# datvo06/MSAU

Measured on AMD Instinct MI355X. Metric: chargrid tiles/sec (train fwd+bwd), 336x256x64 3-stage MSAU, higher is better.
Workload: dtype bf16; 1 GPU; configs[1]: one-hot chargrid 336x256x64, 3-stage MSAU (featRoot 8, 4 scales, res_depth 2), batch 16/GPU, fwd+masked-CE+bwd+clip+Adam; global_batch=16, parallelism=dp1, graph=False

## Files before the change

### include/msau_hip.h

```cpp
#ifndef MSAU_HIP_H
#define MSAU_HIP_H

#include <stdint.h>

#ifdef __cplusplus
extern "C" {
#endif

typedef enum { MSAU_F32 = 0, MSAU_BF16 = 1 } msau_dtype;

typedef enum {
    MSAU_OK = 0,
    MSAU_ERR_ARG = -1,
    MSAU_ERR_LDS = -2,
    MSAU_ERR_HIP = -3
} msau_status;

const char* msau_last_error(void);
int msau_version(void);
const char* msau_source_hash(void);
int msau_sizeof(int which);
int msau_lds_pixel_stride(int raw_bytes, int esz, int c8_per_chunk, int read_stride);
int msau_lds_wrow_stride(int nks, int esz);

enum {
    MSAU_CONV_RELU_IN  = 1,
    MSAU_CONV_RELU_OUT = 2,
    MSAU_CONV_ADD      = 4,
    MSAU_CONV_ACCUM    = 8,
    MSAU_CONV_MASK_A   = 16,
    MSAU_CONV_MASK_B   = 32,
    MSAU_CONV_DOUT     = 128,
    MSAU_CONV_LRN      = 256,
    MSAU_CONV_POOL     = 512,
    MSAU_CONV_IDS      = 1024,
    MSAU_CONV_OWNER    = 2048,
    MSAU_CONV_NCHW     = 4096,
    MSAU_CONV_WGRAD    = 8192,
    MSAU_CONV_ELU      = 32768,
    MSAU_CONV_EXTENT   = 65536,
    MSAU_CONV_HEAD     = 64
};

typedef struct {
    int32_t B, Hin, Win, Hout, Wout;
    int32_t C1, C2;
    int32_t Cout;
    int32_t KH, KW, dil;
    int32_t pad_t, pad_l;
    int32_t stride;
    int32_t ups;
    int32_t flags;
    const void* x1;
    const void* x2;
    const void* wpack;
    const float* bias;
    const void* add;
    const void* mask_a;
    const void* mask_b;
    void* y;
    float* head_probs;
    uint8_t* head_argmax;
    int32_t head_classes;
    int32_t flags2;
    void* y2;
    const void* mask_b2;
    float lrn_alpha_over_n, lrn_beta, lrn_k;
    int32_t reserved0;
    void* pool_y;
    uint8_t* pool_idx;
    const void* wg_x1;
    float* wg_slabs;
    int32_t wg_nslabs;
    int32_t reserved1;
    const int32_t* extent;
} msau_conv_desc;
int msau_conv2d_rider_slabs(int dtype, const msau_conv_desc* d);

typedef struct {
    int32_t cch;
    int32_t nchunks;
    int32_t kchunk;
    int32_t rows;
    int64_t bytes;
} msau_conv_pack_geom;

int msau_conv_pack_geometry(int dtype, int C1_stored, int C2_stored, int Cout_stored, int KH, int KW, int dil,
                            int stride, int ups, msau_conv_pack_geom* out);
int msau_conv2d(void* stream, int dtype, const msau_conv_desc* d);
int msau_conv2d_launch_info(int dtype, const msau_conv_desc* d, int32_t* info8);

enum { MSAU_PAIR_RELU_IN = 1, MSAU_PAIR_RELU_MID = 2, MSAU_PAIR_MASK_MID = 4,
       MSAU_PAIR_LRN_BWD = 16,
       MSAU_PAIR_WGRAD1 = 32,
       MSAU_PAIR_COUPLE = 64,
       MSAU_PAIR_DCOUPLE = 128,
       MSAU_PAIR_TILES = 8 };
typedef struct {
    int32_t B, H, W, C;
    int32_t flags1, flags2;
    const void* x;
    const void* w1;
    const float* b1;
    const void* mask_mid;
    void* mid;
    const void* w2;
    const float* b2;
    const void* add;
    const void* mask_a;
    const void* mask_b;
    void* y;
    void* pool_y;
    uint8_t* pool_idx;
    uint8_t* bits_mid;
    uint8_t* bits_a;
    const void* lrn_a;
    void* lrn_da;
    float lrn_alpha_over_n, lrn_beta, lrn_k;
    int32_t reserved0;
    const void* wg1_x;
    float* wg1_slabs;
    int32_t wg1_nslabs;
    int32_t reserved1;
    const void* cpl_prev;
    const void* cpl_w;
    const float* cpl_b;
    void* cpl_y;
    void* cpl_pool_y;
    uint8_t* cpl_pool_idx;
    const void* dcp_dz;
    const void* dcp_w;
    const void* dcp_mask;
    void* dcp_dprev;
} msau_conv_pair_desc;
int msau_conv_pair_applicable(int dtype, const msau_conv_pair_desc* d);
int msau_conv_pair(void* stream, int dtype, const msau_conv_pair_desc* d);
int64_t msau_conv_pair_bits_bytes(int dtype, const msau_conv_pair_desc* d);
int msau_conv_pair_wgrad_slabs(int dtype, const msau_conv_pair_desc* d);
int msau_conv_pair_instance(int dtype, const msau_conv_pair_desc* d);
void msau_reload_env(void);

typedef struct {
    int32_t B, Hin, Win, Hout, Wout;
    int32_t C1, C2, Cout;
    int32_t KH, KW, dil, pad_t, pad_l, stride;
    int32_t flags;
    const void* x1;
    const void* x2;
    const void* g;
    float* slabs;
    int32_t nslabs;
} msau_wgrad_desc;

typedef struct {
    int32_t cch, nchunks;
    int32_t kext;
    int32_t max_slabs;
    int64_t slab_bytes;
    int32_t lean;
    int32_t reserved;
} msau_wgrad_geom;

int msau_wgrad_geometry(int dtype, const msau_wgrad_desc* d, msau_wgrad_geom* out);
int msau_conv2d_wgrad(void* stream, int dtype, const msau_wgrad_desc* d);
int msau_conv2d_wgrad_groupable(int dtype, const msau_wgrad_desc* a, const msau_wgrad_desc* b);
int msau_conv2d_wgrad_group(void* stream, int dtype, const msau_wgrad_desc* const* ds, int n);

typedef struct {
    int64_t src_off;
    int64_t dst_off;
    int32_t kind;
    int32_t dim0, dim1;
    int32_t KH, KW;
    int32_t row_is_dim0;
    int32_t flip;
    int32_t row_off;
    int32_t rows_real;
    int32_t rows_pad;
    int32_t k1_real, k1_store, k2_real, k2_store;
    int32_t cch, nchunks, kchunk;
    int32_t dtype;
} msau_pack_entry;

int msau_pack_params(void* stream, const float* flat_params, void* pack_arena,
                     const msau_pack_entry* table_dev, int n_entries, int max_elems_per_entry);

typedef struct {
    int64_t slab_off;
    int64_t w_off;
    int64_t b_off;
    int64_t b_src_off;
    int64_t b_slab_stride;
    int32_t b_elem_stride;
    int32_t b_nslabs;
    int32_t b_count;
    int32_t nslabs;
    int32_t slab_elems;
    int32_t kext;
    int32_t dim0, dim1, KH, KW;
    int32_t row_is_dim0;
    int32_t rows_real;
    int32_t k1_real, k1_store, k2_real, k2_store;
    int32_t cch, nchunks;
    int32_t accumulate;
} msau_unpack_entry;

int msau_wgrad_reduce(void* stream, const float* slab_arena, float* flat_grads,
                      const msau_unpack_entry* table_dev, int n_entries, int max_elems_per_entry);

int msau_channel_sum(void* stream, int dtype, const void* g, int64_t npix, int Cs, float* partials, int nblk);

int msau_nchw_to_nhwc(void* stream, int dtype, const float* src, void* dst, int B, int C, int Cs, int H, int W);
int msau_nhwc_to_nchw(void* stream, int dtype, const void* src, float* dst, int B, int C, int Cs, int H, int W);
int msau_nchw_grad_to_nhwc(void* stream, int dtype, const float* src, void* dst, int B, int C, int Cs, int H, int W,
                           int accumulate);

int msau_lrn_fwd(void* stream, int dtype, const void* a, void* y, int64_t npix, int C, int Cs, int n,
                 float alpha, float beta, float k);
int msau_lrn_bwd(void* stream, int dtype, const void* a, const void* dy, void* da, int64_t npix, int C, int Cs,
                 int n, float alpha, float beta, float k);

int msau_maxpool2x2_fwd(void* stream, int dtype, const void* x, void* y, uint8_t* idx, int B, int H, int W, int Cs);
int msau_maxpool2x2_bwd(void* stream, int dtype, const void* dy, const uint8_t* idx, void* dx, const void* mask,
                        int B, int H, int W, int Cs, int accumulate);
int msau_maxpool2x2_bwd_ext(void* stream, int dtype, const void* dy, const uint8_t* idx, void* dx, const void* mask,
                            int B, int H, int W, int Cs, int accumulate, const int32_t* extent);

int msau_selfattn_fwd(void* stream, int dtype, const void* f, const void* g, const void* h, const void* x, void* y,
                      float* stats , int B, int N, int Ds, int Cs);
int msau_selfattn_bwd(void* stream, int dtype, const void* f, const void* g, const void* h, const void* dy,
                      const float* stats, void* df, void* dg, void* dh, float* ws, int B, int N, int Ds, int Cs);
int msau_selfattn_fwd_ext(void* stream, int dtype, const void* f, const void* g, const void* h, const void* x, void* y,
                          float* stats, int B, int N, int Ds, int Cs, const int32_t* extent, int W);
int msau_selfattn_bwd_ext(void* stream, int dtype, const void* f, const void* g, const void* h, const void* dy,
                          const float* stats, void* df, void* dg, void* dh, float* ws, int B, int N, int Ds, int Cs,
                          const int32_t* extent, int W);

int msau_extent_copy(void* stream, const void* src, void* dst, int B, int planes, int H, int W, int pixel_bytes, const int32_t* extent);

typedef struct {
    const void* df; const void* dg; const void* dh;
    const void* wf_pack; const void* wg_pack; const void* wh_pack;
    const void* add;
    const void* mask_b;
    void* dx;
    int64_t npix;
    int32_t C, accumulate;
} msau_attn_proj_bwd_args;
int msau_attn_proj_bwd(void* stream, int dtype, const msau_attn_proj_bwd_args* a);

typedef struct {
    const void* g;
    const void* w1_pack; const void* w2_pack;
    void* dx1; void* dx2;
    const void* mask1; const void* mask2;
    int64_t npix;
    int32_t C, accumulate1, accumulate2, reserved;
} msau_dgrad2_args;
int msau_dgrad2_1x1(void* stream, int dtype, const msau_dgrad2_args* a);

int msau_label_counts(void* stream, const int64_t* labels, int32_t* counts, int B, int64_t hw);
int msau_label_counts_split(void* stream, const int64_t* labels, int32_t* partial, int B, int64_t hw, int K);
int64_t msau_ce_ws_floats(int64_t npix_total);
int msau_masked_ce(void* stream, int dtype, const void* logits, const int64_t* labels, const int32_t* counts,
                   void* dlogits, float* loss_accum, float* ws, int B, int64_t hw, int C, int Cs, float scale);
int64_t msau_ce_multi_ws_floats(int64_t npix_total);
int msau_masked_ce_multi(void* stream, int dtype, const void* logits, const void* aux, const int64_t* labels,
                         const int32_t* counts, void* dlogits, void* daux, float* loss, float* ws,
                         int B, int64_t hw, int C, int Cs, float scale, int counts_k);

int msau_softmax_ce(void* stream, int dtype, const void* logits, const int64_t* labels, void* dlogits,
                    float* loss_accum, float* ws, int B, int64_t hw, int C, int Cs, float scale);
int msau_softmax_ce_weighted(void* stream, int dtype, const void* logits, const int64_t* labels, const float* class_w,
                             void* dlogits, float* sums, float* ws, int B, int64_t hw, int C, int Cs);

int64_t msau_adam_ws_floats(int64_t n);
int msau_clip_adam_step(void* stream, float* params, const float* grads, float* m, float* v, float* state,
                        float* ws, int64_t n, float lr, float beta1, float beta2, float eps, float max_norm,
                        float grad_scale);

#define MSAU_OPTIM_ADAM 0
#define MSAU_OPTIM_RMSPROP 1
#define MSAU_OPTIM_MOMENTUM 2
#define MSAU_OPTIM_MAX_SKIP 8
int64_t msau_optim_ws_floats(int64_t n);
int msau_optim_step(void* stream, int kind, float* params, const float* grads, float* state_a, float* state_b, float* state,
                    float* ws, int64_t n, float lr, double c1, double c2, float eps, float weight_decay, float max_norm,
                    float grad_scale, const int64_t* skip, int n_skip);

int msau_raster_owner(void* stream, const int32_t* boxes, int n, int32_t* owner, int B, int H, int W);
int msau_raster_owner_ext(void* stream, const int32_t* boxes, int n, int32_t* owner, int B, int H, int W, const int32_t* extent);
int msau_raster_onehot(void* stream, int dtype, const int32_t* boxes, const int32_t* owner, void* grid_nhwc,
                       int B, int H, int W, int C, int Cs);
int msau_raster_labels(void* stream, const int32_t* boxes, const int32_t* owner, int64_t* labels, int B, int H, int W);
int msau_raster_dense(void* stream, int dtype, const int32_t* boxes, const int32_t* owner, const float* feats,
                      void* grid_nhwc, int B, int H, int W, int C, int Cs);

int64_t msau_box_integral_ws_floats(int B, int H, int W, int C);
int msau_box_integral(void* stream, int dtype, const void* in_nhwc, float* ii, float* ws, int B, int H, int W, int C, int Cs, int relu_in);
int msau_box_params(void* stream, const float* flat_params, int64_t off_hmin, int64_t off_hmax, int64_t off_wmin, int64_t off_wmax,
                    int C, int F, float max_h, float max_w, float* params_fwd, float* params_refl);
// ... 119 lines not shown
```

### msau_amd/_lib.py

```python
from __future__ import annotations

import ctypes as C
import os

HERE = os.path.dirname(os.path.abspath(__file__))
LIB_PATH = os.environ.get("MSAU_HIP_LIB", os.path.join(HERE, "libmsau_hip.so"))

F32, BF16 = 0, 1
OPTIM_ADAM, OPTIM_RMSPROP, OPTIM_MOMENTUM, OPTIM_MAX_SKIP = 0, 1, 2, 8

CONV_RELU_IN, CONV_RELU_OUT, CONV_ADD, CONV_ACCUM, CONV_MASK_A, CONV_MASK_B, CONV_HEAD, CONV_DOUT = 1, 2, 4, 8, 16, 32, 64, 128
CONV_LRN, CONV_POOL, CONV_IDS, CONV_OWNER, CONV_NCHW, CONV_WGRAD, CONV_ELU = 256, 512, 1024, 2048, 4096, 8192, 32768
CONV_EXTENT = 65536

i32, i64, vp, f32 = C.c_int32, C.c_int64, C.c_void_p, C.c_float


class ConvDesc(C.Structure):
    _fields_ = [(n, i32) for n in ("B", "Hin", "Win", "Hout", "Wout", "C1", "C2", "Cout", "KH", "KW", "dil",
                                   "pad_t", "pad_l", "stride", "ups", "flags")] + \
               [(n, vp) for n in ("x1", "x2", "wpack", "bias", "add", "mask_a", "mask_b", "y", "head_probs", "head_argmax")] + \
               [("head_classes", i32), ("flags2", i32), ("y2", vp), ("mask_b2", vp)] + \
               [("lrn_alpha_over_n", f32), ("lrn_beta", f32), ("lrn_k", f32), ("reserved0", i32), ("pool_y", vp), ("pool_idx", vp)] + \
               [("wg_x1", vp), ("wg_slabs", vp), ("wg_nslabs", i32), ("reserved1", i32), ("extent", vp)]


class ConvPairDesc(C.Structure):
    _fields_ = [(n, i32) for n in ("B", "H", "W", "C", "flags1", "flags2")] + \
               [(n, vp) for n in ("x", "w1", "b1", "mask_mid", "mid", "w2", "b2", "add", "mask_a", "mask_b", "y", "pool_y", "pool_idx", "bits_mid", "bits_a",
                                  "lrn_a", "lrn_da")] + \
               [("lrn_alpha_over_n", f32), ("lrn_beta", f32), ("lrn_k", f32), ("reserved0", i32), ("wg1_x", vp), ("wg1_slabs", vp), ("wg1_nslabs", i32), ("reserved1", i32)] + \
               [(n, vp) for n in ("cpl_prev", "cpl_w", "cpl_b", "cpl_y", "cpl_pool_y", "cpl_pool_idx", "dcp_dz", "dcp_w", "dcp_mask", "dcp_dprev")]


PAIR_RELU_IN, PAIR_RELU_MID, PAIR_MASK_MID, PAIR_TILES, PAIR_LRN_BWD, PAIR_WGRAD1, PAIR_COUPLE, PAIR_DCOUPLE = 1, 2, 4, 8, 16, 32, 64, 128


class BoxArgs(C.Structure):
    _fields_ = [(n, vp) for n in ("in_", "ii", "params_fwd", "params_refl", "out", "gout", "gin", "ii_g", "ws", "flat_grads", "ws_ii",
                                  "mask_a", "add", "mask_b")] + \
               [(n, i64) for n in ("off_hmin", "off_hmax", "off_wmin", "off_wmax")] + \
               [(n, i32) for n in ("B", "H", "W", "C", "F", "Cs_in", "Cs_out", "relu_in", "accumulate")] + \
               [("max_h", f32), ("max_w", f32)]


class ConvPackGeom(C.Structure):
    _fields_ = [("cch", i32), ("nchunks", i32), ("kchunk", i32), ("rows", i32), ("bytes", i64)]


class WgradDesc(C.Structure):
    _fields_ = [(n, i32) for n in ("B", "Hin", "Win", "Hout", "Wout", "C1", "C2", "Cout", "KH", "KW", "dil",
                                   "pad_t", "pad_l", "stride", "flags")] + \
               [(n, vp) for n in ("x1", "x2", "g", "slabs")] + [("nslabs", i32)]


class WgradGeom(C.Structure):
    _fields_ = [("cch", i32), ("nchunks", i32), ("kext", i32), ("max_slabs", i32), ("slab_bytes", i64),
                ("lean", i32), ("reserved", i32)]


class PackEntry(C.Structure):
    _fields_ = [("src_off", i64), ("dst_off", i64)] + \
               [(n, i32) for n in ("kind", "dim0", "dim1", "KH", "KW", "row_is_dim0", "flip", "row_off", "rows_real",
                                   "rows_pad", "k1_real", "k1_store", "k2_real", "k2_store", "cch", "nchunks",
                                   "kchunk", "dtype")]


class UnpackEntry(C.Structure):
    _fields_ = [("slab_off", i64), ("w_off", i64), ("b_off", i64), ("b_src_off", i64), ("b_slab_stride", i64)] + \
               [(n, i32) for n in ("b_elem_stride", "b_nslabs", "b_count", "nslabs", "slab_elems", "kext", "dim0", "dim1", "KH",
                                   "KW", "row_is_dim0", "rows_real", "k1_real", "k1_store", "k2_real", "k2_store",
                                   "cch", "nchunks", "accumulate")]


class Op(C.Structure):
    _fields_ = [("kind", i32), ("dtype", i32), ("args", vp)]


class LrnArgs(C.Structure):
    _fields_ = [("a", vp), ("dy", vp), ("out", vp), ("npix", i64), ("C", i32), ("Cs", i32), ("n", i32),
                ("alpha", f32), ("beta", f32), ("k", f32)]


class PoolArgs(C.Structure):
    _fields_ = [("x_or_dy", vp), ("y_or_dx", vp), ("idx", vp), ("mask", vp)] + \
               [(n, i32) for n in ("B", "H", "W", "Cs", "accumulate")] + [("extent", vp)]


class AttnArgs(C.Structure):
    _fields_ = [(n, vp) for n in ("f", "g", "h", "x_or_dy", "y", "stats", "df", "dg", "dh", "ws")] + \
               [(n, i32) for n in ("B", "N", "Ds", "Cs")] + [("extent", vp), ("W", i32), ("reserved0", i32)]


class CsumArgs(C.Structure):
    _fields_ = [("g", vp), ("npix", i64), ("Cs", i32), ("partials", vp), ("nblk", i32)]


class ReduceArgs(C.Structure):
    _fields_ = [("slab_arena", vp), ("flat_grads", vp), ("table_dev", vp), ("n_entries", i32), ("max_elems", i32)]


class AllreduceArgs(C.Structure):
    _fields_ = [("comm", vp), ("buf", vp), ("count", i64)]


class OwnerCtx(C.Structure):
    _fields_ = [(n, vp) for n in ("owner", "boxes", "feats", "w", "wt", "table", "sums", "csum")] + \
               [(n, i32) for n in ("n_boxes", "n_vec", "C", "csum_blocks", "wt_floats", "reserved0")]


class AttnProjBwdArgs(C.Structure):
    _fields_ = [(n, vp) for n in ("df", "dg", "dh", "wf_pack", "wg_pack", "wh_pack", "add", "mask_b", "dx")] + \
               [("npix", i64), ("C", i32), ("accumulate", i32)]


class Dgrad2Args(C.Structure):
    _fields_ = [(n, vp) for n in ("g", "w1_pack", "w2_pack", "dx1", "dx2", "mask1", "mask2")] + \
               [("npix", i64), ("C", i32), ("accumulate1", i32), ("accumulate2", i32), ("reserved", i32)]


OP_SIDE = 0x100
OP_PROBE = 0x200
OP_COMM = 0x400
OP_JOIN = 0x800
OP_ALLREDUCE = 14
OP_WGRAD_REDUCE = 10
OP_CONV_PAIR = 11
OP_BOX_FWD, OP_BOX_BWD = 12, 13
OP_ATTN_PROJ_BWD = 15
OP_DGRAD2_1X1 = 16
OP_CONV2D, OP_WGRAD, OP_LRN_FWD, OP_LRN_BWD, OP_POOL_FWD, OP_POOL_BWD, OP_ATTN_FWD, OP_ATTN_BWD, OP_CHANNEL_SUM = range(1, 10)

_SIGNATURES = {
    "msau_last_error": (C.c_char_p, []),
    "msau_version": (C.c_int, []),
    "msau_source_hash": (C.c_char_p, []),
    "msau_sizeof": (C.c_int, [C.c_int]),
    "msau_lds_pixel_stride": (C.c_int, [C.c_int, C.c_int, C.c_int, C.c_int]),
    "msau_lds_wrow_stride": (C.c_int, [C.c_int, C.c_int]),
    "msau_conv_pack_geometry": (C.c_int, [C.c_int] * 9 + [C.POINTER(ConvPackGeom)]),
    "msau_conv2d": (C.c_int, [vp, C.c_int, C.POINTER(ConvDesc)]),
    "msau_conv2d_rider_slabs": (C.c_int, [C.c_int, C.POINTER(ConvDesc)]),
    "msau_attn_proj_bwd": (C.c_int, [vp, C.c_int, C.POINTER(AttnProjBwdArgs)]),
    "msau_dgrad2_1x1": (C.c_int, [vp, C.c_int, C.POINTER(Dgrad2Args)]),
    "msau_conv2d_launch_info": (C.c_int, [C.c_int, C.POINTER(ConvDesc), C.POINTER(i32)]),
    "msau_conv_pair_applicable": (C.c_int, [C.c_int, C.POINTER(ConvPairDesc)]),
    "msau_conv_pair": (C.c_int, [vp, C.c_int, C.POINTER(ConvPairDesc)]),
    "msau_conv_pair_bits_bytes": (C.c_int64, [C.c_int, C.POINTER(ConvPairDesc)]),
    "msau_conv_pair_instance": (C.c_int, [C.c_int, C.POINTER(ConvPairDesc)]),
    "msau_conv_pair_wgrad_slabs": (C.c_int, [C.c_int, C.POINTER(ConvPairDesc)]),
    "msau_owner_slabs": (C.c_int, [C.POINTER(WgradDesc)]),
    "msau_comm_available": (C.c_int, []),
    "msau_comm_unique_id": (C.c_int, [vp, C.c_int]),
    "msau_comm_init": (C.c_int, [C.POINTER(vp), C.c_int, C.c_int, vp, C.c_int]),
    "msau_comm_destroy": (C.c_int, [vp]),
    "msau_allreduce_bucket": (C.c_int, [vp, vp, vp, C.c_int64]),
    "msau_run_ops_dp": (C.c_int, [vp, vp, vp, C.POINTER(Op), C.c_int, C.c_int]),
    "msau_reload_env": (None, []),
    "msau_wgrad_geometry": (C.c_int, [C.c_int, C.POINTER(WgradDesc), C.POINTER(WgradGeom)]),
    "msau_conv2d_wgrad": (C.c_int, [vp, C.c_int, C.POINTER(WgradDesc)]),
    "msau_conv2d_wgrad_groupable": (C.c_int, [C.c_int, C.POINTER(WgradDesc), C.POINTER(WgradDesc)]),
    "msau_conv2d_wgrad_group": (C.c_int, [vp, C.c_int, C.POINTER(C.POINTER(WgradDesc)), C.c_int]),
    "msau_pack_params": (C.c_int, [vp, vp, vp, vp, C.c_int, C.c_int]),
    "msau_wgrad_reduce": (C.c_int, [vp, vp, vp, vp, C.c_int, C.c_int]),
    "msau_channel_sum": (C.c_int, [vp, C.c_int, vp, i64, C.c_int, vp, C.c_int]),
    "msau_nchw_to_nhwc": (C.c_int, [vp, C.c_int, vp, vp] + [C.c_int] * 5),
    "msau_nhwc_to_nchw": (C.c_int, [vp, C.c_int, vp, vp] + [C.c_int] * 5),
    "msau_nchw_grad_to_nhwc": (C.c_int, [vp, C.c_int, vp, vp] + [C.c_int] * 6),
    "msau_lrn_fwd": (C.c_int, [vp, C.c_int, vp, vp, i64, C.c_int, C.c_int, C.c_int, f32, f32, f32]),
    "msau_lrn_bwd": (C.c_int, [vp, C.c_int, vp, vp, vp, i64, C.c_int, C.c_int, C.c_int, f32, f32, f32]),
    "msau_maxpool2x2_fwd": (C.c_int, [vp, C.c_int, vp, vp, vp] + [C.c_int] * 4),
    "msau_maxpool2x2_bwd": (C.c_int, [vp, C.c_int, vp, vp, vp, vp] + [C.c_int] * 5),
    "msau_selfattn_fwd": (C.c_int, [vp, C.c_int, vp, vp, vp, vp, vp, vp] + [C.c_int] * 4),
    "msau_selfattn_bwd": (C.c_int, [vp, C.c_int, vp, vp, vp, vp, vp, vp, vp, vp, vp] + [C.c_int] * 4),
    "msau_maxpool2x2_bwd_ext": (C.c_int, [vp, C.c_int, vp, vp, vp, vp] + [C.c_int] * 5 + [vp]),
    "msau_selfattn_fwd_ext": (C.c_int, [vp, C.c_int, vp, vp, vp, vp, vp, vp] + [C.c_int] * 4 + [vp, C.c_int]),
    "msau_selfattn_bwd_ext": (C.c_int, [vp, C.c_int, vp, vp, vp, vp, vp, vp, vp, vp, vp] + [C.c_int] * 4 + [vp, C.c_int]),
    "msau_extent_copy": (C.c_int, [vp, vp, vp] + [C.c_int] * 5 + [vp]),
    "msau_label_counts": (C.c_int, [vp, vp, vp, C.c_int, i64]),
    "msau_label_counts_split": (C.c_int, [vp, vp, vp, C.c_int, i64, C.c_int]),
    "msau_ce_ws_floats": (i64, [i64]),
    "msau_ce_multi_ws_floats": (i64, [i64]),
    "msau_masked_ce_multi": (C.c_int, [vp, C.c_int, vp, vp, vp, vp, vp, vp, vp, vp, C.c_int, i64, C.c_int, C.c_int, f32, C.c_int]),
    "msau_masked_ce": (C.c_int, [vp, C.c_int, vp, vp, vp, vp, vp, vp, C.c_int, i64, C.c_int, C.c_int, f32]),
    "msau_softmax_ce": (C.c_int, [vp, C.c_int, vp, vp, vp, vp, vp, C.c_int, i64, C.c_int, C.c_int, f32]),
    "msau_softmax_ce_weighted": (C.c_int, [vp, C.c_int, vp, vp, vp, vp, vp, vp, C.c_int, i64, C.c_int, C.c_int]),
    "msau_adam_ws_floats": (i64, [i64]),
    "msau_clip_adam_step": (C.c_int, [vp, vp, vp, vp, vp, vp, vp, i64, f32, f32, f32, f32, f32, f32]),
    "msau_optim_ws_floats": (i64, [i64]),
    "msau_optim_step": (C.c_int, [vp, C.c_int, vp, vp, vp, vp, vp, vp, i64, f32, C.c_double, C.c_double, f32, f32, f32, f32, vp, C.c_int]),
    "msau_raster_owner": (C.c_int, [vp, vp, C.c_int, vp, C.c_int, C.c_int, C.c_int]),
    "msau_raster_owner_ext": (C.c_int, [vp, vp, C.c_int, vp, C.c_int, C.c_int, C.c_int, vp]),
    "msau_raster_onehot": (C.c_int, [vp, C.c_int, vp, vp, vp] + [C.c_int] * 5),
    "msau_raster_labels": (C.c_int, [vp, vp, vp, vp, C.c_int, C.c_int, C.c_int]),
    "msau_raster_dense": (C.c_int, [vp, C.c_int, vp, vp, vp, vp] + [C.c_int] * 5),
    "msau_box_integral_ws_floats": (i64, [C.c_int] * 4),
    "msau_box_integral": (C.c_int, [vp, C.c_int, vp, vp, vp] + [C.c_int] * 6),
    "msau_box_params": (C.c_int, [vp, vp, i64, i64, i64, i64, C.c_int, C.c_int, f32, f32, vp, vp]),
    "msau_box_filter": (C.c_int, [vp, C.c_int, vp, vp, vp] + [C.c_int] * 8 + [vp, vp, vp]),
    "msau_box_fwd": (C.c_int, [vp, C.c_int, C.POINTER(BoxArgs)]),
    "msau_box_bwd": (C.c_int, [vp, C.c_int, C.POINTER(BoxArgs)]),
    "msau_box_pgrad_ws_floats": (i64, [C.c_int] * 5),
    "msau_box_param_grad": (C.c_int, [vp, C.c_int, vp, vp, vp, vp, vp, i64, i64, i64, i64] + [C.c_int] * 6 + [f32, f32]),
    "msau_run_ops": (C.c_int, [vp, C.POINTER(Op), C.c_int]),
    "msau_run_ops_overlap": (C.c_int, [vp, vp, C.POINTER(Op), C.c_int, C.c_int]),
    "msau_spin": (C.c_int, [vp, C.c_int]),
    "msau_fill_zero": (C.c_int, [vp, vp, i64]),
    "msau_fork_visibility_check": (C.c_int, [vp, vp, C.c_int, i64, C.c_int, C.POINTER(i64)]),
    "msau_stream_create": (C.c_int, [C.c_int, C.POINTER(vp)]),
    "msau_stream_destroy": (C.c_int, [vp]),
    "msau_softmax_channels_nchw": (C.c_int, [vp, vp, vp, C.c_int, C.c_int, i64]),
    "msau_probe_read": (C.c_int, [vp, C.c_int, vp]),
    "msau_probe_overhead": (C.c_int, [vp, C.c_int, vp]),
    "msau_softmax_argmax_nhwc": (C.c_int, [vp, C.c_int, vp, vp, vp, i64, C.c_int, C.c_int]),
    "msau_onehot_ids": (C.c_int, [vp, C.c_int, vp, vp, i64, C.c_int, C.c_int]),
    "msau_onehot_ids_ext": (C.c_int, [vp, C.c_int, vp, vp] + [C.c_int] * 5 + [vp]),
    "msau_eval_confusion": (C.c_int, [vp, C.c_int, vp, vp, vp] + [C.c_int] * 6 + [vp]),
    "msau_kv_regions_limits": (C.c_int, [C.POINTER(i32)]),
    "msau_kv_regions": (C.c_int, [vp] * 7 + [C.c_int] * 4 + [vp, vp, C.c_int, vp, C.c_int, vp]),
    "msau_kv_paint": (C.c_int, [vp] * 6 + [C.c_int] * 3 + [vp, vp, vp]),
    "msau_kv_paint_train": (C.c_int, [vp] * 7 + [C.c_int] * 3 + [vp, vp, vp]),
    "msau_label_hist": (C.c_int, [vp, vp, vp, vp] + [C.c_int] * 5),
    "msau_unet_ce_ws_floats": (i64, [i64]),
    "msau_unet_ce": (C.c_int, [vp, C.c_int] + [vp] * 7 + [C.c_int, vp, vp, vp, vp] + [C.c_int] * 5),
    "msau_unet_eval_ws_bytes": (i64, [C.c_int, C.c_int]),
    "msau_unet_eval": (C.c_int, [vp, C.c_int] + [vp] * 6 + [C.c_int, vp, vp, vp] + [C.c_int] * 5),
}

EXPORTED_SYMBOLS = tuple(_SIGNATURES)

ABI_STRUCTS = (ConvDesc, WgradDesc, PackEntry, UnpackEntry, Op, LrnArgs, PoolArgs, AttnArgs, CsumArgs, ReduceArgs,
               ConvPackGeom, WgradGeom, ConvPairDesc, BoxArgs, AllreduceArgs, OwnerCtx, AttnProjBwdArgs, Dgrad2Args)


class MsauHipError(RuntimeError):
    pass


_lib = None


def load():
    global _lib
    if _lib is not None:
        return _lib
    if not os.path.exists(LIB_PATH):
        raise MsauHipError(f"{LIB_PATH} not found: the MSAU HIP kernels are not built "
                           f"(run `python -m msau_amd.build`); there is no CPU fallback")
    lib = C.CDLL(LIB_PATH)
    for name, (res, args) in _SIGNATURES.items():
        fn = getattr(lib, name)
        fn.restype = res
        fn.argtypes = args
    for which, st in enumerate(ABI_STRUCTS):
        if lib.msau_sizeof(which) != C.sizeof(st):
            raise MsauHipError(f"{LIB_PATH}: sizeof({st.__name__}) is {lib.msau_sizeof(which)} in the library, "
                               f"{C.sizeof(st)} in msau_amd/_lib.py -- rebuild (python -m msau_amd.build)")
    if "MSAU_HIP_LIB" not in os.environ and os.path.isdir(os.path.join(HERE, "csrc")):
        from .build import source_hash
        have, want = lib.msau_source_hash().decode(), source_hash()
        if have != want:
            raise MsauHipError(f"{LIB_PATH} was built from kernel sources {have}, the tree holds {want}: rebuild "
                               f"(python -m msau_amd.build)")
    _lib = lib
    return lib


def check(rc: int, what: str = ""):
    if rc != 0:
        msg = load().msau_last_error().decode("utf-8", "replace")
        raise MsauHipError(f"{what or 'msau call'} failed (status {rc}): {msg}")


class Profiler:

    def __init__(self):
        self.records = []
        self.key = None

    def summary(self):
        import collections
        out = collections.OrderedDict()
        for key, e0, e1 in self.records:
            c, t = out.get(key, (0, 0.0))
            out[key] = (c + 1, t + e0.elapsed_time(e1))
        return out


_profiler = None


def set_profiler(p):
    global _profiler
    _profiler = p


def call(name: str, *args, key=None):
    if _profiler is None:
# ... 48 lines not shown
```

### msau_amd/csrc/conv.hip

```cpp
#include "msau_common.h"

namespace {

struct ConvGeom {
    int esz, taps, cch, nchunks, kchunk, rows, CT, ngroups;
    int nslices;
};

__host__ __device__ inline int pix_stride_bytes(int cch, int esz) {
    int ps = cch * esz;
    if (((ps >> 4) & 1) == 0) ps += 16;
    return ps;
}

struct TileGeom { int TH, TIH, TIW, PS, WS, in_bytes, w_bytes, tab_bytes, total; };

inline bool conv_compact(int KH, int KW, int dil, int stride, int ups) { return stride == 1 && ups == 1 && dil >= 16 && KH * KW > 1; }

inline TileGeom tile_geom(const ConvGeom& g, int PT, int KH, int KW, int dil, int stride, int ups = 1) {
    TileGeom t;
    t.TH = 4 * PT;
    t.TIH = (t.TH - 1) * stride + (KH - 1) * dil + 1;
    t.TIW = 15 * stride + (KW - 1) * dil + 1;
    if (conv_compact(KH, KW, dil, stride, ups)) { t.TIH = KH * KW * t.TH; t.TIW = 16; }
// ... 161 lines not shown
            }
            *reinterpret_cast<V8*>(lds_in + pix * a.PS + cg * 8 * (int)sizeof(T)) = v;
        }
        const T* wsrc = wp + ((size_t)chunk * a.rows_total + ct0 * 16) * a.kchunk;
        for (int idx = tid; idx < rows * wg_per_row; idx += 256) {
            int r = idx / wg_per_row, g8 = idx - r * wg_per_row;
            *reinterpret_cast<V8*>(lds_w + r * a.WS + g8 * 8 * (int)sizeof(T)) = load8<T>(wsrc + (size_t)r * a.kchunk + g8 * 8);
        }
        __syncthreads();
        for (int ks = 0; ks < nks; ++ks) {
            const int G = ks * 4 + lg;
            const int koff = koff_tab[G];
            V8 bfrag[PT];
#pragma unroll
            for (int pt = 0; pt < PT; ++pt) bfrag[pt] = *reinterpret_cast<const V8*>(lds_in + pixoff[pt] + koff);
#pragma unroll
            for (int ct = 0; ct < CT; ++ct) {
                V8 afrag = *reinterpret_cast<const V8*>(lds_w + (ct * 16 + lr) * a.WS + G * 8 * (int)sizeof(T));
#pragma unroll
                for (int pt = 0; pt < PT; ++pt) acc[ct][pt] = mma8(afrag, bfrag[pt], acc[ct][pt]);
            }
        }
    }

    const int Cout = d.Cout;
    T* y = static_cast<T*>(d.y);
    const T* add = static_cast<const T*>(d.add);
    const T* mask_a = static_cast<const T*>(d.mask_a);
    const T* mask_b = static_cast<const T*>(d.mask_b);
    const int flags = d.flags;
    int ext_h = d.Hout, ext_w = d.Wout;
    if (flags & MSAU_CONV_EXTENT) { ext_h = d.extent[2 * b]; ext_w = d.extent[2 * b + 1]; }
#pragma unroll
    for (int pt = 0; pt < PT; ++pt) {
        const int oy = oy0 + wave * PT + pt, ox = ox0 + lr;
        if (oy >= d.Hout || ox >= d.Wout) continue;
        const bool outside = oy >= ext_h || ox >= ext_w;
        const size_t pbase = (((size_t)b * d.Hout + oy) * d.Wout + ox) * a.ystride;
#pragma unroll
        for (int ct = 0; ct < CT; ++ct) {
            const int co = lg * (CTT * 4) + (ct0 + ct) * 4;
            if (co >= Cout) continue;
            f32x4 v = acc[ct][pt];
            if (d.bias) {
                f32x4 bv = *reinterpret_cast<const f32x4*>(d.bias + co);
                v += bv;
            }
            if (flags & MSAU_CONV_MASK_A) {
                V4 m = load4<T>(mask_a + pbase + co);
#pragma unroll
                for (int j = 0; j < 4; ++j) v[j] = ((float)m[j] > 0.f) ? v[j] : 0.f;
            }
            if (flags & MSAU_CONV_ADD) {
                V4 r = load4<T>(add + pbase + co);
#pragma unroll
                for (int j = 0; j < 4; ++j) v[j] += (float)r[j];
            }
            if (flags & MSAU_CONV_ACCUM) {
                V4 r = load4<T>(y + pbase + co);
#pragma unroll
                for (int j = 0; j < 4; ++j) v[j] += (float)r[j];
            }
            if (flags & MSAU_CONV_RELU_OUT) {
                if (flags & MSAU_CONV_ELU) {
#pragma unroll
                    for (int j = 0; j < 4; ++j) v[j] = v[j] > 0.f ? v[j] : expm1f(v[j]);
                } else {
#pragma unroll
                    for (int j = 0; j < 4; ++j) v[j] = fmaxf(v[j], 0.f);
                }
            }
            if (flags & MSAU_CONV_MASK_B) {
                V4 m = load4<T>(mask_b + pbase + co);
                if (flags & MSAU_CONV_ELU) {
#pragma unroll
                    for (int j = 0; j < 4; ++j) v[j] = ((float)m[j] > 0.f) ? v[j] : v[j] * ((float)m[j] + 1.f);
                } else {
#pragma unroll
                    for (int j = 0; j < 4; ++j) v[j] = ((float)m[j] > 0.f) ? v[j] : 0.f;
                }
            }
            if (outside) v = f32x4{0.f, 0.f, 0.f, 0.f};
            V4 o;
#pragma unroll
            for (int j = 0; j < 4; ++j) o[j] = (T)v[j];
            store4<T>(y + pbase + co, o);
        }
    }
}

template <typename T, int CT, int PT>
int launch_conv(hipStream_t s, const ConvArgs& a, int nblocks, int nsplit, int lds) {
    static bool attr_set = false;
    if (!attr_set) {
        hipError_t e = hipFuncSetAttribute(reinterpret_cast<const void*>(&conv_kernel<T, CT, PT>),
                                           hipFuncAttributeMaxDynamicSharedMemorySize, MSAU_LDS_LIMIT);
        if (e != hipSuccess) return msau_set_error(MSAU_ERR_HIP, "conv: hipFuncSetAttribute: %s", hipGetErrorString(e));
        attr_set = true;
    }
    hipLaunchKernelGGL((conv_kernel<T, CT, PT>), dim3(nblocks, nsplit), dim3(256), lds, s, a);
    MSAU_CHECK_LAUNCH("conv_kernel");
    return 0;
}

template <typename T, int CT>
int launch_conv_pt(hipStream_t s, const ConvArgs& a, int PT, int nblocks, int nsplit, int lds) {
    switch (PT) {
        case 4: return launch_conv<T, CT, 4>(s, a, nblocks, nsplit, lds);
        case 2: return launch_conv<T, CT, 2>(s, a, nblocks, nsplit, lds);
        default: return launch_conv<T, CT, 1>(s, a, nblocks, nsplit, lds);
    }
}

template <typename T>
int launch_conv_ct(hipStream_t s, const ConvArgs& a, int CT, int PT, int nblocks, int nsplit, int lds) {
    switch (CT) {
        case 1: return launch_conv_pt<T, 1>(s, a, PT, nblocks, nsplit, lds);
        case 2: return launch_conv_pt<T, 2>(s, a, PT, nblocks, nsplit, lds);
        case 4: return launch_conv_pt<T, 4>(s, a, PT, nblocks, nsplit, lds);
        default: return launch_conv_pt<T, 8>(s, a, PT, nblocks, nsplit, lds);
    }
}

}

extern "C" int msau_conv_pack_geometry(int dtype, int C1, int C2, int Cout, int KH, int KW, int dil, int stride, int ups,
                                       msau_conv_pack_geom* out) {
    ConvGeom g;
    int rc = conv_geom(dtype, C1, C2, Cout, KH, KW, dil, stride, ups, &g);
    if (rc) return rc;
    out->cch = g.cch; out->nchunks = g.nchunks; out->kchunk = g.kchunk; out->rows = g.rows * g.nslices;
    out->bytes = (int64_t)g.nslices * g.nchunks * g.rows * g.kchunk * g.esz;
    return 0;
}

static int conv_plan(int dtype, const msau_conv_desc* d, ConvGeom* gout, TileGeom* tout, int* PTout, int64_t* nbout) {
    ConvGeom g;
    int rc = conv_geom(dtype, d->C1, d->C2, d->Cout, d->KH, d->KW, d->dil, d->stride, d->ups, &g);
    if (rc) return rc;
    int PT = 4;
    auto ntiles = [&](int pt) { return (int64_t)d->B * cdiv(d->Hout, 4 * pt) * cdiv(d->Wout, 16); };
    if (ntiles(4) < 512) PT = ntiles(2) >= 384 ? 2 : 1;
    TileGeom t = tile_geom(g, PT, d->KH, d->KW, d->dil, d->stride, d->ups);
    while (t.total > 150 * 1024 && PT > 1) { PT >>= 1; t = tile_geom(g, PT, d->KH, d->KW, d->dil, d->stride, d->ups); }
    if (t.total > 150 * 1024) return msau_set_error(MSAU_ERR_LDS, "conv2d: tile needs %d B of LDS", t.total);
    int64_t nb = ntiles(PT);
    MSAU_CHECK_ARG(nb < (1ll << 31), "conv2d: grid too large");
    *gout = g; *tout = t; *PTout = PT; *nbout = nb;
    return 0;
}

enum { CONV_TILE = 0, CONV_LEAN = 1, CONV_CHUNKED = 2, CONV_ROWS = 3,
       CONV_OWNER = 4, CONV_FIRST_NCHW = 5, CONV_REFUSED = 6 };
constexpr int kRefusalOrder[] = {MSAU_CONV_EXTENT, MSAU_CONV_WGRAD, MSAU_CONV_OWNER, MSAU_CONV_NCHW, MSAU_CONV_HEAD, MSAU_CONV_DOUT,
                                 MSAU_CONV_LRN, MSAU_CONV_IDS, MSAU_CONV_POOL};
constexpr int kOnlyOthers = MSAU_CONV_WGRAD | MSAU_CONV_OWNER | MSAU_CONV_NCHW | MSAU_CONV_HEAD | MSAU_CONV_DOUT | MSAU_CONV_LRN |
                            MSAU_CONV_IDS | MSAU_CONV_POOL;
struct ConvRoute {
    int family, inst;
    int refused;
    int geom_rc;
    ConvGeom g; TileGeom t; int PT; int64_t nb;
};

static int conv_route(int dtype, const msau_conv_desc* d, ConvRoute* r, int families = ~0) {
    const int f = d->flags;
    auto asked = [&](int family) { return (families >> family) & 1; };
    *r = ConvRoute{};
    r->family = CONV_REFUSED;
    const int rc = r->geom_rc = conv_plan(dtype, d, &r->g, &r->t, &r->PT, &r->nb);
    if (f & MSAU_CONV_OWNER) {
        if (asked(CONV_OWNER) && msau_ownerconv_takes(dtype, d)) { r->family = CONV_OWNER; r->inst = 1; return 0; }
    } else if (f & MSAU_CONV_NCHW) {
        if (asked(CONV_FIRST_NCHW) && msau_firstconv_takes(dtype, d)) { r->family = CONV_FIRST_NCHW; r->inst = 1; return 0; }
    } else if (!rc) {
        const ConvGeom& g = r->g;
        if (g.nslices > 1) r->inst = 0;
        else if (asked(CONV_ROWS) && (r->inst = msau_rowconv_case(dtype, d))) r->family = CONV_ROWS;
        else if (asked(CONV_CHUNKED) && (r->inst = msau_conv_chunked_case(dtype, d, g.cch, g.nchunks, g.CT))) r->family = CONV_CHUNKED;
        else if (asked(CONV_LEAN) && (r->inst = msau_conv_lean_case(dtype, d, g.nchunks, g.CT))) r->family = CONV_LEAN;
        if (r->family == CONV_REFUSED && asked(CONV_TILE) && !(f & kOnlyOthers)) r->family = CONV_TILE;
    }
    if (rc) return rc;
    if (r->family == CONV_REFUSED)
        for (int flag : kRefusalOrder)
            if (f & flag) { r->refused = flag; break; }
    return 0;
}

static int conv_refusal(const msau_conv_desc* d, int flag) {
    switch (flag) {
        case MSAU_CONV_EXTENT:
            return msau_set_error(MSAU_ERR_ARG, "conv2d: MSAU_CONV_EXTENT is not implemented for this launch (flags 0x%x; see "
                                  "msau_conv2d_launch_info info[7] & 128): only the generic tile kernel and the box-list instance have it", d->flags);
        case MSAU_CONV_WGRAD:
            return msau_set_error(MSAU_ERR_ARG, "conv2d: MSAU_CONV_WGRAD is not implemented for this launch (msau_conv2d_rider_slabs says 0)");
        case MSAU_CONV_OWNER:
            return msau_set_error(MSAU_ERR_ARG, "conv2d: MSAU_CONV_OWNER is the 3x3 stride-1 C -> 8 conv, no other flag but RELU_OUT and EXTENT");
        case MSAU_CONV_NCHW:
            return msau_set_error(MSAU_ERR_ARG, "conv2d: MSAU_CONV_NCHW is the bf16 3x3 64 -> 8 conv (W %% 4 == 0, W <= 288), head_classes = real input channels");
        case MSAU_CONV_HEAD:
            return msau_set_error(MSAU_ERR_ARG, "conv2d: MSAU_CONV_HEAD is not implemented for this launch (see "
                                  "msau_conv2d_launch_info info[7]); run msau_softmax_argmax_nhwc on y instead");
        case MSAU_CONV_DOUT:
            return msau_set_error(MSAU_ERR_ARG, "conv2d: MSAU_CONV_DOUT is not implemented for this launch (see "
                                  "msau_conv2d_launch_info info[7]); issue one launch per output instead");
        case MSAU_CONV_LRN:
            return msau_set_error(MSAU_ERR_ARG, "conv2d: MSAU_CONV_LRN is not implemented for this launch (see "
                                  "msau_conv2d_launch_info info[7]); run msau_lrn_fwd on y instead");
        case MSAU_CONV_IDS:
            return msau_set_error(MSAU_ERR_ARG, "conv2d: MSAU_CONV_IDS is not implemented for this launch (see msau_conv2d_launch_info "
                                  "info[7] & 16); paint the one-hot input with msau_onehot_ids instead");
        default:
            return msau_set_error(MSAU_ERR_ARG, "conv2d: MSAU_CONV_POOL is not implemented for this launch (see "
                                  "msau_conv2d_launch_info info[7]); run msau_maxpool2x2_fwd on y instead");
    }
}

static int conv_offers(int dtype, const msau_conv_desc* d, int flag, int ignore = 0, int families = ~0) {
    msau_conv_desc p = *d;
    p.flags = (p.flags & ~ignore) | flag;
    if (flag == MSAU_CONV_LRN) {
        if (!p.y2) p.y2 = p.y;
        if (!(p.lrn_k > 0.f)) p.lrn_k = 1.f;
    }
    ConvRoute r;
    return conv_route(dtype, &p, &r, families) || r.family == CONV_REFUSED ? -1 : r.family;
}

extern "C" int msau_conv2d_launch_info(int dtype, const msau_conv_desc* d, int32_t* info) {
    MSAU_CHECK_ARG(d && info, "conv2d_launch_info: null pointer");
    ConvRoute r;
    int rc = conv_route(dtype, d, &r);
    if (rc || r.geom_rc) return rc ? rc : r.geom_rc;
    info[0] = r.g.CT; info[1] = r.PT; info[2] = r.t.total; info[3] = (int32_t)r.nb; info[4] = r.g.cch; info[5] = r.g.nchunks;
    info[6] = r.family <= CONV_ROWS ? r.family : 0;
    const int lean = 1 << CONV_LEAN, rows = 1 << CONV_ROWS;
    const int feeds = MSAU_CONV_IDS | MSAU_CONV_OWNER | MSAU_CONV_NCHW | MSAU_CONV_WGRAD;
    const int fused = MSAU_CONV_HEAD | MSAU_CONV_DOUT | MSAU_CONV_LRN | MSAU_CONV_POOL;
    info[7] = (conv_offers(dtype, d, MSAU_CONV_HEAD, feeds | fused, lean) == CONV_LEAN) |
              ((conv_offers(dtype, d, MSAU_CONV_DOUT, feeds | fused, lean) == CONV_LEAN ||
                ((d->flags & MSAU_CONV_DOUT) && r.family == CONV_ROWS)) << 1) |
              ((conv_offers(dtype, d, MSAU_CONV_LRN, feeds, lean) == CONV_LEAN || conv_offers(dtype, d, MSAU_CONV_LRN, 0, rows) == CONV_ROWS) << 2) |
              ((conv_offers(dtype, d, MSAU_CONV_POOL, feeds, lean) == CONV_LEAN) << 3) |
              ((conv_offers(dtype, d, MSAU_CONV_IDS) == CONV_LEAN) << 4) |
              ((conv_offers(dtype, d, MSAU_CONV_OWNER) == CONV_OWNER) << 5) |
              ((conv_offers(dtype, d, MSAU_CONV_NCHW) == CONV_FIRST_NCHW) << 6) |
              ((conv_offers(dtype, d, MSAU_CONV_EXTENT) >= 0) << 7);
    return 0;
}

extern "C" int msau_conv2d_rider_slabs(int dtype, const msau_conv_desc* d) {
    ConvRoute r;
    if (!d || !(d->flags & MSAU_CONV_WGRAD) || conv_route(dtype, d, &r) || r.family != CONV_ROWS) return 0;
    return msau_rowconv_workgroups(d);
}

static int tile_launch(hipStream_t s, int dtype, const msau_conv_desc* d, const ConvRoute& r) {
    const ConvGeom& g = r.g;
    const TileGeom& t = r.t;
    const int PT = r.PT;
    static const int split_wgs = getenv("MSAU_CONV_ROWSPLIT") ? atoi(getenv("MSAU_CONV_ROWSPLIT")) : 768;
    int cts = g.CT;
    while (cts > 1 && r.nb * g.nslices * (g.CT / cts) < split_wgs) cts >>= 1;
    const int w_bytes = roundup(cts * 16 * t.WS, 16), lds_total = t.in_bytes + w_bytes + t.tab_bytes;
    for (int sl = 0; sl < g.nslices; ++sl) {
        ConvArgs a;
        a.d = *d;
        a.ystride = d->Cout;
        a.compact = conv_compact(d->KH, d->KW, d->dil, d->stride, d->ups);
        if (g.nslices > 1) {
            const size_t co0 = (size_t)sl * 128, esz = g.esz;
            a.d.Cout = d->Cout - (int)co0 < 128 ? d->Cout - (int)co0 : 128;
            a.d.wpack = static_cast<const char*>(d->wpack) + (size_t)sl * g.nchunks * g.rows * g.kchunk * esz;
            if (d->bias) a.d.bias = d->bias + co0;
            a.d.y = static_cast<char*>(d->y) + co0 * esz;
            if (d->add) a.d.add = static_cast<const char*>(d->add) + co0 * esz;
            if (d->mask_a) a.d.mask_a = static_cast<const char*>(d->mask_a) + co0 * esz;
            if (d->mask_b) a.d.mask_b = static_cast<const char*>(d->mask_b) + co0 * esz;
        }
        a.cch = g.cch; a.nchunks = g.nchunks; a.kchunk = g.kchunk; a.ngroups = g.ngroups;
        a.TIH = t.TIH; a.TIW = t.TIW; a.PS = t.PS; a.WS = t.WS; a.in_bytes = t.in_bytes; a.w_bytes = w_bytes;
        a.tiles_x = cdiv(d->Wout, 16); a.tiles_y = cdiv(d->Hout, 4 * PT);
        a.ct_total = g.CT; a.rows_total = g.rows;
        int rc = dtype == MSAU_F32 ? launch_conv_ct<float>(s, a, cts, PT, (int)r.nb, g.CT / cts, lds_total)
                                   : launch_conv_ct<bf16_t>(s, a, cts, PT, (int)r.nb, g.CT / cts, lds_total);
        if (rc) return rc;
    }
    return 0;
}

extern "C" int msau_conv2d(void* stream, int dtype, const msau_conv_desc* d) {
    MSAU_CHECK_ARG(d && d->x1 && d->wpack && d->y, "conv2d: null pointer");
    MSAU_CHECK_ARG(d->B > 0 && d->Hin > 0 && d->Win > 0 && d->Hout > 0 && d->Wout > 0, "conv2d: bad dims");
    MSAU_CHECK_ARG(d->C1 % 8 == 0 && d->C2 % 8 == 0 && (d->C2 == 0 || d->x2), "conv2d: bad sources");
    MSAU_CHECK_ARG(!(d->flags & MSAU_CONV_ADD) || d->add, "conv2d: ADD without pointer");
    MSAU_CHECK_ARG(!(d->flags & MSAU_CONV_MASK_A) || d->mask_a, "conv2d: MASK_A without pointer");
    MSAU_CHECK_ARG(!(d->flags & MSAU_CONV_MASK_B) || d->mask_b, "conv2d: MASK_B without pointer");
    MSAU_CHECK_ARG(!(d->flags & MSAU_CONV_EXTENT) || d->extent, "conv2d: MSAU_CONV_EXTENT without extent pointer");
    ConvRoute r;
    int rc = conv_route(dtype, d, &r);
    if (rc) return rc;
    const bool refused = r.family == CONV_REFUSED;
    if (refused && (r.refused & (MSAU_CONV_EXTENT | MSAU_CONV_WGRAD | MSAU_CONV_OWNER | MSAU_CONV_NCHW))) return conv_refusal(d, r.refused);
    if (d->flags & MSAU_CONV_HEAD)
        MSAU_CHECK_ARG(d->head_probs && d->head_argmax && d->head_classes > 0 && d->head_classes <= 16 &&
                       d->head_classes <= d->Cout && d->flags == MSAU_CONV_HEAD, "conv2d: bad HEAD arguments");
    if (d->flags & MSAU_CONV_DOUT) {
        const int okf = MSAU_CONV_DOUT | MSAU_CONV_ADD | MSAU_CONV_ACCUM | MSAU_CONV_MASK_B | MSAU_CONV_WGRAD;
        MSAU_CHECK_ARG(d->y2 && !(d->flags & ~okf) && !(d->flags2 & ~(MSAU_CONV_ACCUM | MSAU_CONV_MASK_B)) &&
                       (!(d->flags2 & MSAU_CONV_MASK_B) || d->mask_b2), "conv2d: bad DOUT arguments");
    }
    if (d->flags & MSAU_CONV_LRN)
        MSAU_CHECK_ARG(d->y2 && !(d->flags & ~(MSAU_CONV_LRN | MSAU_CONV_RELU_IN)) && d->lrn_k > 0.f, "conv2d: bad LRN arguments");
    if (refused && r.refused != MSAU_CONV_POOL) return conv_refusal(d, r.refused);
    if (d->flags & MSAU_CONV_POOL)
        MSAU_CHECK_ARG(d->pool_y && !(d->flags & (MSAU_CONV_DOUT | MSAU_CONV_HEAD | MSAU_CONV_LRN)), "conv2d: bad POOL arguments");
    if (refused) return conv_refusal(d, r.refused);
    hipStream_t s = static_cast<hipStream_t>(stream);
    switch (r.family) {
        case CONV_OWNER: return msau_ownerconv_fwd(s, dtype, d);
        case CONV_FIRST_NCHW:
            if (!(d->head_classes > 0 && d->head_classes <= d->C1)) return conv_refusal(d, MSAU_CONV_NCHW);
            return msau_firstconv_launch(s, dtype, d, d->head_classes);
        case CONV_ROWS: return msau_rowconv_launch(s, d, r.g.kchunk, r.g.rows, r.inst);
        case CONV_CHUNKED: return msau_conv_chunked_launch(s, dtype, d, r.g.kchunk, r.g.nchunks, r.g.CT, r.inst);
        case CONV_LEAN: return msau_conv_lean_launch(s, dtype, d, r.g.kchunk, r.g.CT, r.inst);
        default: return tile_launch(s, dtype, d, r);
    }
}
```

### msau_amd/csrc/conv_first.hip

```cpp
#include "msau_common.h"
#include <cstdlib>

#ifndef MSAU_FIRST_DEPTH
#define MSAU_FIRST_DEPTH 2
#endif

namespace {

typedef unsigned int u32x4 __attribute__((ext_vector_type(4)));
constexpr unsigned kOOB = 0x80000000u;
constexpr int PS = 160;
constexpr int WS = 18 * 64 + 32;
constexpr int W_BYTES = 16 * WS;

struct FirstArgs {
    const float* x;
    unsigned char* xn;
    const bf16_t* wpack;
    const float* bias;
    unsigned char* y;
    int B, C, H, W;
    int nseg, SH;
    int slot_px;
    int relu_out;
};

__device__ __forceinline__ __amdgpu_buffer_rsrc_t rsrc_of(const void* p, unsigned bytes) {
    return __builtin_amdgcn_make_buffer_rsrc(const_cast<void*>(p), 0, bytes, 0x00020000);
}

template <int NI, int NTW>
__global__ __launch_bounds__(256) void first_conv_nchw_kernel(const FirstArgs a) {
    extern __shared__ __align__(16) unsigned char smem[];
    const int tid = threadIdx.x, lane = tid & 63;
    const int wave = __builtin_amdgcn_readfirstlane(tid >> 6);
    const int lr = lane & 15, lg = lane >> 4;
    const int b = blockIdx.x / a.nseg, seg = blockIdx.x - b * a.nseg;
    const int H = a.H, W = a.W;
    const int y0 = seg * a.SH, y1 = min(H, y0 + a.SH);
    if (y0 >= y1) return;
    const int slot_bytes = a.slot_px * PS;
    unsigned char* wl = smem + 3 * slot_bytes;

    {
        constexpr int NWI = 16 * 72, NITW = (NWI + 255) / 256;
        bf16x8 wr[NITW];
#pragma unroll
        for (int it = 0; it < NITW; ++it) {
            const int idx = min(tid + it * 256, NWI - 1);
            const int r = idx / 72, g8 = idx - r * 72;
            wr[it] = load8<bf16_t>(a.wpack + r * 576 + g8 * 8);
        }
        for (int i = tid; i < 3 * slot_bytes / 16; i += 256) *reinterpret_cast<u32x4*>(smem + i * 16) = u32x4{0u, 0u, 0u, 0u};
#pragma unroll
        for (int it = 0; it < NITW; ++it) {
            const int idx = tid + it * 256;
            const int r = idx / 72, g8 = idx - r * 72;
            if (idx < NWI) *reinterpret_cast<bf16x8*>(wl + r * WS + g8 * 16) = wr[it];
        }
    }

    const unsigned plane = (unsigned)H * (unsigned)W * 4u;
    const float* xb = a.x + (size_t)b * a.C * H * W;
    const unsigned img_n = (unsigned)H * (unsigned)W * 128u;
    unsigned char* nb = a.xn ? a.xn + (size_t)b * img_n : nullptr;
    const unsigned img_y = (unsigned)H * (unsigned)W * 16u;
    const __amdgpu_buffer_rsrc_t ry = rsrc_of(a.y + (size_t)b * img_y, img_y);

    const int cg = lane & 7, qs = lane >> 3;
    unsigned ld_off[NI];
    unsigned st_off[NI];
    int lds_px[NI];
#pragma unroll
    for (int it = 0; it < NI; ++it) {
        const int px0 = ((wave + 4 * it) * 8 + qs) * 4;
        ld_off[it] = px0 < W ? (unsigned)(cg * 8) * plane + (unsigned)px0 * 4u : kOOB;
        st_off[it] = px0 < W ? (unsigned)px0 * 128u + (unsigned)cg * 16u : kOOB;
        lds_px[it] = px0 < W ? (px0 + 1) * PS : 0;
    }
    constexpr int DEPTH = MSAU_FIRST_DEPTH;
    f32x4 rr[DEPTH][NI][8];
    auto load_row = [&](int r, f32x4 (&v)[NI][8]) {
        const bool ok = r >= 0 && r < H;
        const __amdgpu_buffer_rsrc_t rx = rsrc_of(xb, ok ? (unsigned)a.C * plane : 0u);
        const unsigned ro = ok ? (unsigned)r * (unsigned)W * 4u : 0u;
#pragma unroll
        for (int it = 0; it < NI; ++it)
#pragma unroll
            for (int k = 0; k < 8; ++k)
                v[it][k] = __builtin_bit_cast(f32x4, __builtin_amdgcn_raw_buffer_load_b128(rx, ld_off[it] + (unsigned)k * plane + ro, 0, 0));
    };
    auto put_row = [&](int r, const f32x4 (&v)[NI][8]) {
        unsigned char* slot = smem + ((r + 3) % 3) * slot_bytes;
        const bool own = r >= y0 && r < y1;
        const __amdgpu_buffer_rsrc_t rn = rsrc_of(nb, own && nb ? img_n : 0u);
        const unsigned no = own ? (unsigned)r * (unsigned)W * 128u : 0u;
#pragma unroll
        for (int it = 0; it < NI; ++it) {
#pragma unroll
            for (int p = 0; p < 4; ++p) {
                bf16x8 o;
#pragma unroll
                for (int k = 0; k < 8; ++k) o[k] = (bf16_t)v[it][k][p];
                *reinterpret_cast<bf16x8*>(slot + lds_px[it] + (lds_px[it] ? p * PS : 0) + cg * 16) = o;
                __builtin_amdgcn_raw_buffer_store_b128(__builtin_bit_cast(u32x4, o), rn, st_off[it] + (unsigned)p * 128u + no, 0, 0);
            }
        }
    };

    const int col0 = wave * 16 + lr;
    float bv[4] = {0.f, 0.f, 0.f, 0.f};
    if (a.bias && lg < 2) {
#pragma unroll
        for (int j = 0; j < 4; ++j) bv[j] = a.bias[lg * 4 + j];
    }
    auto compute_row = [&](int o) {
        f32x4 acc[NTW];
#pragma unroll
        for (int t = 0; t < NTW; ++t) acc[t] = f32x4{0.f, 0.f, 0.f, 0.f};
#pragma unroll
        for (int ks = 0; ks < 18; ++ks) {
            const int tap = ks >> 1, ky = tap / 3, kx = tap - ky * 3;
            const bf16x8 af = *reinterpret_cast<const bf16x8*>(wl + lr * WS + ks * 64 + lg * 16);
            const unsigned char* rowp = smem + ((o + ky + 2) % 3) * slot_bytes + (col0 + kx) * PS + ((ks & 1) * 4 + lg) * 16;
#pragma unroll
            for (int t = 0; t < NTW; ++t) {
                const bf16x8 bf = *reinterpret_cast<const bf16x8*>(rowp + t * 64 * PS);
                acc[t] = __builtin_amdgcn_mfma_f32_16x16x32_bf16(af, bf, acc[t], 0, 0, 0);
            }
        }
        const unsigned yo = (unsigned)o * (unsigned)W * 16u;
#pragma unroll
        for (int t = 0; t < NTW; ++t) {
            const int col = col0 + 64 * t;
            bf16x4 ov;
#pragma unroll
            for (int j = 0; j < 4; ++j) {
                float v = acc[t][j] + bv[j];
                if (a.relu_out) v = fmaxf(v, 0.f);
                ov[j] = (bf16_t)v;
            }
            __builtin_amdgcn_raw_buffer_store_b64(__builtin_bit_cast(unsigned __attribute__((ext_vector_type(2))), ov), ry,
                                                  lg < 2 && col < W ? yo + (unsigned)col * 16u + (unsigned)lg * 8u : kOOB, 0, 0);
        }
    };

#pragma unroll
    for (int dd = 0; dd < DEPTH; ++dd) load_row(y0 - 1 + dd, rr[dd]);
    __syncthreads();
    for (int r = y0 - 1; r <= y1; r += DEPTH) {
#pragma unroll
        for (int dd = 0; dd < DEPTH; ++dd) {
            const int row = r + dd;
            if (row <= y1) {
                put_row(row, rr[dd]);
                load_row(row + DEPTH <= y1 ? row + DEPTH : -1, rr[dd]);
                __syncthreads();
                if (row - 1 >= y0) compute_row(row - 1);
                __syncthreads();
            }
        }
    }
}

int slot_pixels(int W) { return roundup(W, 16) + 2; }

}

int msau_firstconv_takes(int dtype, const msau_conv_desc* d) {
    static const bool off = std::getenv("MSAU_FIRST_NCHW") && std::getenv("MSAU_FIRST_NCHW")[0] == '0';
    if (off || dtype != MSAU_BF16 || !d) return 0;
    if (d->flags & ~(MSAU_CONV_NCHW | MSAU_CONV_RELU_OUT)) return 0;
    if (d->C1 != 64 || d->C2 || d->Cout != 8 || d->KH != 3 || d->KW != 3 || d->dil != 1 || d->stride != 1 || d->ups != 1) return 0;
    if (d->pad_t != 1 || d->pad_l != 1 || d->Hin != d->Hout || d->Win != d->Wout) return 0;
    if (d->Win % 4 || d->Win > 320 || d->Win < 16 || d->Hin < 2) return 0;
    if ((int64_t)d->Hin * d->Win * 64 * 4 >= (1ll << 31)) return 0;
    if (3 * slot_pixels(d->Win) * PS + W_BYTES + 256 > MSAU_LDS_LIMIT) return 0;
    return 1;
}

int msau_firstconv_launch(hipStream_t s, int dtype, const msau_conv_desc* d, int real_channels) {
    (void)dtype;
    FirstArgs a;
    a.x = static_cast<const float*>(d->x1);
    a.xn = static_cast<unsigned char*>(d->y2);
    a.wpack = static_cast<const bf16_t*>(d->wpack);
    a.bias = d->bias;
    a.y = static_cast<unsigned char*>(d->y);
    a.B = d->B; a.C = real_channels; a.H = d->Hin; a.W = d->Win;
    int nseg = cdiv(256, d->B);
    if (nseg > d->Hin / 8) nseg = d->Hin / 8;
    if (nseg < 1) nseg = 1;
    a.SH = cdiv(d->Hin, nseg);
    a.nseg = cdiv(d->Hin, a.SH);
    a.slot_px = slot_pixels(d->Win);
    a.relu_out = (d->flags & MSAU_CONV_RELU_OUT) ? 1 : 0;
    const int lds = 3 * a.slot_px * PS + W_BYTES;
    const int ni = cdiv(d->Win, 128), ntw = cdiv(d->Win, 64);
#define FIRST_CASE(NIV, NTWV)                                                                                                  \
    if (ni <= NIV && ntw <= NTWV) {                                                                                            \
        static bool attr_set = false;                                                                                          \
        if (!attr_set) {                                                                                                       \
            hipError_t e = hipFuncSetAttribute(reinterpret_cast<const void*>(&first_conv_nchw_kernel<NIV, NTWV>),              \
                                               hipFuncAttributeMaxDynamicSharedMemorySize, MSAU_LDS_LIMIT);                    \
            if (e != hipSuccess) return msau_set_error(MSAU_ERR_HIP, "first_conv: hipFuncSetAttribute: %s", hipGetErrorString(e)); \
            attr_set = true;                                                                                                   \
        }                                                                                                                      \
        hipLaunchKernelGGL((first_conv_nchw_kernel<NIV, NTWV>), dim3(a.B * a.nseg), dim3(256), lds, s, a);                    \
        MSAU_CHECK_LAUNCH("first_conv_nchw_kernel");                                                                           \
        return 0;                                                                                                              \
    }
    FIRST_CASE(1, 2) FIRST_CASE(2, 4) FIRST_CASE(3, 5)
#undef FIRST_CASE
    return msau_set_error(MSAU_ERR_ARG, "first_conv: no instance for width %d", d->Win);
}
```

### msau_amd/csrc/conv_wgrad.hip

```cpp
#include "msau_common.h"

namespace {

struct WGeom {
    int esz, taps, cch, nchunks, kreal, kextc, NKT, NKW, CTN, compact, slice;
    int TIH, TIW, PSx, PSg, x_bytes, g_bytes, tab_bytes, total;
};

inline int pix_stride(int c, int esz) {
    int ps = c * esz;
    if (((ps >> 4) & 1) == 0) ps += 16;
    return ps;
}

int wgrad_geom(int dtype, const msau_wgrad_desc* d, WGeom* out) {
    MSAU_CHECK_ARG(dtype == MSAU_F32 || dtype == MSAU_BF16, "wgrad: bad dtype");
    const int Cin = d->C1 + d->C2;
    MSAU_CHECK_ARG(Cin > 0 && Cin % 8 == 0 && d->Cout > 0 && d->Cout % 8 == 0 && d->Cout <= 1024, "wgrad: bad channels");
    MSAU_CHECK_ARG(d->KH >= 1 && d->KW >= 1 && d->KH <= 7 && d->KW <= 7 && d->dil >= 1 && (d->stride == 1 || d->stride == 2), "wgrad: bad kernel");
    WGeom g;
    g.esz = dtype == MSAU_F32 ? 4 : 2;
    g.taps = d->KH * d->KW;
    g.compact = d->stride == 1 && d->dil >= 16 && g.taps > 1;
    g.slice = g.esz == 4 ? (g.compact ? 32 : 64) : 128;
// ... 116 lines not shown
            *reinterpret_cast<V8*>(lds_x + pix * a.PSx + cg * 8 * (int)sizeof(T)) = v;
        }
        for (int idx = tid; idx < 256 * cog; idx += 256) {
            int m = idx / cog, cg = idx - m * cog;
            int oy = oy0 + (m >> 4), ox = ox0 + (m & 15);
            V8 v = zero8<T>();
            if (oy < d.Hout && ox < d.Wout)
                v = load8<T>(gp + (((size_t)b * d.Hout + oy) * d.Wout + ox) * a.g_stride + a.co0 + cg * 8);
            *reinterpret_cast<V8*>(lds_g + m * a.PSg + cg * 8 * (int)sizeof(T)) = v;
        }
        __syncthreads();

        if constexpr (sizeof(T) == 2) {
            typedef __attribute__((address_space(3))) bf16x4* lds_v4;
            const int q = li >> 2, p = li & 3;
            for (int blk = 0; blk < 8; ++blk) {
                const int m0 = blk * 32 + lg * 8 + q;
                const int m1 = m0 + 4;
                bf16x8 afrag[CTN];
#pragma unroll
                for (int ct = 0; ct < CTN; ++ct) {
                    bf16x4 lo = __builtin_amdgcn_ds_read_tr16_b64_v4bf16((lds_v4)(lds_g + m0 * a.PSg + (ct * 16 + 4 * p) * 2));
                    bf16x4 hi = __builtin_amdgcn_ds_read_tr16_b64_v4bf16((lds_v4)(lds_g + m1 * a.PSg + (ct * 16 + 4 * p) * 2));
                    afrag[ct] = __builtin_shufflevector(lo, hi, 0, 1, 2, 3, 4, 5, 6, 7);
                }
                const int pb0 = (((m0 >> 4) * d.stride) * a.TIW + (m0 & 15) * d.stride) * a.PSx;
                const int pb1 = (((m1 >> 4) * d.stride) * a.TIW + (m1 & 15) * d.stride) * a.PSx;
#pragma unroll
                for (int i = 0; i < NKW; ++i) {
                    const int e = tab[(wave + 4 * i) * 4 + p];
                    const int o0 = (e & TAB_ABS) ? (e & ~TAB_ABS) : pb0 + e;
                    const int o1 = (e & TAB_ABS) ? (e & ~TAB_ABS) : pb1 + e;
                    bf16x4 lo = __builtin_amdgcn_ds_read_tr16_b64_v4bf16((lds_v4)(smem + o0));
                    bf16x4 hi = __builtin_amdgcn_ds_read_tr16_b64_v4bf16((lds_v4)(smem + o1));
                    bf16x8 bfrag = __builtin_shufflevector(lo, hi, 0, 1, 2, 3, 4, 5, 6, 7);
#pragma unroll
                    for (int ct = 0; ct < CTN; ++ct)
                        acc[i][ct] = __builtin_amdgcn_mfma_f32_16x16x32_bf16(afrag[ct], bfrag, acc[i][ct], 0, 0, 0);
                }
            }
        } else {
            int colofs[NKW];
#pragma unroll
            for (int i = 0; i < NKW; ++i) colofs[i] = tab[(wave + 4 * i) * 4 + (li >> 2)] + (li & 3) * 4;
            for (int step = 0; step < 64; ++step) {
                const int m = step * 4 + lg;
                float afrag[CTN];
#pragma unroll
                for (int ct = 0; ct < CTN; ++ct)
                    afrag[ct] = *reinterpret_cast<const float*>(lds_g + m * a.PSg + (ct * 16 + li) * 4);
                const int pb = (((m >> 4) * d.stride) * a.TIW + (m & 15) * d.stride) * a.PSx;
#pragma unroll
                for (int i = 0; i < NKW; ++i) {
                    const int e = colofs[i];
                    const int o = (e & TAB_ABS) ? (e & ~TAB_ABS) : pb + e;
                    const float bv = *reinterpret_cast<const float*>(smem + o);
#pragma unroll
                    for (int ct = 0; ct < CTN; ++ct)
                        acc[i][ct] = __builtin_amdgcn_mfma_f32_16x16x4f32(afrag[ct], bv, acc[i][ct], 0, 0, 0);
                }
            }
        }
    }

    float* slab = d.slabs + (((size_t)blockIdx.x * a.nchunks + chunk) * a.cout_total + a.co0) * a.kextc;
#pragma unroll
    for (int i = 0; i < NKW; ++i) {
        const int nkt = wave + 4 * i;
        if (nkt >= a.NKT) continue;
#pragma unroll
        for (int ct = 0; ct < CTN; ++ct)
#pragma unroll
            for (int j = 0; j < 4; ++j) {
                const int co = ct * 16 + lg * 4 + j;
                if (co < d.Cout) slab[(size_t)co * a.kextc + nkt * 16 + li] = acc[i][ct][j];
            }
    }
}

template <typename T, int CTN, int NKW>
int launch_wgrad(hipStream_t s, const WArgs& a, dim3 grid, int lds) {
    static bool attr_set = false;
    if (!attr_set) {
        hipError_t e = hipFuncSetAttribute(reinterpret_cast<const void*>(&wgrad_kernel<T, CTN, NKW>),
                                           hipFuncAttributeMaxDynamicSharedMemorySize, MSAU_LDS_LIMIT);
        if (e != hipSuccess) return msau_set_error(MSAU_ERR_HIP, "wgrad: hipFuncSetAttribute: %s", hipGetErrorString(e));
        attr_set = true;
    }
    hipLaunchKernelGGL((wgrad_kernel<T, CTN, NKW>), grid, dim3(256), lds, s, a);
    MSAU_CHECK_LAUNCH("wgrad_kernel");
    return 0;
}

template <typename T, int CTN>
int launch_wgrad_nkw(hipStream_t s, const WArgs& a, int NKW, dim3 grid, int lds) {
    if constexpr (CTN == 8) {
        switch (NKW) {
            case 1: return launch_wgrad<T, CTN, 1>(s, a, grid, lds);
            case 2: return launch_wgrad<T, CTN, 2>(s, a, grid, lds);
            case 3: return launch_wgrad<T, CTN, 3>(s, a, grid, lds);
            default: return launch_wgrad<T, CTN, 5>(s, a, grid, lds);
        }
    } else {
        switch (NKW) {
            case 1: return launch_wgrad<T, CTN, 1>(s, a, grid, lds);
            case 2: return launch_wgrad<T, CTN, 2>(s, a, grid, lds);
            case 3: return launch_wgrad<T, CTN, 3>(s, a, grid, lds);
            case 5: return launch_wgrad<T, CTN, 5>(s, a, grid, lds);
            default: return launch_wgrad<T, CTN, 10>(s, a, grid, lds);
        }
    }
}

template <typename T>
int launch_wgrad_ct(hipStream_t s, const WArgs& a, int CTN, int NKW, dim3 grid, int lds) {
    switch (CTN) {
        case 1: return launch_wgrad_nkw<T, 1>(s, a, NKW, grid, lds);
        case 2: return launch_wgrad_nkw<T, 2>(s, a, NKW, grid, lds);
        case 3: case 4: return launch_wgrad_nkw<T, 4>(s, a, NKW, grid, lds);
        default: return launch_wgrad_nkw<T, 8>(s, a, NKW, grid, lds);
    }
}

}

int msau_wgrad_lean_applicable(int dtype, const msau_wgrad_desc* d, int cch);
int msau_wgrad_lean_try(hipStream_t s, int dtype, const msau_wgrad_desc* d, int cch, int nchunks, int kextc);
int msau_wgrad_lean_group(hipStream_t s, int dtype, const msau_wgrad_desc* const* ds, int n, int cch, int nchunks, int kextc);
int msau_wgrad_lean_groupable(int dtype, const msau_wgrad_desc* d, int cch);

extern "C" int msau_wgrad_geometry(int dtype, const msau_wgrad_desc* d, msau_wgrad_geom* out) {
    WGeom g;
    int rc = wgrad_geom(dtype, d, &g);
    if (rc) return rc;
    out->cch = g.cch; out->nchunks = g.nchunks; out->kext = g.kextc;
    out->max_slabs = d->B * cdiv(d->Hout, 16) * cdiv(d->Wout, 16);
    out->slab_bytes = (int64_t)g.nchunks * d->Cout * g.kextc * 4;
    out->lean = msau_wgrad_lean_applicable(dtype, d, g.cch);
    if (d->nslabs >= 1 && msau_rowwgrad_takes(dtype, d, g.cch, g.nchunks, g.kextc)) out->lean = 2;
    out->reserved = 0;
    return 0;
}

extern "C" int msau_conv2d_wgrad(void* stream, int dtype, const msau_wgrad_desc* d) {
    MSAU_CHECK_ARG(d && d->x1 && d->g && d->slabs, "wgrad: null pointer");
    MSAU_CHECK_ARG(d->C2 == 0 || d->x2, "wgrad: x2 missing");
    WGeom g;
    int rc = wgrad_geom(dtype, d, &g);
    if (rc) return rc;
    if (d->flags & MSAU_CONV_OWNER)
        return msau_ownerconv_wgrad(static_cast<hipStream_t>(stream), dtype, d, g.cch, g.nchunks, g.kextc);
    const int tiles_x = cdiv(d->Wout, 16), tiles_y = cdiv(d->Hout, 16), ntiles = d->B * tiles_x * tiles_y;
    MSAU_CHECK_ARG(d->nslabs >= 1 && d->nslabs <= ntiles, "wgrad: nslabs %d not in [1,%d]", d->nslabs, ntiles);
    if (msau_rowwgrad_takes(dtype, d, g.cch, g.nchunks, g.kextc))
        return msau_rowwgrad_launch(static_cast<hipStream_t>(stream), d);
    if (d->Cout <= g.slice) {
        rc = msau_wgrad_lean_try(static_cast<hipStream_t>(stream), dtype, d, g.cch, g.nchunks, g.kextc);
        if (rc != 0) return rc < 0 ? rc : 0;
    }
    MSAU_CHECK_ARG(!(d->flags & MSAU_CONV_IDS), "wgrad: MSAU_CONV_IDS is implemented by the bf16 64 -> 8 3x3 instance only");
    int CTN = g.CTN == 3 ? 4 : (g.CTN > 4 ? 8 : g.CTN);
    MSAU_CHECK_ARG(!(CTN == 8 && g.NKW > 5), "wgrad: Cout %d with K %d unsupported", d->Cout, g.kextc);
    dim3 grid(d->nslabs, g.nchunks);
    hipStream_t s = static_cast<hipStream_t>(stream);
    for (int co0 = 0; co0 < d->Cout; co0 += g.slice) {
        WArgs a;
        a.d = *d;
        a.d.Cout = d->Cout - co0 < g.slice ? d->Cout - co0 : g.slice;
        a.g_stride = d->Cout; a.co0 = co0; a.cout_total = d->Cout; a.compact = g.compact;
        a.cch = g.cch; a.nchunks = g.nchunks; a.kreal = g.kreal; a.kextc = g.kextc; a.NKT = g.NKT;
        a.TIH = g.TIH; a.TIW = g.TIW; a.PSx = g.PSx; a.PSg = g.PSg;
        a.x_bytes = g.x_bytes; a.g_bytes = g.g_bytes; a.tab_bytes = g.tab_bytes;
        a.tiles_x = tiles_x; a.tiles_y = tiles_y; a.ntiles = ntiles;
        rc = dtype == MSAU_F32 ? launch_wgrad_ct<float>(s, a, CTN, g.NKW, grid, g.total) : launch_wgrad_ct<bf16_t>(s, a, CTN, g.NKW, grid, g.total);
        if (rc) return rc;
    }
    return 0;
}

extern "C" int msau_owner_slabs(const msau_wgrad_desc* d) { return d ? msau_ownerconv_slabs(d) : 0; }

extern "C" int msau_conv2d_wgrad_groupable(int dtype, const msau_wgrad_desc* a, const msau_wgrad_desc* b) {
    if (!a || !b) return 0;
    WGeom g;
    if (wgrad_geom(dtype, a, &g)) return 0;
    if (msau_rowwgrad_takes(dtype, a, g.cch, g.nchunks, g.kextc)) return 0;
    if (a->Cout > g.slice || !msau_wgrad_lean_groupable(dtype, a, g.cch)) return 0;
    return a->B == b->B && a->Hin == b->Hin && a->Win == b->Win && a->Hout == b->Hout && a->Wout == b->Wout && a->C1 == b->C1 &&
           a->C2 == b->C2 && a->Cout == b->Cout && a->KH == b->KH && a->KW == b->KW && a->dil == b->dil && a->pad_t == b->pad_t &&
           a->pad_l == b->pad_l && a->stride == b->stride && a->nslabs == b->nslabs;
}

extern "C" int msau_conv2d_wgrad_group(void* stream, int dtype, const msau_wgrad_desc* const* ds, int n) {
    MSAU_CHECK_ARG(ds && n >= 1 && n <= 4, "wgrad_group: 1..4 launches");
    for (int i = 0; i < n; ++i) {
        MSAU_CHECK_ARG(ds[i] && ds[i]->x1 && ds[i]->g && ds[i]->slabs && (ds[i]->C2 == 0 || ds[i]->x2), "wgrad_group: null pointer");
        MSAU_CHECK_ARG(i == 0 || msau_conv2d_wgrad_groupable(dtype, ds[0], ds[i]), "wgrad_group: launch %d differs in shape from launch 0", i);
    }
    if (n == 1) return msau_conv2d_wgrad(stream, dtype, ds[0]);
    WGeom g;
    int rc = wgrad_geom(dtype, ds[0], &g);
    if (rc) return rc;
    const int ntiles = ds[0]->B * cdiv(ds[0]->Wout, 16) * cdiv(ds[0]->Hout, 16);
    MSAU_CHECK_ARG(ds[0]->nslabs >= 1 && ds[0]->nslabs <= ntiles, "wgrad: nslabs %d not in [1,%d]", ds[0]->nslabs, ntiles);
    rc = msau_wgrad_lean_group(static_cast<hipStream_t>(stream), dtype, ds, n, g.cch, g.nchunks, g.kextc);
    if (rc == 1) return 0;
    if (rc < 0) return rc;
    return msau_set_error(MSAU_ERR_ARG, "wgrad_group: no shared-grid instance for this shape");
}
```

### msau_amd/csrc/wgrad_lean.hip

```cpp
#include "msau_common.h"
#include <cstdlib>

namespace {

struct WLeanArgs {
    msau_wgrad_desc d;
    int kextc, nchunks;
    int tiles_x, tiles_y, ntiles;
    unsigned mag_tx, mag_ty;
};

constexpr int kWGroup = 4;
struct WLeanMulti { WLeanArgs a[kWGroup]; };

#define WL_ABS 0x40000000
#ifndef MSAU_WPS_MAX
#define MSAU_WPS_MAX 10
#endif

typedef __attribute__((address_space(3))) bf16x4* lds_v4;

template <typename T, int C8, int CO8, int KS, int DIL = 1, int STRIDE = 1>
struct WLeanCfg {
    static constexpr int ESZ = (int)sizeof(T);
// ... 143 lines not shown

        if constexpr (PS) {
            const int q = li >> 2, p = li & 3;
#pragma unroll
            for (int bb = 0; bb < 2; ++bb) {
                const int blk = wave * 2 + bb;
                const int row = blk * 2 + (lg >> 1), col = (lg & 1) * Cfg::QS + q;
                const unsigned char* ga = lds_g + (row * 16 + col) * PSG + 4 * p * 2;
                bf16x8 afrag[CTN];
#pragma unroll
                for (int ct = 0; ct < CTN; ++ct) {
                    bf16x4 lo = __builtin_amdgcn_ds_read_tr16_b64_v4bf16((lds_v4)(ga + ct * 32));
                    bf16x4 hi = __builtin_amdgcn_ds_read_tr16_b64_v4bf16((lds_v4)(ga + Cfg::HI * PSG + ct * 32));
                    afrag[ct] = __builtin_shufflevector(lo, hi, 0, 1, 2, 3, 4, 5, 6, 7);
                }
                const int pb0 = (row * STRIDE * TI + col * STRIDE) * PSX;
#pragma unroll
                for (int i = 0; i < NKT; ++i) {
                    const int e = coloff[i];
                    const bool abs_ok = (i + 1) * 16 > Cfg::KREAL;
                    const int o0 = (abs_ok && (e & WL_ABS)) ? (e & ~WL_ABS) : pb0 + e;
                    const int o1 = (abs_ok && (e & WL_ABS)) ? (e & ~WL_ABS) : pb0 + Cfg::HI * STRIDE * PSX + e;
                    bf16x4 lo = __builtin_amdgcn_ds_read_tr16_b64_v4bf16((lds_v4)(smem + o0));
                    bf16x4 hi = __builtin_amdgcn_ds_read_tr16_b64_v4bf16((lds_v4)(smem + o1));
                    bf16x8 bfrag = __builtin_shufflevector(lo, hi, 0, 1, 2, 3, 4, 5, 6, 7);
#pragma unroll
                    for (int ct = 0; ct < CTN; ++ct)
                        acc[i][ct] = __builtin_amdgcn_mfma_f32_16x16x32_bf16(afrag[ct], bfrag, acc[i][ct], 0, 0, 0);
                }
            }
        } else if constexpr (sizeof(T) == 2) {
            const int q = li >> 2, p = li & 3;
            constexpr int NBLK = Cfg::W2 ? 4 : 8;
            constexpr int UNR = NKW * CTN >= 40 ? 1 : NBLK;
#pragma unroll UNR
            for (int bq = 0; bq < NBLK; ++bq) {
                const int blk = Cfg::W2 ? wset * 4 + bq : bq;
                const int row = blk * 2 + (lg >> 1), col = (lg & 1) * Cfg::QS + q;
                const unsigned char* ga = lds_g + (row * 16 + col) * PSG + 4 * p * 2;
                bf16x8 afrag[CTN];
#pragma unroll
                for (int ct = 0; ct < CTN; ++ct) {
                    bf16x4 lo = __builtin_amdgcn_ds_read_tr16_b64_v4bf16((lds_v4)(ga + ct * 32));
                    bf16x4 hi = __builtin_amdgcn_ds_read_tr16_b64_v4bf16((lds_v4)(ga + Cfg::HI * PSG + ct * 32));
                    afrag[ct] = __builtin_shufflevector(lo, hi, 0, 1, 2, 3, 4, 5, 6, 7);
                }
                const int pb0 = (row * STRIDE * TI + col * STRIDE) * PSX;
#pragma unroll
                for (int i = 0; i < NKW; ++i) {
                    const int e = coloff[i];
                    const int o0 = (e & WL_ABS) ? (e & ~WL_ABS) : pb0 + e;
                    const int o1 = (e & WL_ABS) ? (e & ~WL_ABS) : pb0 + Cfg::HI * STRIDE * PSX + e;
                    bf16x4 lo = __builtin_amdgcn_ds_read_tr16_b64_v4bf16((lds_v4)(smem + o0));
                    bf16x4 hi = __builtin_amdgcn_ds_read_tr16_b64_v4bf16((lds_v4)(smem + o1));
                    bf16x8 bfrag = __builtin_shufflevector(lo, hi, 0, 1, 2, 3, 4, 5, 6, 7);
#pragma unroll
                    for (int ct = 0; ct < CTN; ++ct)
                        acc[i][ct] = __builtin_amdgcn_mfma_f32_16x16x32_bf16(afrag[ct], bfrag, acc[i][ct], 0, 0, 0);
                }
            }
        } else {
            for (int step = 0; step < 64; ++step) {
                const int m = step * 4 + lg;
                float afrag[CTN];
#pragma unroll
                for (int ct = 0; ct < CTN; ++ct) afrag[ct] = *reinterpret_cast<const float*>(lds_g + m * PSG + (ct * 16 + li) * 4);
                const int pb = ((m >> 4) * STRIDE * TI + (m & 15) * STRIDE) * PSX;
#pragma unroll
                for (int i = 0; i < NKW; ++i) {
                    const int e = coloff[i];
                    const float bv = *reinterpret_cast<const float*>(smem + ((e & WL_ABS) ? (e & ~WL_ABS) : pb + e));
#pragma unroll
                    for (int ct = 0; ct < CTN; ++ct)
                        acc[i][ct] = __builtin_amdgcn_mfma_f32_16x16x4f32(afrag[ct], bv, acc[i][ct], 0, 0, 0);
                }
            }
        }
    }

    float* slab = d.slabs + ((size_t)blockIdx.x * a.nchunks + chunk) * d.Cout * a.kextc;
    if constexpr (PS) {
        __syncthreads();
        f32x4* red = reinterpret_cast<f32x4*>(smem);
#pragma unroll
        for (int i = 0; i < NKT; ++i)
#pragma unroll
            for (int ct = 0; ct < CTN; ++ct) red[((wave * NKT + i) * CTN + ct) * 64 + lane] = acc[i][ct];
        __syncthreads();
#pragma unroll
        for (int ii = 0; ii < NKW; ++ii) {
            const int nkt = wave + 4 * ii;
            if (nkt >= NKT) continue;
#pragma unroll
            for (int ct = 0; ct < CTN; ++ct) {
                f32x4 v = red[((0 * NKT + nkt) * CTN + ct) * 64 + lane];
#pragma unroll
                for (int w = 1; w < 4; ++w) v += red[((w * NKT + nkt) * CTN + ct) * 64 + lane];
#pragma unroll
                for (int j = 0; j < 4; ++j) {
                    const int co = ct * 16 + lg * 4 + j;
                    if (co < d.Cout) slab[(size_t)co * a.kextc + nkt * 16 + li] = v[j];
                }
            }
        }
        return;
    }
    if constexpr (Cfg::W2) {
        constexpr int PER = Cfg::TILE_BYTES / (4 * CTN * 1024) < 1 ? 1 : Cfg::TILE_BYTES / (4 * CTN * 1024);
        f32x4* red = reinterpret_cast<f32x4*>(smem);
        for (int i0 = 0; i0 < NKW; i0 += PER) {
            __syncthreads();
            if (wset == 1) {
#pragma unroll
                for (int i = 0; i < NKW; ++i)
                    if (i >= i0 && i < i0 + PER)
#pragma unroll
                        for (int ct = 0; ct < CTN; ++ct) red[((wave * PER + (i - i0)) * CTN + ct) * 64 + lane] = acc[i][ct];
            }
            __syncthreads();
            if (wset == 0) {
#pragma unroll
                for (int i = 0; i < NKW; ++i)
                    if (i >= i0 && i < i0 + PER)
#pragma unroll
                        for (int ct = 0; ct < CTN; ++ct) acc[i][ct] += red[((wave * PER + (i - i0)) * CTN + ct) * 64 + lane];
            }
        }
        if (wset == 1) return;
    }
#pragma unroll
    for (int i = 0; i < NKW; ++i) {
        const int nkt = wave + 4 * i;
        if (nkt >= NKT) continue;
#pragma unroll
        for (int ct = 0; ct < CTN; ++ct)
#pragma unroll
            for (int j = 0; j < 4; ++j) {
                const int co = ct * 16 + lg * 4 + j;
                if (co < d.Cout) slab[(size_t)co * a.kextc + nkt * 16 + li] = acc[i][ct][j];
            }
    }
}


struct WIn64 {
    static constexpr int PSX = 64 * 2 + 32, PSG = 8 * 2 + 32, TG = 18;
    static constexpr int X_BYTES = 256 * PSX, G_BYTES = TG * TG * PSG;
    static constexpr int ZERO = X_BYTES + G_BYTES;
    static constexpr int TILE_BYTES = ZERO + 64;
    static constexpr int RED_BYTES = 4 * 10 * 1024;
    static constexpr int LDS = TILE_BYTES > RED_BYTES ? TILE_BYTES : RED_BYTES;
};

template <bool IDS>
__global__ __launch_bounds__(256) void wgrad_in64_kernel(const WLeanArgs a) {
    typedef bf16_t T;
    typedef Vec8<T>::type V8;
    constexpr int PSX = WIn64::PSX, PSG = WIn64::PSG, TG = WIn64::TG;
    extern __shared__ __align__(16) unsigned char smem[];
    unsigned char* lds_x = smem;
    unsigned char* lds_g = smem + WIn64::X_BYTES;
    const msau_wgrad_desc& d = a.d;
    const int tid = threadIdx.x, lane = tid & 63;
    const int wave = __builtin_amdgcn_readfirstlane(tid >> 6);
    const int li = lane & 15, lg = lane >> 4;
    const int chunk = blockIdx.y;
    const bool relu_in = d.flags & MSAU_CONV_RELU_IN;
    const int c0 = chunk * 64;
    const bool second = d.C2 != 0 && c0 >= d.C1;
    const char* xsrc = static_cast<const char*>(second ? d.x2 : d.x1);
    const int Cx = second ? d.C2 : d.C1;
    const int cb = (second ? c0 - d.C1 : c0) * 2;
    const int in_px = Cx * 2, in_row = d.Win * in_px;
    const int g_px = d.Cout * 2, g_row = d.Wout * g_px;
    if (tid < 4) reinterpret_cast<unsigned*>(smem + WIn64::ZERO)[tid] = 0u;

    int goff[5];
#pragma unroll
    for (int nt = 0; nt < 5; ++nt) {
        const int grp = li & 3, tap = 2 * nt + (grp >> 1);
        const int ky = tap / 3, kx = tap - ky * 3;
        goff[nt] = tap < 9 ? ((2 - ky) * TG + (2 - kx)) * PSG + (grp & 1) * 8 : WL_ABS | WIn64::ZERO;
    }
    f32x4 acc[4][5];
#pragma unroll
    for (int mt = 0; mt < 4; ++mt)
#pragma unroll
        for (int nt = 0; nt < 5; ++nt) acc[mt][nt] = f32x4{0.f, 0.f, 0.f, 0.f};
    float bsum[2][8];
#pragma unroll
    for (int it = 0; it < 2; ++it)
#pragma unroll
        for (int j = 0; j < 8; ++j) bsum[it][j] = 0.f;

    V8 xr[IDS ? 1 : 8], gr[2];
    int idr = -1;
    auto issue_loads = [&](int tile) {
        const int t1 = a.tiles_x > 1 ? __umulhi((unsigned)tile, a.mag_tx) : tile;
        const int txi = tile - t1 * a.tiles_x;
        const int b = a.tiles_y > 1 ? __umulhi((unsigned)t1, a.mag_ty) : t1;
        const int tyi = t1 - b * a.tiles_y;
        const int iy0 = tyi * 16, ix0 = txi * 16;
        const char* xb = xsrc + (long long)b * d.Hin * in_row + cb;
        if constexpr (IDS) {
            const int iy = iy0 + (tid >> 4), ix = ix0 + (tid & 15);
            idr = -1;
            if (iy < d.Hin && ix < d.Win) idr = static_cast<const int*>(d.x1)[((long long)b * d.Hin + iy) * d.Win + ix];
        } else
#pragma unroll
        for (int it = 0; it < 8; ++it) {
            const int idx = tid + it * 256;
            const int pix = idx >> 3, cg = idx & 7;
            const int iy = iy0 + (pix >> 4), ix = ix0 + (pix & 15);
            xr[it] = zero8<T>();
            if (iy < d.Hin && ix < d.Win) xr[it] = *reinterpret_cast<const V8*>(xb + (unsigned)(iy * in_row + ix * in_px + cg * 16));
        }
        const char* gb = static_cast<const char*>(d.g) + (long long)b * d.Hout * g_row;
        const int gy0 = iy0 + d.pad_t - 2, gx0 = ix0 + d.pad_l - 2;
#pragma unroll
        for (int it = 0; it < 2; ++it) {
            const int m = tid + it * 256;
            const int i = m / TG, j = m - i * TG;
            const int oy = gy0 + i, ox = gx0 + j;
            gr[it] = zero8<T>();
            if (m < TG * TG && (unsigned)oy < (unsigned)d.Hout && (unsigned)ox < (unsigned)d.Wout)
                gr[it] = *reinterpret_cast<const V8*>(gb + (unsigned)(oy * g_row + ox * g_px));
        }
    };
    if ((int)blockIdx.x < a.ntiles) issue_loads(blockIdx.x);

    for (int tile = blockIdx.x; tile < a.ntiles; tile += gridDim.x) {
        __syncthreads();
        if constexpr (IDS) {
#pragma unroll
            for (int cg = 0; cg < 8; ++cg) {
                V8 v;
#pragma unroll
                for (int j = 0; j < 8; ++j) v[j] = (T)(cg * 8 + j == idr ? 1.0f : 0.0f);
                *reinterpret_cast<V8*>(lds_x + tid * PSX + cg * 16) = v;
            }
        } else
#pragma unroll
        for (int it = 0; it < 8; ++it) {
            const int idx = tid + it * 256;
            V8 v = xr[it];
            if (relu_in) v = relu8<T>(v);
            *reinterpret_cast<V8*>(lds_x + (idx >> 3) * PSX + (idx & 7) * 16) = v;
        }
#pragma unroll
        for (int it = 0; it < 2; ++it) {
            const int m = tid + it * 256;
            if (m < TG * TG) {
                *reinterpret_cast<V8*>(lds_g + m * PSG) = gr[it];
                const int i = m / TG, j = m - i * TG;
                if (chunk == 0 && i >= 2 - d.pad_t && i <= 17 - d.pad_t && j >= 2 - d.pad_l && j <= 17 - d.pad_l) {
#pragma unroll
                    for (int e = 0; e < 8; ++e) bsum[it][e] += (float)gr[it][e];
                }
            }
        }
        __syncthreads();
        if (tile + (int)gridDim.x < a.ntiles) issue_loads(tile + gridDim.x);

        const int q = li >> 2, p = li & 3;
#pragma unroll
        for (int bb = 0; bb < 2; ++bb) {
            const int blk = wave * 2 + bb;
            const int row = blk * 2 + (lg >> 1), col = (lg & 1) * 4 + q;
            const unsigned char* xa = lds_x + (row * 16 + col) * PSX + 8 * p;
            bf16x8 afrag[4];
#pragma unroll
            for (int mt = 0; mt < 4; ++mt) {
                bf16x4 lo = __builtin_amdgcn_ds_read_tr16_b64_v4bf16((lds_v4)(xa + mt * 32));
                bf16x4 hi = __builtin_amdgcn_ds_read_tr16_b64_v4bf16((lds_v4)(xa + 8 * PSX + mt * 32));
                afrag[mt] = __builtin_shufflevector(lo, hi, 0, 1, 2, 3, 4, 5, 6, 7);
            }
            const int pb0 = WIn64::X_BYTES + (row * TG + col) * PSG;
#pragma unroll
            for (int nt = 0; nt < 5; ++nt) {
                const int e = goff[nt];
                const bool abs_ok = nt == 4;
                const int o0 = (abs_ok && (e & WL_ABS)) ? (e & ~WL_ABS) : pb0 + e;
                const int o1 = (abs_ok && (e & WL_ABS)) ? (e & ~WL_ABS) : pb0 + 8 * PSG + e;
                bf16x4 lo = __builtin_amdgcn_ds_read_tr16_b64_v4bf16((lds_v4)(smem + o0));
                bf16x4 hi = __builtin_amdgcn_ds_read_tr16_b64_v4bf16((lds_v4)(smem + o1));
                bf16x8 bfrag = __builtin_shufflevector(lo, hi, 0, 1, 2, 3, 4, 5, 6, 7);
#pragma unroll
                for (int mt = 0; mt < 4; ++mt)
                    acc[mt][nt] = __builtin_amdgcn_mfma_f32_16x16x32_bf16(afrag[mt], bfrag, acc[mt][nt], 0, 0, 0);
            }
        }
    }

    float* slab = d.slabs + ((size_t)blockIdx.x * a.nchunks + chunk) * d.Cout * a.kextc;
    f32x4* red = reinterpret_cast<f32x4*>(smem);
#pragma unroll
    for (int half = 0; half < 2; ++half) {
        __syncthreads();
#pragma unroll
        for (int t = 0; t < 10; ++t) {
            const int tt = half * 10 + t;
            red[(wave * 10 + t) * 64 + lane] = acc[tt / 5][tt % 5];
        }
        __syncthreads();
#pragma unroll
        for (int ii = 0; ii < 3; ++ii) {
            const int t = wave + 4 * ii;
            if (t >= 10) continue;
            const int tt = half * 10 + t, mt = tt / 5, nt = tt % 5;
            f32x4 v = red[(0 * 10 + t) * 64 + lane];
#pragma unroll
            for (int w = 1; w < 4; ++w) v += red[(w * 10 + t) * 64 + lane];
            const int tap = 2 * nt + (li >> 3), co = li & 7;
            if (tap < 9 && co < d.Cout) {
#pragma unroll
                for (int j = 0; j < 4; ++j) slab[(size_t)co * a.kextc + tap * 64 + mt * 16 + lg * 4 + j] = v[j];
            }
        }
    }
    __syncthreads();
    float* bred = reinterpret_cast<float*>(smem);
#pragma unroll
    for (int it = 0; it < 2; ++it)
#pragma unroll
        for (int e = 0; e < 8; ++e) bred[(it * 256 + tid) * 8 + e] = bsum[it][e];
    __syncthreads();
    if (tid < 8 && tid < d.Cout) {
        float s = 0.f;
        for (int t = 0; t < 512; ++t) s += bred[t * 8 + tid];
        for (int k = 576; k < a.kextc; ++k) slab[(size_t)tid * a.kextc + k] = k == 576 && chunk == 0 ? s : 0.f;
    }
}

int launch_wgrad_in64(hipStream_t s, const WLeanArgs& a) {
    if (a.kextc != 592) return 0;
    if (a.d.flags & MSAU_CONV_IDS) {
        if (a.nchunks != 1 || a.d.C2) return msau_set_error(MSAU_ERR_ARG, "wgrad: MSAU_CONV_IDS needs one 64-channel one-hot source");
        hipLaunchKernelGGL(wgrad_in64_kernel<true>, dim3(a.d.nslabs, 1), dim3(256), WIn64::LDS, s, a);
    } else
    hipLaunchKernelGGL(wgrad_in64_kernel<false>, dim3(a.d.nslabs, a.nchunks), dim3(256), WIn64::LDS, s, a);
    MSAU_CHECK_LAUNCH("wgrad_in64_kernel");
    return 1;
}

template <typename T, int C8, int CO8, int KS, int DIL = 1, int STRIDE = 1>
int launch_wlean(hipStream_t s, const WLeanMulti& m, int n) {
    using Cfg = WLeanCfg<T, C8, CO8, KS, DIL, STRIDE>;
    const WLeanArgs& a = m.a[0];
    if (Cfg::KEXT != a.kextc) return 0;
    static bool attr_set = false;
    if (!attr_set && Cfg::LDS > 60 * 1024) {
        hipError_t e = hipFuncSetAttribute(reinterpret_cast<const void*>(&wgrad_lean_kernel<T, C8, CO8, KS, DIL, STRIDE>),
                                           hipFuncAttributeMaxDynamicSharedMemorySize, MSAU_LDS_LIMIT);
        if (e != hipSuccess) return msau_set_error(MSAU_ERR_HIP, "wgrad_lean: hipFuncSetAttribute: %s", hipGetErrorString(e));
        attr_set = true;
    }
    hipLaunchKernelGGL((wgrad_lean_kernel<T, C8, CO8, KS, DIL, STRIDE>), dim3(a.d.nslabs, a.nchunks, n), dim3(Cfg::NTH), Cfg::LDS, s, m);
    MSAU_CHECK_LAUNCH("wgrad_lean_kernel");
    return 1;
}

template <typename T, int KS>
int wlean_dispatch(hipStream_t s, const WLeanMulti& m, int n, int c8, int co8) {
#define WL_CASE(C, O) if (c8 == C && co8 == O) return launch_wlean<T, C, O, KS>(s, m, n);
    WL_CASE(1, 1) WL_CASE(1, 2) WL_CASE(2, 1) WL_CASE(2, 2) WL_CASE(2, 4) WL_CASE(4, 2) WL_CASE(4, 4) WL_CASE(8, 1)
    WL_CASE(4, 8) WL_CASE(8, 4) WL_CASE(8, 8)
#undef WL_CASE
    return 0;
}

template <typename T>
int wlean_special(hipStream_t s, const WLeanMulti& m, int n, int c8, int co8, int dil, int stride) {
    if (stride == 2 && dil == 1) {
        if (c8 == 1 && co8 == 2) return launch_wlean<T, 1, 2, 3, 1, 2>(s, m, n);
        if (c8 == 2 && co8 == 4) return launch_wlean<T, 2, 4, 3, 1, 2>(s, m, n);
        if (c8 == 4 && co8 == 8) return launch_wlean<T, 4, 8, 3, 1, 2>(s, m, n);
        return 0;
    }
    if (stride == 1) {
        if (dil == 2 && c8 == 1 && co8 == 2) return launch_wlean<T, 1, 2, 3, 2, 1>(s, m, n);
        if (dil == 4 && c8 == 2 && co8 == 4) return launch_wlean<T, 2, 4, 3, 4, 1>(s, m, n);
        if (dil == 8 && c8 == 4 && co8 == 8) return launch_wlean<T, 4, 8, 3, 8, 1>(s, m, n);
    }
    return 0;
}

static bool wlean_special_shape(int c8, int co8, int dil, int stride) {
    if (stride == 2 && dil == 1) return (c8 == 1 && co8 == 2) || (c8 == 2 && co8 == 4) || (c8 == 4 && co8 == 8);
    if (stride == 1) return (dil == 2 && c8 == 1 && co8 == 2) || (dil == 4 && c8 == 2 && co8 == 4) || (dil == 8 && c8 == 4 && co8 == 8);
    return false;
}

}

static const int kLeanShapes[][2] = {{1, 1}, {1, 2}, {2, 1}, {2, 2}, {2, 4}, {4, 2}, {4, 4}, {8, 1}, {4, 8}, {8, 4}, {8, 8}};

int msau_wgrad_lean_applicable(int dtype, const msau_wgrad_desc* d, int cch) {
    if (d->KH != d->KW || (d->KH != 1 && d->KH != 3 && d->KH != 4)) return 0;
    const bool special = d->stride != 1 || d->dil != 1;
    if (special) {
        if (d->KH != 3 || d->C2 || cch != d->C1 || !wlean_special_shape(cch / 8, d->Cout / 8, d->dil, d->stride)) return 0;
        if (d->pad_t != d->dil || d->pad_l != d->dil) return 0;
    } else {
        if (d->Hin != d->Hout || d->Win != d->Wout || d->pad_t < 0 || d->pad_l < 0 || d->pad_t >= d->KH || d->pad_l >= d->KW) return 0;
    }
    if (d->KH == 4 && !(cch == 8 && d->Cout == 8)) return 0;
    const int esz = dtype == MSAU_F32 ? 4 : 2;
    if ((int64_t)d->Hin * d->Win * (d->C1 > d->C2 ? d->C1 : d->C2) * esz >= (1ll << 31)) return 0;
    if ((int64_t)d->Hout * d->Wout * d->Cout * esz >= (1ll << 31)) return 0;
    const int tx = cdiv(d->Wout, 16), ty = cdiv(d->Hout, 16);
    if ((int64_t)d->B * tx * ty >= (1 << 20) || tx >= 4096 || ty >= 4096) return 0;
    if (special) return 1;
    for (auto& sh : kLeanShapes)
        if (sh[0] == cch / 8 && sh[1] == d->Cout / 8 && cch % 8 == 0) return 1;
    return 0;
}

static void wlean_fill(WLeanArgs& a, const msau_wgrad_desc* d, int nchunks, int kextc) {
    a.d = *d;
    a.kextc = kextc; a.nchunks = nchunks;
    a.tiles_x = cdiv(d->Wout, 16); a.tiles_y = cdiv(d->Hout, 16);
    a.ntiles = d->B * a.tiles_x * a.tiles_y;
    a.mag_tx = (unsigned)((0x100000000ull + a.tiles_x - 1) / a.tiles_x);
    a.mag_ty = (unsigned)((0x100000000ull + a.tiles_y - 1) / a.tiles_y);
}

static bool wlean_in64(int dtype, const msau_wgrad_desc* d, int cch) {
    static const bool in64_off = std::getenv("MSAU_WGRAD_IN64") && std::getenv("MSAU_WGRAD_IN64")[0] == '0';
    return !in64_off && dtype == MSAU_BF16 && d->stride == 1 && d->dil == 1 && d->KH == 3 && cch == 64 && d->Cout == 8 &&
           d->pad_t <= 2 && d->pad_l <= 2;
}

int msau_wgrad_lean_group(hipStream_t s, int dtype, const msau_wgrad_desc* const* ds, int n, int cch, int nchunks, int kextc) {
    const msau_wgrad_desc* d = ds[0];
    if (n < 1 || n > kWGroup || !msau_wgrad_lean_applicable(dtype, d, cch)) return 0;
    WLeanMulti m;
    for (int i = 0; i < n; ++i) wlean_fill(m.a[i], ds[i], nchunks, kextc);
    for (int i = n; i < kWGroup; ++i) m.a[i] = m.a[0];
    if (d->stride != 1 || d->dil != 1)
        return dtype == MSAU_F32 ? wlean_special<float>(s, m, n, cch / 8, d->Cout / 8, d->dil, d->stride)
                                 : wlean_special<bf16_t>(s, m, n, cch / 8, d->Cout / 8, d->dil, d->stride);
    if (wlean_in64(dtype, d, cch)) {
        if (n != 1) return 0;
        return launch_wgrad_in64(s, m.a[0]);
    }
    if (d->KH == 4) return dtype == MSAU_F32 ? launch_wlean<float, 1, 1, 4>(s, m, n) : launch_wlean<bf16_t, 1, 1, 4>(s, m, n);
    if (dtype == MSAU_F32) return d->KH == 3 ? wlean_dispatch<float, 3>(s, m, n, cch / 8, d->Cout / 8) : wlean_dispatch<float, 1>(s, m, n, cch / 8, d->Cout / 8);
    return d->KH == 3 ? wlean_dispatch<bf16_t, 3>(s, m, n, cch / 8, d->Cout / 8) : wlean_dispatch<bf16_t, 1>(s, m, n, cch / 8, d->Cout / 8);
}

int msau_wgrad_lean_try(hipStream_t s, int dtype, const msau_wgrad_desc* d, int cch, int nchunks, int kextc) {
    return msau_wgrad_lean_group(s, dtype, &d, 1, cch, nchunks, kextc);
}

int msau_wgrad_lean_groupable(int dtype, const msau_wgrad_desc* d, int cch) {
    return msau_wgrad_lean_applicable(dtype, d, cch) && !wlean_in64(dtype, d, cch);
}
```

### msau_amd/model.py

```python
from __future__ import annotations

import os
import weakref

import math

import numpy as np
from collections import OrderedDict
from typing import Dict, Optional, Tuple

import torch
import torch.nn as nn

from . import _lib as L
from .plan import Plan

DTYPES = {"fp32": L.F32, "float32": L.F32, "bf16": L.BF16, "bfloat16": L.BF16}


def param_shapes(cfg: dict) -> "OrderedDict[str, Tuple[int, ...]]":
    S, R, Fr = cfg["scale_space_num"], cfg["res_depth"], cfg["featRoot"]
    k, nb = cfg["filter_size"], cfg.get("num_blocks", 3)
    out: "OrderedDict[str, Tuple[int, ...]]" = OrderedDict()

# ... 654 lines not shown
        if eps is not None: self.eps = float(eps)
        if max_norm is not None: self.max_norm = float(max_norm)
        if weight_decay is not None: self.weight_decay = float(weight_decay)
        if alpha is not None: self.alpha = float(alpha)
        if momentum is not None: self.momentum = float(momentum)
        self._invalidate_graphs()

    @classmethod
    def from_opt_kwargs(cls, model: MSAUWrapper, opt_kwargs={}, **engine_kwargs) -> "TrainEngine":
        from .training.optimizer import engine_options
        opt = engine_options(opt_kwargs)
        shown = opt.pop("shown")
        print(f"Optimizer: {shown[0]}")
        print(f"Learning Rate: {shown[1]}")
        return cls(model, **{**opt, **engine_kwargs})

    def _clip(self) -> float:
        return float(self.max_norm) if self.max_norm is not None and self.max_norm > 0 else 0.0

    def _default_step(self) -> bool:
        return self.optimizer == "adam" and self.weight_decay == 0.0 and self._clip() > 0.0

    def _has_norm(self) -> bool:
        return self.optimizer == "adam" or self._clip() > 0.0

    def optim_launches(self):
        nparam = sum(p.numel() for _, p in self.model._named)
        if self._default_step():
            return [("msau_clip_adam_step", nparam * 4 * 8)]
        nbuf = len(OPTIM_BUFFERS[self.optimizer])
        out = [("msau_optim_step<sqsum>", nparam * 4)] if self._has_norm() else []
        return out + [(f"msau_optim_step<{self.optimizer}>", nparam * 4 * (2 + 2 * nbuf + 1))]

    def _init_native_comm(self, group):
        import torch.distributed as dist
        if not self.sync.active or self.use_graph or os.environ.get("MSAU_DP_NATIVE", "0") != "1":
            return
        if not (dist.is_available() and dist.is_initialized()) or dist.get_backend(group) != "nccl":
            return
        if not L.load().msau_comm_available():
            return
        import ctypes as C
        rank, world = dist.get_rank(group), dist.get_world_size(group)
        ident = torch.zeros(128, dtype=torch.uint8, device=self.model._flat.device)
        if rank == 0:
            buf = (C.c_ubyte * 128)()
            L.call("msau_comm_unique_id", buf, 128)
            ident.copy_(torch.tensor(list(buf), dtype=torch.uint8))
        dist.broadcast(ident, src=dist.get_global_rank(group, 0) if group is not None else 0, group=group)
        raw = bytes(ident.cpu().tolist())
        comm = C.c_void_p()
        L.call("msau_comm_init", C.byref(comm), world, rank, raw, 128)
        self._comm = comm.value
        self._comm_stream = L.concurrent_stream(self.model._flat.device, index=1)
        weakref.finalize(self, L.load().msau_comm_destroy, self._comm)

    def _fwd_bwd(self, plan: Plan, x, labels, ids=None, nhwc_ready=False, owner=None, nhwc_clean=False, loss_grads=None):
        plan.forward(self.model._flat, x, export=False, ids=ids, nhwc_ready=nhwc_ready, owner=owner, single_stream=self.use_graph,
                     nhwc_clean=nhwc_clean)
        loss = plan.loss_grads(labels) if loss_grads is None else loss_grads(plan)
        self._ar_native = False
        native = self._comm is not None and self.sync.active and plan.overlap_wgrad and L._profiler is None \
            and len(self.sync.buckets) == len(plan._bwd_segs) + 1
        if native:
            if getattr(plan, "_dp_flat", None) != self.flat_grad.data_ptr() or getattr(plan, "_dp_comm", None) != self._comm:
                plan.set_native_dp(self._comm, self._comm_stream, self.sync.buckets, self.flat_grad)
                plan._dp_comm = self._comm
            plan.backward(self.flat_grad, native_dp=True)
            self._ar_started = False
            self._ar_native = True
        elif self.sync.active and not self.use_graph and os.environ.get("MSAU_DP_BUCKETS", "stage") != "1":
            nb = self.model.num_blocks
            plan.backward(self.flat_grad, on_stage_done=lambda b, side: self.sync.start(nb - b, after=side))
            self._ar_started = True
        else:
            plan.backward(self.flat_grad, single_stream=self.use_graph)
            self._ar_started = False
        return loss

    def _optim(self):
        n = self.model._flat.numel()
        if self._default_step():
            b1, b2 = self.betas
            L.call("msau_clip_adam_step", torch.cuda.current_stream().cuda_stream, self.model._flat.data_ptr(),
                   self.flat_grad.data_ptr(), self.m.data_ptr(), self.v.data_ptr(), self.state.data_ptr(),
                   self.adam_ws.data_ptr(), n, self.lr, b1, b2, self.eps, self.max_norm, 1.0 / self.world)
            return
        if self.optimizer == "adam":
            a, b, (c1, c2) = self.m, self.v.data_ptr(), self.betas
        elif self.optimizer == "rmsprop":
            a, b, c1, c2 = self.square_avg, None, self.alpha, 0.0
        else:
            a, b, c1, c2 = self.momentum_buffer, None, self.momentum, 0.0
        L.call("msau_optim_step", torch.cuda.current_stream().cuda_stream, OPTIMIZERS[self.optimizer], self.model._flat.data_ptr(),
               self.flat_grad.data_ptr(), a.data_ptr(), b, self.state.data_ptr(), self.adam_ws.data_ptr(), n, self.lr, c1, c2,
               self.eps, self.weight_decay, self._clip(), 1.0 / self.world, self._skip_arr, len(self._skip))

    def _allreduce(self):
        if self._ar_native:
            return
        if self.sync.active:
            if self._ar_started:
                self.sync.start(0)
            elif os.environ.get("MSAU_DP_BUCKETS", "stage") == "1":
                self.sync.start_whole()
            else:
                self.sync.start_all()
            self.sync.finish()

    def _step(self, plan: Plan, labels, x=None, **feed) -> torch.Tensor:
        loss = self._fwd_bwd(plan, x, labels, **feed)
        self._allreduce()
        self._optim()
        return loss

    def _eager(self, name: str):
        if self.use_graph:
            raise RuntimeError(f"{name} is an eager path (use_graph=False)")

    def step(self, x: torch.Tensor, labels: torch.Tensor, sizes=None) -> torch.Tensor:
        x = x.contiguous().float()
        labels = labels.reshape(x.shape[0], x.shape[2], x.shape[3]).contiguous().long()
        if sizes is not None:
            sizes = self.model._check_sizes(x, sizes)
        plan = self.model._plan_for(x, training=True, ragged=sizes is not None)
        if not self.use_graph:
            plan.set_extents(sizes)
            return self._step(plan, labels, x)
        _bury_graphs()
        graphs = plan.__dict__.setdefault("_tgraphs", {})
        key = self._token
        cur = torch.cuda.current_stream()
        gs = self._gstream
        gs.wait_stream(cur)
        with torch.cuda.stream(gs):
            plan.set_extents(sizes)
            if key not in graphs:
                sx, sl = x.clone(), labels.clone()
                self._fwd_bwd(plan, sx, sl)
                torch.cuda.synchronize()
                g1 = _keep_graph(torch.cuda.CUDAGraph())
                with _capture_section():
                    with torch.cuda.graph(g1, stream=gs):
                        loss = self._fwd_bwd(plan, sx, sl)
                g2 = _keep_graph(torch.cuda.CUDAGraph())
                with _capture_section():
                    with torch.cuda.graph(g2, stream=gs):
                        self._optim()
                graphs[key] = (g1, g2, loss, sx, sl)
            g1, g2, loss, sx, sl = graphs[key]
            sx.copy_(x, non_blocking=True)
            sl.copy_(labels, non_blocking=True)
            g1.replay()
            self._allreduce()
            g2.replay()
        cur.wait_stream(gs)
        return loss

    def step_ids(self, ids: torch.Tensor, labels: torch.Tensor, sizes=None) -> torch.Tensor:
        self._eager("step_ids")
        ids = self.model._check_ids(ids)
        B, H, W = ids.shape
        sizes = self.model._check_sizes_for(sizes, B, H, W)
        labels = labels.reshape(B, H, W).contiguous().long()
        plan = self.model._plan(B, H, W, ids.device, True, sizes)
        return self._step(plan, labels, ids=ids)

    def _class_weights(self, class_weights, n_class: int) -> Optional[torch.Tensor]:
        return _device_class_weights(self, class_weights, n_class, self.model._flat.device)

    def step_unet(self, ids: torch.Tensor, labels: torch.Tensor, aux_labels: torch.Tensor, sizes=None, class_weights=None,
                  stats=None) -> torch.Tensor:
        self._eager("step_unet")
        cw = self._class_weights(class_weights, self.model.n_class)
        ids = self.model._check_ids(ids)
        B, H, W = ids.shape
        sizes = self.model._check_sizes_for(sizes, B, H, W)
        labels = labels.reshape(B, H, W).contiguous().long()
        plan = self.model._plan(B, H, W, ids.device, True, sizes)
        aux_labels = aux_labels.reshape(B, H, W).contiguous().long() if plan.aux is not None else None
        if stats is None:
            loss_grads = lambda p: p.loss_grads_unet(labels, aux_labels, cw)
        else:
            def loss_grads(p):
                p.eval_unet(labels, aux_labels, cw, out=stats)
                return p.loss_grads_unet(labels, aux_labels, cw)
        return self._step(plan, None, ids=ids, loss_grads=loss_grads)

    def step_kv(self, tables, class_weights=None, round_to: int = 16, stats=None) -> torch.Tensor:
        self._eager("step_kv")
        from .training import kv_data
        ids, labels, aux_labels, sizes = kv_data.paint_train_device(tables, round_to=round_to, device=self.model._flat.device)
        return self.step_unet(ids, labels, aux_labels, sizes=sizes, class_weights=class_weights, stats=stats)

    def input_nhwc(self, B: int, H: int, W: int) -> torch.Tensor:
        return self.model._plan_for_shape(B, H, W, self.model._flat.device, True).input_nhwc

    def step_nhwc(self, grid: torch.Tensor, labels: torch.Tensor) -> torch.Tensor:
        self._eager("step_nhwc")
        B, H, W, Cs = grid.shape
        plan = self.model._plan_for_shape(B, H, W, grid.device, True)
        buf = plan.input_nhwc
        if tuple(grid.shape) != tuple(buf.shape) or grid.dtype != buf.dtype:
            raise ValueError(f"step_nhwc wants {tuple(buf.shape)} {buf.dtype} (channels padded to a multiple of 8), got {tuple(grid.shape)} {grid.dtype}")
        if grid.data_ptr() != buf.data_ptr():
            buf.copy_(grid)
        labels = labels.reshape(B, H, W).contiguous().long()
        return self._step(plan, labels, nhwc_ready=True)

    def step_boxes(self, grid_boxes, label_boxes, B: int, H: int, W: int, feats=None, sizes=None) -> torch.Tensor:
        self._eager("step_boxes")
        m = self.model
        sizes = m._check_sizes_for(sizes, B, H, W)
        plan = m._plan(B, H, W, m._flat.device, True, sizes)
        feed, labels = m._paint_boxes(plan, grid_boxes, label_boxes, feats)
        return self._step(plan, labels, **feed)

    def prefetch_boxes(self, grid_boxes, label_boxes, B: int, H: int, W: int, feats=None, sizes=None):
        self._eager("prefetch_boxes")
        if sizes is not None:
            raise NotImplementedError("prefetch_boxes paints dense batches only: a ragged batch (sizes=...) goes through "
                                      "step_boxes(..., sizes=sizes)")
        plan = self.model._plan_for_shape(B, H, W, self.model._flat.device, True)
        q = self._prefetched
        if len(q) >= 2:
            raise RuntimeError("prefetch_boxes: two batches are already queued (the plan has two input buffers); call "
                               "step_prefetched() before painting another one")
        k = (q[-1][1] + 1) % 2 if q else (self._pf_last + 1) % 2
        buf = plan.input_buffer(k)
        cur = torch.cuda.current_stream()
        if plan._side is None:
            plan._side = L.concurrent_stream(plan.device)
        side = plan._side
        side.wait_stream(cur)
        with torch.cuda.stream(side):
            _, labels = self.model._paint_boxes(plan, grid_boxes, label_boxes, feats, out=buf)
            ev = torch.cuda.Event()
            ev.record(side)
        labels.record_stream(cur)
        q.append((plan, k, labels, ev))

    def step_prefetched(self) -> torch.Tensor:
        plan, k, labels, ev = self._prefetched.pop(0)
        self._pf_last = k
        torch.cuda.current_stream().wait_event(ev)
        plan.use_input(k)
        return self._step(plan, labels, nhwc_ready=True)

    @property
    def grad_norm(self) -> torch.Tensor:
        if not self._has_norm():
            raise RuntimeError(f"grad_norm: {self.optimizer} without clipping (max_norm {self.max_norm}) is one launch that never "
                               f"computes the gradient's norm; build the engine with max_norm > 0 to have it")
        return self.state[1]

    def _buffers(self):
        return {"adam": (self.m, self.v), "rmsprop": (self.square_avg,), "momentum": (self.momentum_buffer,)}[self.optimizer]

    def state_dict(self) -> dict:
        sd = {"engine": 1, "step": int(round(float(self.state[0])))}
        for name, buf in zip(OPTIM_BUFFERS[self.optimizer], self._buffers()):
            sd[name] = buf.detach().clone()
        sd["lr"] = self.lr
        if self.optimizer == "adam":
            sd.update(betas=tuple(self.betas), eps=self.eps, max_norm=self.max_norm if self.max_norm is not None else 0.0,
                      numel=int(self.m.numel()))
            if self.weight_decay != 0.0:
                sd["weight_decay"] = self.weight_decay
            return sd
        sd.update(optimizer=self.optimizer, eps=self.eps, weight_decay=self.weight_decay, max_norm=self._clip(),
                  numel=int(self.flat_grad.numel()))
        sd["alpha" if self.optimizer == "rmsprop" else "momentum"] = self.alpha if self.optimizer == "rmsprop" else self.momentum
        return sd

    def load_state_dict(self, sd: dict):
        bufs = self._buffers()
        if sd.get("engine") == 1:
            have = sd.get("optimizer", "adam")
            if have != self.optimizer:
                raise ValueError(f"optimizer state is {have}'s, the engine runs {self.optimizer}")
            if int(sd["numel"]) != self.flat_grad.numel():
                raise ValueError(f"optimizer state is for {sd['numel']} parameters, the model has {self.flat_grad.numel()}")
            for name, buf in zip(OPTIM_BUFFERS[self.optimizer], bufs):
                buf.copy_(sd[name])
            self.state.zero_()
            self.state[0] = float(sd["step"])
            self.lr, self.eps = float(sd["lr"]), float(sd["eps"])
            if self.optimizer == "adam":
                self.betas = tuple(sd["betas"])
            self.max_norm = float(sd.get("max_norm", self.max_norm))
            self.weight_decay = float(sd.get("weight_decay", 0.0))
            self.alpha, self.momentum = float(sd.get("alpha", self.alpha)), float(sd.get("momentum", self.momentum))
            self._invalidate_graphs()
            return
        named = [(k, p.numel()) for k, p in self.model._named if p.requires_grad]
        step, flats, g0 = torch_optim_state_to_flat(sd, named, self.model._poff, self.flat_grad.numel(), self.optimizer)
        for buf, flat in zip(bufs, flats):
            buf.copy_(flat)
        self.state.zero_()
        self.state[0] = float(step)
        self.lr, self.weight_decay = float(g0["lr"]), float(g0.get("weight_decay", 0.0))
        if self.optimizer == "adam":
            self.betas, self.eps = tuple(g0["betas"]), float(g0["eps"])
        elif self.optimizer == "rmsprop":
            self.alpha, self.eps = float(g0["alpha"]), float(g0["eps"])
        else:
# ... 3 lines not shown
```

### msau_amd/plan.py

```python
from __future__ import annotations

import ctypes as C
import math
import os
from typing import Dict, List, NamedTuple, Optional, Tuple

import torch

from . import _lib as L


def same_pads(in_size: int, k: int, stride: int = 1, dilation: int = 1) -> Tuple[int, int]:
    k_eff = k + (k - 1) * (dilation - 1)
    out = -(-in_size // stride)
    pad = max((out - 1) * stride + k_eff - in_size, 0)
    return pad // 2, pad - pad // 2


def _ru(a: int, b: int) -> int:
    return -(-a // b) * b


def _launch_info(dtype: int, d) -> "C.Array":
    info = (L.i32 * 8)()
    L.call("msau_conv2d_launch_info", dtype, C.byref(d), info)
    return info


def _ptr(t: Optional[torch.Tensor]) -> Optional[int]:
    return None if t is None else t.data_ptr()


class Launch(NamedTuple):
    kind: int
    args: Optional[C.Structure]
    key: str
    nbytes: float
    flops: float = 0.0


class Act:

    def __init__(self, plan: "Plan", name: str, H: int, W: int, C: int, relu_out: bool = False,
                 needs_grad: bool = True):
        self.plan, self.name, self.H, self.W, self.C = plan, name, H, W, C
        self.Cs = _ru(C, 8)
        self.relu_out = relu_out
        self.needs_grad = needs_grad and plan.training
        self.data = None if plan.reuse else torch.zeros((plan.B, H, W, self.Cs), dtype=plan.tdtype, device=plan.device)
        self.grad: Optional[torch.Tensor] = None
        self.n_contrib = 0
        plan.acts.append(self)

    @property
    def npix(self) -> int:
        return self.plan.B * self.H * self.W

    def register(self) -> int:
        k = self.n_contrib
        self.n_contrib += 1
        return k

    def slot_flags(self, k: int) -> Tuple[bool, bool]:
        return k != self.n_contrib - 1, (k == 0 and self.relu_out)

    def alloc_grad(self):
        if self.needs_grad and self.n_contrib > 0 and self.grad is None:
            self.grad = torch.zeros_like(self.data)


class Op:
    name = "op"

    def reads(self) -> List["Act"]:
        return []

    def writes(self) -> List["Act"]:
        return []

    def finalize(self):
        pass

    def fwd_recs(self) -> List[Launch]:
        raise NotImplementedError

    def bwd_recs(self) -> List[Launch]:
        return []


class ConvOp(Op):

    def __init__(self, plan: "Plan", name: str, x1: Act, x2: Optional[Act], wname: str, bname: str, out: Act,
                 k: int, dil: int = 1, relu_in: bool = False, relu_out: bool = False,
                 fwd_add: Optional[Act] = None, kind: str = "conv", head: bool = False):
        self.plan, self.name, self.x1, self.x2, self.out = plan, name, x1, x2, out
        self.head = head
        self.wname, self.bname, self.k, self.dil, self.kind = wname, bname, k, dil, kind
        self.relu_in, self.relu_out, self.fwd_add = relu_in, relu_out, fwd_add
        self.bwd_add: Optional[Act] = None
        self.pair: Optional["PairOp"] = None
        self.cpl: Optional["ConvOp"] = None
        self.cpl_fused_into: Optional["PairOp"] = None
        self.proj: Optional["ProjBwd"] = None
        self.dgrad2 = None
        self.dgrad_in_pair: Optional["PairOp"] = None
        if kind == "conv" and k == 1 and x2 is not None and relu_out and not relu_in and fwd_add is None and plan.ops:
            prod = plan.ops[-1]
            if isinstance(prod, ConvOp) and prod.out is x2 and prod.pair is not None and prod is prod.pair.c2 \
                    and x1.Cs == x2.Cs == out.Cs == x2.C == out.C:
                prod.cpl = self
        assert out.relu_out == relu_out
        if kind == "conv":
            assert out.H == x1.H and out.W == x1.W
            self.pad_t = same_pads(x1.H, k, 1, dil)[0]
            self.pad_l = same_pads(x1.W, k, 1, dil)[0]
        else:
            assert x2 is None and dil == 1 and not relu_in
            p = k // 2
            for o, i in ((out.H, x1.H), (out.W, x1.W)):
                op = o - ((i - 1) * 2 - 2 * p + k)
                assert 0 <= op < 2, f"{name}: output size {o} unreachable from {i}"
            self.pad_t = self.pad_l = k - 1 - p
        self.slots = []
        for x in (x1, x2):
            self.slots.append(x.register() if (x is not None and x.needs_grad) else None)
        self.stage = plan._cur_stage
        plan.ops.append(self)

    def reduce_group(self):
        return -1 if (self.stage == 0 and self.name.startswith("s0.d0.")) else self.stage

    def reads(self):
        return [t for t in (self.x1, self.x2, self.fwd_add) if t is not None]

    def writes(self):
        lrn, pool = getattr(self, "lrn", None), getattr(self, "pool", None)
        w = [self.out] + ([lrn.y] if lrn is not None else []) + ([pool.y] if pool is not None else [])
        if self.cpl is not None:
            w += [t for t in self.cpl.writes() if t not in w]
        return w

    def _geom(self, C1, C2, Cout, dil, stride, ups):
        g = L.ConvPackGeom()
        L.call("msau_conv_pack_geometry", self.plan.dtype, C1, C2, Cout, self.k, self.k, dil, stride, ups, C.byref(g))
        return g

    def _pack_entry(self, g, off, row_is_dim0, flip, row_off, rows_real, k1, k2):
        shp = self.plan.pshape[self.wname]
        e = L.PackEntry()
        e.src_off = self.plan.poff[self.wname]
        e.dst_off = off
        e.kind, e.dim0, e.dim1, e.KH, e.KW = 0, shp[0], shp[1], self.k, self.k
        e.row_is_dim0, e.flip, e.row_off, e.rows_real, e.rows_pad = int(row_is_dim0), int(flip), row_off, rows_real, g.rows
        e.k1_real, e.k1_store = k1
        e.k2_real, e.k2_store = k2
        e.cch, e.nchunks, e.kchunk, e.dtype = g.cch, g.nchunks, g.kchunk, self.plan.dtype
        return e, g.nchunks * g.rows * g.kchunk

    def finalize(self):
        P = self.plan
        x1, x2, out = self.x1, self.x2, self.out
        C2s = x2.Cs if x2 is not None else 0
        C2r = x2.C if x2 is not None else 0
        conv = self.kind == "conv"
        g = self._geom(x1.Cs, C2s, out.Cs, self.dil, 1, 1 if conv else 2)
        self.w_off = P.alloc_pack(g.bytes)
        e, n = self._pack_entry(g, self.w_off, row_is_dim0=conv, flip=not conv, row_off=0, rows_real=out.C,
                                k1=(x1.C, x1.Cs), k2=(C2r, C2s))
        P.add_pack_entry(e, n)
        self.b_off = P.alloc_pack(out.Cs * 4)
        be = L.PackEntry()
        be.src_off, be.dst_off, be.kind = P.poff[self.bname], self.b_off, 1
        be.row_off, be.rows_real, be.rows_pad = 0, out.C, out.Cs
        P.add_pack_entry(be, out.Cs)
        self.d_off = [None, None]
        self.wg_fused = False
        self.uentry = None
        self.dd_off = None
        if P.training and conv and x2 is not None and None not in self.slots and x1.C == x1.Cs == x2.C == x2.Cs \
                and x1.Cs + x2.Cs <= 128 and os.environ.get("MSAU_FUSE_DGRAD", "1") != "0" and not P.generic_only:
            proto = L.ConvDesc()
            proto.B, proto.Hin, proto.Win, proto.Hout, proto.Wout = P.B, out.H, out.W, x1.H, x1.W
            proto.C1, proto.C2, proto.Cout = out.Cs, 0, x1.Cs + x2.Cs
            proto.KH = proto.KW = self.k
            proto.dil, proto.stride, proto.ups = self.dil, 1, 1
            proto.pad_t = (self.k - 1) * self.dil - self.pad_t
            proto.pad_l = (self.k - 1) * self.dil - self.pad_l
            info = _launch_info(P.dtype, proto)
            if info[7] & 2:
                gd = self._geom(out.Cs, 0, x1.Cs + x2.Cs, self.dil, 1, 1)
                self.dd_off = P.alloc_pack(gd.bytes)
                e, n = self._pack_entry(gd, self.dd_off, row_is_dim0=False, flip=True, row_off=0,
                                        rows_real=x1.C + x2.C, k1=(out.C, out.Cs), k2=(0, 0))
                P.add_pack_entry(e, n)
        self.dcp_off = self.dd_off
        if P.training and conv and self.k == 1 and x2 is not None and self.dd_off is None and None not in self.slots \
                and x1.C == x1.Cs == x2.C == x2.Cs == out.Cs == 32 and P.dtype == L.BF16 and not P.generic_only \
                and any(pr.c2.cpl is self for pr in P.pairs):
            gd = self._geom(out.Cs, 0, x1.Cs + x2.Cs, self.dil, 1, 1)
            self.dcp_off = P.alloc_pack(gd.bytes)
            e, n = self._pack_entry(gd, self.dcp_off, row_is_dim0=False, flip=True, row_off=0,
                                    rows_real=x1.C + x2.C, k1=(out.C, out.Cs), k2=(0, 0))
            P.add_pack_entry(e, n)
        if P.training and self.dd_off is None:
            for si, x in enumerate((x1, x2)):
                if x is None or self.slots[si] is None:
                    continue
                if conv:
                    gd = self._geom(out.Cs, 0, x.Cs, self.dil, 1, 1)
                    self.d_off[si] = P.alloc_pack(gd.bytes)
                    e, n = self._pack_entry(gd, self.d_off[si], row_is_dim0=False, flip=True,
                                            row_off=(0 if si == 0 else x1.C), rows_real=x.C,
                                            k1=(out.C, out.Cs), k2=(0, 0))
                else:
                    gd = self._geom(out.Cs, 0, x.Cs, 1, 2, 1)
                    self.d_off[si] = P.alloc_pack(gd.bytes)
                    e, n = self._pack_entry(gd, self.d_off[si], row_is_dim0=True, flip=False, row_off=0,
                                            rows_real=x.C, k1=(out.C, out.Cs), k2=(0, 0))
                P.add_pack_entry(e, n)

    def bind(self):
# ... 576 lines not shown
        if not bwd:
            return f"pool_fwd<{T},C{x.Cs}>", (nx + ny) * esz + (ny if P.training else 0)
        accum, maskb = x.slot_flags(self.slot)
        return f"pool_bwd<{T},C{x.Cs}>", (ny + nx * (1 + int(accum) + int(maskb))) * esz + ny

    def fwd_recs(self):
        x, y = self.x, self.y
        if self.fused_into is not None:
            return []
        self._fa = L.PoolArgs(_ptr(x.data), _ptr(y.data), _ptr(self.idx), None, self.plan.B, x.H, x.W, x.Cs, 0, None)
        return [Launch(L.OP_POOL_FWD, self._fa, *self._meta(False))]

    def bwd_recs(self):
        x, y = self.x, self.y
        if y.grad is None or x.grad is None:
            return []
        accum, maskb = x.slot_flags(self.slot)
        self._ba = L.PoolArgs(_ptr(y.grad), _ptr(x.grad), _ptr(self.idx), _ptr(x.data) if maskb else None,
                              self.plan.B, x.H, x.W, x.Cs, int(accum) | (2 if maskb and self.plan.act_flag else 0),
                              self.plan.extent_ptr(x))
        return [Launch(L.OP_POOL_BWD, self._ba, *self._meta(True))]


class AttnCoreOp(Op):

    def __init__(self, plan, name, f: Act, g: Act, h: Act, x: Act, y: Act):
        self.plan, self.name, self.f, self.g, self.h, self.x, self.y = plan, name, f, g, h, x, y
        self.N = x.H * x.W
        self.stats = torch.zeros((plan.B, self.N, 2), dtype=torch.float32, device=plan.device)
        self.ws = torch.zeros((plan.B, self.N), dtype=torch.float32, device=plan.device)
        for t in (f, g, h):
            t.register()
        self.stage = plan._cur_stage
        plan.ops.append(self)

    def reads(self):
        return [self.f, self.g, self.h, self.x]

    def writes(self):
        return [self.y]

    def _args(self, bwd):
        return L.AttnArgs(_ptr(self.f.data), _ptr(self.g.data), _ptr(self.h.data),
                          _ptr(self.y.grad) if bwd else _ptr(self.x.data), _ptr(self.y.data), _ptr(self.stats),
                          _ptr(self.f.grad), _ptr(self.g.grad), _ptr(self.h.grad), _ptr(self.ws),
                          self.plan.B, self.N, self.f.Cs, self.h.Cs, self.plan.extent_ptr(self.x), self.x.W)

    def _meta(self, bwd: bool) -> Tuple[str, float, float]:
        P = self.plan
        esz = 4 if P.dtype == L.F32 else 2
        T = "f32" if P.dtype == L.F32 else "bf16"
        npx = P.B * self.N
        small, big = npx * self.f.Cs * esz, npx * self.h.Cs * esz
        ffl = 2.0 * P.B * self.N * self.N * (self.f.C + self.h.C)
        if not bwd:
            return f"selfattn_fwd<{T}>", 2 * small + 3 * big, ffl
        return f"selfattn_bwd<{T}>", 4 * small + 4 * big, 2.0 * ffl

    def fwd_recs(self):
        self._fa = self._args(False)
        return [Launch(L.OP_ATTN_FWD, self._fa, *self._meta(False))]

    def bwd_recs(self):
        if self.y.grad is None:
            return []
        self._ba = self._args(True)
        return [Launch(L.OP_ATTN_BWD, self._ba, *self._meta(True))]


class ProjBwd:

    def __init__(self, plan: "Plan", f: ConvOp, g: ConvOp, h: ConvOp):
        self.plan, self.f, self.g, self.h = plan, f, g, h
        self.active = False
        self.args = None
        for c in (f, g, h):
            c.proj = self
        plan.projs.append(self)

    def bind(self):
        P, f, g, h = self.plan, self.f, self.g, self.h
        x = f.x1
        df, dg, dh = f.ddesc[0], g.ddesc[0], h.ddesc[0]
        if P.dtype != L.BF16 or P.generic_only or os.environ.get("MSAU_ATTN_PROJ_FUSE", "1") == "0" or None in (df, dg, dh):
            return
        if not (x.C == x.Cs == 64 and f.out.Cs == g.out.Cs == 8 and h.out.Cs == 64 and f.k == g.k == h.k == 1
                and g.x1 is x and h.x1 is x and f.x2 is None and g.x2 is None and h.x2 is None
                and f.dd_off is None and not (f.relu_in or g.relu_in or h.relu_in)):
            return
        A, M, D = L.CONV_ACCUM, L.CONV_MASK_B, L.CONV_ADD
        if (dh.flags & ~(A | D)) or dg.flags != A or (df.flags & ~M) != A:
            return
        for c, kch in ((f, 32), (g, 32), (h, 64)):
            gd = c._geom(c.out.Cs, 0, x.Cs, 1, 1, 1)
            if (gd.nchunks, gd.rows, gd.kchunk) != (1, 64, kch):
                return
        a = L.AttnProjBwdArgs()
        a.df, a.dg, a.dh = _ptr(f.out.grad), _ptr(g.out.grad), _ptr(h.out.grad)
        a.wf_pack, a.wg_pack, a.wh_pack = (P.pack_ptr(c.d_off[0]) for c in (f, g, h))
        a.add = dh.add if dh.flags & D else None
        a.mask_b = df.mask_b if df.flags & M else None
        a.dx, a.npix, a.C, a.accumulate = _ptr(x.grad), x.npix, x.Cs, int(bool(dh.flags & A))
        self.args, self.active = a, True

    def recs(self):
        x, outs = self.f.x1, (self.f.out, self.g.out, self.h.out)
        nops = 1 + (1 if self.args.add else 0) + self.args.accumulate + (1 if self.args.mask_b else 0)
        nbytes = x.npix * (sum(o.Cs for o in outs) + nops * x.Cs) * 2
        return [Launch(L.OP_ATTN_PROJ_BWD, self.args, "attn_proj_bwd<bf16,C64>", nbytes, 2.0 * x.npix * x.C * sum(o.C for o in outs))]


class Plan:
    def __init__(self, cfg: dict, B: int, H: int, W: int, dtype: int, device, poff: Dict[str, int],
                 pshape: Dict[str, Tuple[int, ...]], training: bool = True, builder=None, ragged: bool = False):
        self.cfg, self.B, self.H, self.W, self.dtype, self.device = cfg, B, H, W, dtype, device
        self.tdtype = torch.float32 if dtype == L.F32 else torch.bfloat16
        self.poff, self.pshape, self.training = poff, pshape, training
        self.reuse = (not training) and bool(cfg.get("reuse_activations", True))
        assert cfg.get("activation", "relu") in ("relu", "elu"), cfg.get("activation")
        self.act_flag = L.CONV_ELU if cfg.get("activation", "relu") == "elu" else 0
        self.ragged = bool(ragged)
        self.extent_flag = L.CONV_EXTENT if self.ragged else 0
        self.levels = [(-(-H // 2 ** l), -(-W // 2 ** l)) for l in range(max(1, int(cfg.get("scale_space_num", 1))))]
        self.extents = torch.ones((len(self.levels), B, 2), dtype=torch.int32, device=device) if self.ragged else None
        self._ext_host = None
        self.generic_only = bool(self.act_flag) or self.ragged
        self.head_probs = self.head_argmax = None
        self.head_fused = False
        self.acts: List[Act] = []
        self.ops: List[Op] = []
        self.pairs: List[PairOp] = []
        self.projs: List[ProjBwd] = []
        self.box_ops: List["BoxOp"] = []
        self.box_scratch = 0
        self.box_ws_ii = 0
        self.box_ws = None
        self.box_ii_g = None
        self._box_bwd_args: list = []
        self._pack_bytes = 0
        self._slab_elems = 0
        self._pack_entries: List[L.PackEntry] = []
        self._unpack_entries: List[L.UnpackEntry] = []
        self._unpack_stage: List[int] = []
        self._pack_max = 1
        self._unpack_max = 1
        self.launch_meta: Dict[str, Tuple[int, float, float]] = {}
        self.rec_meta: Dict[int, Tuple[str, float]] = {}
        self._cur_stage = 0
        self.overlap_wgrad = bool(cfg.get("overlap_wgrad", os.environ.get("MSAU_OVERLAP_WGRAD", "1") != "0")) and \
            str(device).startswith("cuda")
        self._side = None
        self.deterministic = bool(cfg.get("deterministic", os.environ.get("MSAU_DETERMINISTIC", "0") == "1"))
        self.overlap_max_pix = int(cfg.get("overlap_max_pix", 1 << 62))
        self.x_in = Act(self, "input", H, W, cfg["channels"], needs_grad=bool(cfg.get("input_grad", False)))
        self.logits: Optional[Act] = None
        self.aux: Optional[Act] = None
        if builder is None:
            self._build_net()
        else:
            builder(self)
        self._finish()

    def extent_ptr(self, a: Act) -> Optional[int]:
        if not self.ragged:
            return None
        lv = self.levels.index((a.H, a.W))
        return self.extents.data_ptr() + lv * self.B * 2 * 4

    @staticmethod
    def level_extents(sizes: torch.Tensor, levels: int) -> torch.Tensor:
        s = sizes.to(torch.int64)
        return torch.stack([-((-s) // (2 ** l)) for l in range(levels)]).to(torch.int32).contiguous()

    @staticmethod
    def check_sizes(sizes, B: int, H: int, W: int) -> torch.Tensor:
        if not isinstance(sizes, torch.Tensor):
            sizes = torch.as_tensor(sizes)
        if sizes.device.type != "cpu" or sizes.dtype.is_floating_point or sizes.dtype == torch.bool:
            raise ValueError(f"sizes must be a CPU integer tensor [B, 2] of (h, w), got {sizes.dtype} on {sizes.device}")
        if tuple(sizes.shape) != (B, 2):
            raise ValueError(f"sizes must have shape ({B}, 2) for this batch, got {tuple(sizes.shape)}")
        h, w = sizes[:, 0], sizes[:, 1]
        if bool((h < 1).any() or (w < 1).any() or (h > H).any() or (w > W).any()):
            raise ValueError(f"sizes must satisfy 1 <= h <= {H} and 1 <= w <= {W} (the canvas), got {sizes.tolist()}")
        return sizes

    def set_extents(self, sizes) -> None:
        if not self.ragged:
            assert sizes is None, "sizes on a dense plan"
            return
        host = self.level_extents(self.check_sizes(sizes, self.B, self.H, self.W), len(self.levels))
        if str(self.device).startswith("cuda"):
            host = host.pin_memory()
        self._ext_host = host
        self.extents.copy_(host, non_blocking=True)

    def _zero_outside(self, src: torch.Tensor, dst: torch.Tensor, planes: int, H: int, W: int, pixel_bytes: int, level: int = 0):
        L.call("msau_extent_copy", self._stream(), src.data_ptr(), dst.data_ptr(), self.B, planes, H, W, pixel_bytes,
               self.extents.data_ptr() + level * self.B * 2 * 4)

    def alloc_pack(self, nbytes: int) -> int:
        off = self._pack_bytes
        self._pack_bytes += _ru(int(nbytes), 256)
        return off

    def alloc_slab(self, nelems: int) -> int:
        off = self._slab_elems
        self._slab_elems += _ru(int(nelems), 64)
        return off

    def add_pack_entry(self, e, nelems):
        self._pack_entries.append(e)
        self._pack_max = max(self._pack_max, int(nelems))

    def add_unpack_entry(self, e, nelems, stage=0):
        self._unpack_entries.append(e)
        self._unpack_stage.append(stage)
        self._unpack_max = max(self._unpack_max, int(nelems))

    def pack_ptr(self, off: int) -> int:
        return self.pack_arena.data_ptr() + off

    def slab_ptr(self, off: int) -> int:
        return self.slab_arena.data_ptr() + 4 * off

    def _res_block(self, x0: Act, prefix: str, tag: str) -> Act:
        R, k = self.cfg["res_depth"], self.cfg["filter_size"]
        r_in, first = x0, None
        for i in range(R):
            o = Act(self, f"{tag}.res{i}", x0.H, x0.W, x0.C, relu_out=True)
            op = ConvOp(self, f"{tag}.res{i}", r_in, None, f"{prefix}.conv_res_list.{i}.custom_conv.weight",
                        f"{prefix}.conv_res_list.{i}.custom_conv.bias", o, k, relu_in=(i == 0), relu_out=True,
                        fwd_add=(x0 if i == R - 1 else None))
            first = first or op
            r_in = o
        first.bwd_add = r_in
        if R == 2:
            PairOp(self, first, op)
        return r_in

    def _box_block(self, x0: Act, prefix: str, tag: str) -> Act:
        n, Fn = self.cfg["num_box_convs"], self.cfg["num_box_per_channels"]
        r_in, first = x0, None
        for i in range(n):
            bx = Act(self, f"{tag}.box{i}", x0.H, x0.W, x0.C * Fn)
            bop = BoxOp(self, f"{tag}.box{i}", r_in, bx, f"{prefix}.conv_list.{2 * i}", relu_in=(i == 0))
            first = first or bop
            o = Act(self, f"{tag}.bres{i}", x0.H, x0.W, x0.C, relu_out=True)
            ConvOp(self, f"{tag}.bres{i}", bx, None, f"{prefix}.conv_list.{2 * i + 1}.custom_conv.weight",
                   f"{prefix}.conv_list.{2 * i + 1}.custom_conv.bias", o, 1, relu_out=True, fwd_add=(x0 if i == n - 1 else None))
            r_in = o
        first.bwd_add = r_in
        return r_in

    def _build_net(self):
        cfg = self.cfg
        box = cfg.get("variant") == "box"
        block = (lambda x0, pre, tag: self._box_block(x0, pre.replace(".conv_res_list.", ".conv_box_list."), tag)) if box else self._res_block
        S, Fr, k, nb = cfg["scale_space_num"], cfg["featRoot"], cfg["filter_size"], cfg.get("num_blocks", 3)
        ncls = cfg["n_class"]
        assert cfg["pool_size"] == 2
        inp = self.x_in
        prev_dw = prev_up = None
        self.stage_logits: List[Act] = []
        for b in range(nb):
            self._cur_stage = b
            coupled, last = b > 0, b == nb - 1
            pd = f"msau_net.blocks.{b}.downsamplingblock"
            pu = f"msau_net.blocks.{b}.upsamplingblock"
            dw: Dict[int, Act] = {}
            x_in = inp
            x2 = None
            for l in range(S):
                c = Fr * 2 ** l
                t = f"s{b}.d{l}"
                a = Act(self, t + ".a", x_in.H, x_in.W, c)
                ConvOp(self, t + ".dil", x_in, None, f"{pd}.conv1s.{l}.conv.weight", f"{pd}.conv1s.{l}.conv.bias", a, k,
                       dil=2 ** l)
                x0 = Act(self, t + ".lrn", a.H, a.W, c)
                LrnOp(self, t + ".lrn", a, x0)
                x1 = block(x0, f"{pd}.conv_res_list.{l}", t)
                if coupled:
                    x2 = Act(self, t + ".cpl", a.H, a.W, c, relu_out=True)
                    ConvOp(self, t + ".cpl", prev_dw[l], x1, f"{pd}.conv1_1s.{l}.custom_conv.weight",
                           f"{pd}.conv1_1s.{l}.custom_conv.bias", x2, 1, relu_out=True)
                else:
                    x2 = x1
                if l == S - 1 and not last:
                    pa = f"{pd}.layer_attentions.attention_block"
                    fa = Act(self, t + ".f", a.H, a.W, c // 8)
                    ga = Act(self, t + ".g", a.H, a.W, c // 8)
                    ha = Act(self, t + ".h", a.H, a.W, c)
                    fop = ConvOp(self, t + ".f", x2, None, f"{pa}.f.conv.weight", f"{pa}.f.conv.bias", fa, 1)
                    gop = ConvOp(self, t + ".g", x2, None, f"{pa}.g.conv.weight", f"{pa}.g.conv.bias", ga, 1)
                    hop = ConvOp(self, t + ".h", x2, None, f"{pa}.h.conv.weight", f"{pa}.h.conv.bias", ha, 1)
                    if self.training:
                        ProjBwd(self, fop, gop, hop)
                    y = Act(self, t + ".attn", a.H, a.W, c)
                    AttnCoreOp(self, t + ".attn", fa, ga, ha, x2, y)
                    hop.bwd_add = y
                    dw[l] = y
                else:
                    dw[l] = x2
                if l < S - 1:
                    pooled = Act(self, t + ".pool", (x2.H + 1) // 2, (x2.W + 1) // 2, c, relu_out=False)
                    PoolOp(self, t + ".pool", x2, pooled)
                    x_in = pooled
# ... 35 lines not shown
                    self.ext_slot[t.name] = t.register()
        if self.reuse:
            self._assign_buffers()
        if not self.training and self.logits.C <= 255:
            lg = self.logits
            self.head_probs = torch.zeros((self.B, lg.H, lg.W, lg.C), dtype=torch.float32, device=self.device)
            self.head_argmax = torch.zeros((self.B, lg.H, lg.W), dtype=torch.uint8, device=self.device)
        for a in self.acts:
            a.alloc_grad()
        for op in self.ops:
            op.finalize()
        if self.box_ops:
            self.box_ii_g = torch.zeros((max(self.box_scratch, 1),), dtype=torch.float32, device=self.device)
            self.box_ws = torch.zeros((max(self.box_ws_ii, 1),), dtype=torch.float32, device=self.device)
        self.pack_arena = torch.zeros(max(self._pack_bytes, 256), dtype=torch.uint8, device=self.device)
        for op in self.ops:
            if isinstance(op, ConvOp):
                op.bind()
        for pr in self.pairs:
            pr.bind()
        for pj in self.projs:
            pj.bind()
        self.slab_arena = torch.zeros(max(self._slab_elems, 64), dtype=torch.float32, device=self.device)
        for op in self.ops:
            if isinstance(op, ConvOp):
                op.late_bind()
        for pr in self.pairs:
            pr.late_bind()
        boundary = self._boundary_launches()
        side_ops, join_ops = set(), set()
        if self.training and self.overlap_wgrad and os.environ.get("MSAU_ATTN_SIDE", "1") != "0":
            for op in self.ops:
                if isinstance(op, AttnCoreOp):
                    branch = [c for c in self.ops if isinstance(c, ConvOp) and c.out in (op.f, op.g, op.h)]
                    users = [c for c in self.ops if c is not op and any(t is op.y for t in c.reads())]
                    later = self.ops[self.ops.index(op) + 1:]
                    first = min(users, key=self.ops.index) if users else None
                    if len(branch) == 3 and users and all(u in later for u in users) and \
                            isinstance(first, ConvOp) and first.fwd_recs() and \
                            not any(t in (op.f, op.g, op.h) for o2 in later for t in o2.reads()):
                        side_ops.update(id(c) for c in branch)
                        side_ops.add(id(op))
                        join_ops.add(id(first))
        frecs = []
        for op in self.ops:
            for r in op.fwd_recs():
                if id(op) in side_ops:
                    r = r._replace(kind=r.kind | L.OP_SIDE)
                elif id(op) in join_ops:
                    r = r._replace(kind=r.kind | L.OP_JOIN)
                    join_ops.discard(id(op))
                frecs.append(r)
        assert not join_ops, "a side-stream attention branch lost its join: its first reader emitted no launch record"
        self._fwd_side = bool(side_ops)

        self._fwd_seq = self._make_seq(frecs)
        self.pack_table = self._upload(self._pack_entries, L.PackEntry) if self._pack_entries else None
        self.unpack_table = self._upload(self._unpack_entries, L.UnpackEntry) if self._unpack_entries else None
        self._bwd_seq, self._bwd_segs, self._reduce_args = None, [], []
        if self.training:
            recs = []
            stages = sorted({op.stage for op in self.ops}, reverse=True)
            esz = C.sizeof(L.UnpackEntry)
            slabs = [e.nslabs * e.slab_elems for e in self._unpack_entries]

            def reduce_rec(group):
                idx = [i for i, st in enumerate(self._unpack_stage) if st == group]
                if not idx:
                    return
                assert idx == list(range(idx[0], idx[-1] + 1)), "unpack entries of a group must be contiguous"
                ra = L.ReduceArgs(self.slab_arena.data_ptr(), None, self.unpack_table.data_ptr() + idx[0] * esz,
                                  len(idx), self._unpack_max)
                self._reduce_args.append(ra)
                recs.append(Launch(L.OP_WGRAD_REDUCE | (L.OP_SIDE if self.overlap_wgrad else 0), ra, "msau_wgrad_reduce",
                                   self.reduce_bytes * sum(slabs[i] for i in idx) / sum(slabs)))

            for b in stages:
                start = len(recs)
                ops_b = [op for op in reversed(self.ops) if op.stage == b]
                cut = next((i for i, op in enumerate(ops_b) if isinstance(op, ConvOp) and op.reduce_group() != b), len(ops_b))
                assert all(not isinstance(op, ConvOp) or op.reduce_group() != b for op in ops_b[cut:]), \
                    "separately reduced convs must close their stage's backward"
                recs += [r for op in ops_b[:cut] for r in op.bwd_recs()]
                reduce_rec(b)
                if cut < len(ops_b):
                    recs += [r for op in ops_b[cut:] for r in op.bwd_recs()]
                    reduce_rec(-1)
                self._bwd_segs.append((b, start, len(recs) - start))
            self._bwd_seq = self._make_seq(recs)
        for r in frecs + (recs if self.training else []) + boundary:
            n, nbytes, flops = self.launch_meta.get(r.key, (0, 0.0, 0.0))
            self.launch_meta[r.key] = (n + 1, nbytes + r.nbytes, flops + r.flops)
        HW = self.H * self.W
        lg = self.logits
        self.out_logits = torch.zeros((self.B, lg.C, lg.H, lg.W), dtype=torch.float32, device=self.device)
        self.out_aux = torch.zeros((self.B, self.aux.C, self.aux.H, self.aux.W), dtype=torch.float32,
                                   device=self.device) if self.aux is not None else None
        if self.training:
            self.counts_k = max(1, min(16, 256 // self.B)) if self.B <= 1024 and os.environ.get("MSAU_LABEL_SPLIT", "1") != "0" else 1
            self.counts = torch.zeros((self.B * self.counts_k,), dtype=torch.int32, device=self.device)
            self.ce_ws = torch.zeros((int(L.load().msau_ce_ws_floats(self.B * HW)),), dtype=torch.float32, device=self.device)
            self.ce_multi_ws = torch.zeros((int(L.load().msau_ce_multi_ws_floats(self.B * HW)),), dtype=torch.float32, device=self.device)
            self.loss_buf = torch.zeros((1,), dtype=torch.float32, device=self.device)

    def _assign_buffers(self):
        last_read: Dict[int, int] = {}
        for i, op in enumerate(self.ops):
            for t in op.reads():
                last_read[id(t)] = i
        keep = {id(t) for t in getattr(self, "stage_logits", [])} | {id(t) for t in (self.logits, self.aux) if t is not None}
        free: Dict[int, List[torch.Tensor]] = {}
        self.buffers: List[torch.Tensor] = []

        def take(a: Act):
            n = self.B * a.H * a.W * a.Cs
            pool = free.setdefault(n, [])
            if pool:
                buf = pool.pop()
            else:
                buf = torch.zeros((n,), dtype=self.tdtype, device=self.device)
                self.buffers.append(buf)
            a.data = buf.view(self.B, a.H, a.W, a.Cs)
            a._buf = buf

        def release(a: Act):
            if id(a) not in keep and a.data is not None:
                keep.add(id(a))
                free[a._buf.numel()].append(a._buf)

        take(self.x_in)
        for i, op in enumerate(self.ops):
            for t in op.writes():
                if t.data is None:
                    take(t)
            for t in set(op.reads()) | set(op.writes()):
                if last_read.get(id(t), -1) <= i and (t in op.reads() or id(t) not in last_read):
                    release(t)
        for a in self.acts:
            if a.data is None:
                take(a)

    def _boundary_launches(self) -> List[Launch]:
        esz = 4 if self.dtype == L.F32 else 2
        a = self.x_in
        api_bytes = self.B * a.C * a.H * a.W * 4
        out = []
        c = self._nchw_first_conv()
        if c is None:
            out.append(Launch(0, None, "msau_nchw_to_nhwc", api_bytes + a.npix * a.Cs * esz))
        else:
            T = "f32" if self.dtype == L.F32 else "bf16"
            c.fkey = f"first_conv_nchw<{T},CIN{a.Cs},CO{c.out.Cs}>"
            c.fbytes = api_bytes + (a.npix * a.Cs * esz if self.training else 0) + c.out.npix * c.out.Cs * esz
        nparam = sum(int(math.prod(shp)) for shp in self.pshape.values())
        out.append(Launch(0, None, "msau_pack_params", nparam * 4 + self._pack_bytes))
        if self.training:
            HW = self.H * self.W
            lg = self.logits
            nl = 2 if self.aux is not None else 1
            out.append(Launch(0, None, "msau_label_counts", self.B * HW * 8))
            out.append(Launch(0, None, "msau_masked_ce_multi" if lg.Cs <= 16 else "msau_masked_ce", self.B * HW * (8 + nl * 2 * lg.Cs * esz)))
            self.reduce_bytes = self._slab_elems * 4 + nparam * 4
            out.append(Launch(0, None, "msau_clip_adam_step", nparam * 4 * 8))
        return out

    def set_probe_keys(self, keys, side: bool = False) -> List[Tuple[str, float]]:
        order = []
        for seq in (self._fwd_seq, self._bwd_seq):
            if seq is None:
                continue
            arr, cnt, _ = seq
            for i in range(cnt):
                meta = self.rec_meta.get(arr[i].args)
                if keys is not None and meta is not None and meta[0] in keys and bool(arr[i].kind & L.OP_SIDE) == side:
                    arr[i].kind |= L.OP_PROBE
                    order.append(meta)
                else:
                    arr[i].kind &= ~L.OP_PROBE
        return order

    @staticmethod
    def read_probe(cap: int = 1 << 16):
        buf = (C.c_float * cap)()
        n = C.c_int(0)
        L.call("msau_probe_read", buf, cap, C.byref(n))
        return list(buf[:n.value])

    def _make_seq(self, recs: List[Launch]):
        arr = (L.Op * max(len(recs), 1))()
        for i, r in enumerate(recs):
            arr[i].kind, arr[i].dtype, arr[i].args = r.kind, self.dtype, C.addressof(r.args)
            self.rec_meta[arr[i].args] = (r.key, r.nbytes)
        return arr, len(recs), recs

    def _run_seq(self, seq, s):
        arr, n, recs = seq
        if L._profiler is None:
            L.call("msau_run_ops", s, arr, n)
            return
        for i in range(n):
            L.call("msau_run_ops", s, C.cast(C.byref(arr, i * C.sizeof(L.Op)), C.POINTER(L.Op)), 1, key=recs[i].key)

    def _one_stream(self, single_stream: bool) -> bool:
        return single_stream or L._profiler is not None or \
            (str(self.device).startswith("cuda") and torch.cuda.is_current_stream_capturing())

    def _upload(self, entries, ctype):
        n = len(entries)
        arr = (ctype * n)(*entries)
        raw = bytes(memoryview(arr))
        host = torch.frombuffer(bytearray(raw), dtype=torch.uint8)
        return host.to(self.device)

    @staticmethod
    def _stream() -> int:
        return torch.cuda.current_stream().cuda_stream

    def pack(self, flat_params: torch.Tensor):
        if self.pack_table is None:
            return
        L.call("msau_pack_params", self._stream(), flat_params.data_ptr(), self.pack_arena.data_ptr(),
               self.pack_table.data_ptr(), len(self._pack_entries), self._pack_max)
        for bop in self.box_ops:
            bop.load_params(self._stream(), flat_params)

    def load_input(self, x_nchw: torch.Tensor):
        assert x_nchw.dtype == torch.float32 and x_nchw.is_contiguous() and tuple(x_nchw.shape) == \
            (self.B, self.cfg["channels"], self.H, self.W), (x_nchw.shape, x_nchw.dtype)
        a = self.x_in
        L.call("msau_nchw_to_nhwc", self._stream(), self.dtype, x_nchw.data_ptr(), a.data.data_ptr(), self.B, a.C, a.Cs, self.H, self.W)
        if self.ragged:
            self._zero_outside(a.data, a.data, 1, self.H, self.W, a.data.element_size() * a.Cs)

    def _nchw_first_conv(self):
        if not hasattr(self, "_nchw_conv"):
            c = next((op for op in self.ops if isinstance(op, ConvOp) and op.x1 is self.x_in and op.x2 is None), None)
            ok = c is not None and os.environ.get("MSAU_FIRST_NCHW", "1") != "0" and not (c.pair is not None and c.pair.active) \
                and not (c.fdesc.flags & ~L.CONV_RELU_OUT)
            if ok:
                info = _launch_info(self.dtype, c.fdesc)
                ok = bool(info[7] & 64)
            self._nchw_conv = c if ok else None
            self._nchw_on = False
        return self._nchw_conv

    def _feed_nchw(self, x_nchw: Optional[torch.Tensor]) -> bool:
        c = self._nchw_first_conv()
        if c is None:
            return False
        if x_nchw is not None:
            assert x_nchw.dtype == torch.float32 and x_nchw.is_contiguous() and tuple(x_nchw.shape) == \
                (self.B, self.cfg["channels"], self.H, self.W), (x_nchw.shape, x_nchw.dtype)
            if x_nchw.data_ptr() % 16:
                x_nchw = None
        if x_nchw is not None:
            c.fdesc.flags |= L.CONV_NCHW
            c.fdesc.x1 = x_nchw.data_ptr()
            c.fdesc.y2 = _ptr(self.x_in.data) if self.training else None
            c.fdesc.head_classes = self.x_in.C
            self._nchw_on = True
            return True
        if self._nchw_on:
            c.fdesc.flags &= ~L.CONV_NCHW
            c.fdesc.x1 = _ptr(self.x_in.data)
            c.fdesc.y2 = None
            c.fdesc.head_classes = 0
            self._nchw_on = False
        return False

    def _feed_ids(self, ids: Optional[torch.Tensor]) -> bool:
        self._feed_nchw(None)
        if not hasattr(self, "_ids_conv"):
            c = next((op for op in self.ops if isinstance(op, ConvOp) and op.x1 is self.x_in and op.x2 is None), None)
            ok = c is not None and os.environ.get("MSAU_IDS_DIRECT", "1") != "0" and not (c.pair is not None and c.pair.active)
            if ok:
                probe = L.ConvDesc.from_buffer_copy(c.fdesc)
                probe.flags |= L.CONV_IDS
                info = _launch_info(self.dtype, probe)
                ok = bool(info[7] & 16)
            if ok and self.training and c.wdesc is not None:
                ok = self.dtype == L.BF16 and c.wgeom.lean and c.wdesc.C1 == 64 and c.wdesc.Cout == 8 and c.wgeom.nchunks == 1
            self._ids_conv = c if ok else None
            self._ids_keep = None
        c = self._ids_conv
        if c is None:
            return False
        if ids is not None:
            c.fdesc.flags |= L.CONV_IDS
            c.fdesc.x1 = ids.data_ptr()
            if c.wdesc is not None:
                c.wdesc.flags |= L.CONV_IDS
                c.wdesc.x1 = ids.data_ptr()
            self._ids_keep = ids
        else:
            c.fdesc.flags &= ~L.CONV_IDS
            c.fdesc.x1 = _ptr(self.x_in.data)
            if c.wdesc is not None:
                c.wdesc.flags &= ~L.CONV_IDS
                c.wdesc.x1 = _ptr(self.x_in.data)
            self._ids_keep = None
        return True

    def _feed_owner(self, src, flat_params: Optional[torch.Tensor] = None) -> bool:
        self._feed_nchw(None)
        if not hasattr(self, "_owner_conv"):
            c = next((op for op in self.ops if isinstance(op, ConvOp) and op.x1 is self.x_in and op.x2 is None), None)
            ok = c is not None and os.environ.get("MSAU_OWNER_CONV", "1") != "0" and not (c.pair is not None and c.pair.active) \
                and not (c.fdesc.flags & ~(L.CONV_RELU_OUT | L.CONV_EXTENT))
            if ok:
                info = _launch_info(self.dtype, c.fdesc)
                ok = bool(info[7] & 32)
                if ok and self.ragged:
                    probe = L.ConvDesc.from_buffer_copy(c.fdesc)
                    probe.flags |= L.CONV_OWNER
                    info = _launch_info(self.dtype, probe)
                    ok = bool(info[7] & 128)
            if ok and self.training and c.wdesc is not None:
                ok = c.wdesc.flags == 0 and c.uentry is not None and c.kind == "conv"
            self._owner_conv = c if ok else None
            self._owner_keep = None
            self._owner_slabs = None
        c = self._owner_conv
        if c is None:
            return False
        if src is None:
            if self._owner_keep is not None:
                c.fdesc.flags &= ~L.CONV_OWNER
                c.fdesc.x1 = _ptr(self.x_in.data)
                if c.wdesc is not None:
                    c.wdesc.flags &= ~(L.CONV_OWNER | L.CONV_EXTENT)
                    c.wdesc.x1 = _ptr(self.x_in.data)
                    self._set_unpack_slabs(c, c.wdesc.nslabs)
                self._owner_keep = None
            return True
        owner, boxes, n_boxes, feats = src
        assert owner.dtype == torch.int32 and owner.is_contiguous() and tuple(owner.shape) == (self.B, self.H, self.W)
        assert feats.dtype == torch.float32 and feats.is_contiguous() and feats.dim() == 2 and int(feats.shape[1]) == self.x_in.C, feats.shape
        self._feed_ids(None)
        n_vec = int(feats.shape[0])
        ctx = L.OwnerCtx()
        blocks = max(1, min(256, c.out.npix // 1024))
        wt = torch.empty((_ru(self.x_in.C, 32) * 72,), dtype=torch.float32, device=self.device)
        table = torch.empty((max(n_vec, 1) * 72,), dtype=torch.float32, device=self.device)
        sums = torch.empty((max(n_boxes, 1) * 72,), dtype=torch.float32, device=self.device)
        csum = torch.empty((blocks * 8,), dtype=torch.float32, device=self.device)
        ctx.owner, ctx.boxes, ctx.feats = owner.data_ptr(), (boxes.data_ptr() if n_boxes else None), feats.data_ptr()
        ctx.w = flat_params.data_ptr() + 4 * self.poff[c.wname]
        ctx.wt, ctx.table, ctx.sums, ctx.csum = wt.data_ptr(), table.data_ptr(), sums.data_ptr(), csum.data_ptr()
        ctx.n_boxes, ctx.n_vec, ctx.C, ctx.csum_blocks, ctx.wt_floats = n_boxes, n_vec, self.x_in.C, blocks, wt.numel()
        c.fdesc.flags |= L.CONV_OWNER
        c.fdesc.x1 = C.addressof(ctx)
        if c.wdesc is not None:
            c.wdesc.flags |= L.CONV_OWNER | self.extent_flag
            c.wdesc.x1 = C.addressof(ctx)
            self._set_unpack_slabs(c, int(L.load().msau_owner_slabs(C.byref(c.wdesc))))
        self._owner_keep = (ctx, owner, boxes, feats, wt, table, sums, csum, flat_params)
        return True

    def _set_unpack_slabs(self, c: "ConvOp", n: int):
        if self._owner_slabs == n or self.unpack_table is None:
            return
        idx = next(i for i, e in enumerate(self._unpack_entries) if e is c.uentry)
        off = idx * C.sizeof(L.UnpackEntry) + L.UnpackEntry.nslabs.offset
        self.unpack_table[off:off + 4].copy_(torch.tensor([n], dtype=torch.int32).view(torch.uint8))
        self._owner_slabs = n

    def load_ids(self, ids: torch.Tensor):
        assert ids.dtype == torch.int32 and ids.is_contiguous() and tuple(ids.shape) == (self.B, self.H, self.W), (ids.shape, ids.dtype)
        a = self.x_in
        if self.ragged:
            L.call("msau_onehot_ids_ext", self._stream(), self.dtype, ids.data_ptr(), a.data.data_ptr(), self.B, self.H, self.W,
                   a.C, a.Cs, self.extents.data_ptr())
            return
        L.call("msau_onehot_ids", self._stream(), self.dtype, ids.data_ptr(), a.data.data_ptr(), a.npix, a.C, a.Cs)

    def _feed(self, flat_params: torch.Tensor, x_nchw: Optional[torch.Tensor], ids: Optional[torch.Tensor] = None, owner=None,
              nhwc_ready: bool = False, nhwc_clean: bool = False):
        if owner is not None:
            assert x_nchw is None and ids is None and not nhwc_ready
            ok = self._feed_owner(owner, flat_params)
            assert ok, "no MSAU_CONV_OWNER instance for this plan's first conv"
            return
        if getattr(self, "_owner_keep", None) is not None:
            self._feed_owner(None)
        if nhwc_ready:
            assert x_nchw is None and ids is None
            self._feed_ids(None)
            if self.ragged and not nhwc_clean:
                a = self.x_in
                self._zero_outside(a.data, a.data, 1, self.H, self.W, a.data.element_size() * a.Cs)
        elif ids is not None:
            assert ids.dtype == torch.int32 and ids.is_contiguous() and tuple(ids.shape) == (self.B, self.H, self.W), (ids.shape, ids.dtype)
            if not self._feed_ids(ids):
                self.load_ids(ids)
        else:
            self._feed_ids(None)
            if not self._feed_nchw(x_nchw):
                self.load_input(x_nchw)

    def predict(self, flat_params: torch.Tensor, x_nchw: Optional[torch.Tensor] = None, ids: Optional[torch.Tensor] = None):
        assert not self.training and self.head_probs is not None
        s = self._stream()
        self.pack(flat_params)
        self._feed(flat_params, x_nchw, ids)
        self._run_seq(self._fwd_seq, s)
        if not self.head_fused:
            lg = self.logits
            L.call("msau_softmax_argmax_nhwc", s, self.dtype, lg.data.data_ptr(), self.head_probs.data_ptr(),
                   self.head_argmax.data_ptr(), lg.npix, lg.C, lg.Cs)
        return self.head_probs, self.head_argmax

    def input_buffer(self, k: int) -> torch.Tensor:
        if not hasattr(self, "_x_bufs"):
            self._x_bufs = [self.x_in.data, None]
        if self._x_bufs[k] is None:
            self._x_bufs[k] = torch.zeros_like(self.x_in.data)
        return self._x_bufs[k]

    def use_input(self, k: int):
        buf = self.input_buffer(k)
        if buf is self.x_in.data:
            return
        self._feed_ids(None)
        old = self.x_in.data.data_ptr()
        for op in self.ops:
            if isinstance(op, ConvOp):
                for d in (op.fdesc, op.wdesc):
                    if d is not None:
                        for f in ("x1", "x2"):
                            if getattr(d, f) == old:
                                setattr(d, f, buf.data_ptr())
        self.x_in.data = buf

    @property
    def input_nhwc(self) -> torch.Tensor:
        return self.x_in.data

    def forward(self, flat_params: torch.Tensor, x_nchw: Optional[torch.Tensor], export: bool = True,
                ids: Optional[torch.Tensor] = None, nhwc_ready: bool = False, owner=None, single_stream: bool = False,
                nhwc_clean: bool = False):
        s = self._stream()
        self.pack(flat_params)
        self._feed(flat_params, x_nchw, ids, owner, nhwc_ready, nhwc_clean)
        if self._fwd_side and not self._one_stream(single_stream):
            if self._side is None:
                self._side = L.concurrent_stream(self.device)
            L.call("msau_run_ops_overlap", s, self._side.cuda_stream, self._fwd_seq[0], self._fwd_seq[1], 1)
        else:
            self._run_seq(self._fwd_seq, s)
        if export:
            self.export_logits()
        return self.out_logits, self.out_aux

    def export_logits(self):
        s = self._stream()
        for act, dst in ((self.logits, self.out_logits), (self.aux, self.out_aux)):
            if act is not None:
                L.call("msau_nhwc_to_nchw", s, self.dtype, act.data.data_ptr(), dst.data_ptr(), self.B, act.C, act.Cs, act.H, act.W)

    def set_external_grads(self, g_logits: Optional[torch.Tensor], g_aux: Optional[torch.Tensor]):
        s = self._stream()
        for act, g in ((self.logits, g_logits), (self.aux, g_aux)):
            if act is None:
                continue
            accum, maskb = act.slot_flags(self.ext_slot[act.name])
            assert not accum
            if g is None:
                act.grad.zero_()
            else:
                g = g.contiguous().float()
                L.call("msau_nchw_grad_to_nhwc", s, self.dtype, g.data_ptr(), act.grad.data_ptr(), self.B, act.C, act.Cs,
                       act.H, act.W, 0)
                if self.ragged:
                    self._zero_outside(act.grad, act.grad, 1, act.H, act.W, act.grad.element_size() * act.Cs)
                if maskb:
                    act.grad.mul_(act.data > 0)

    def loss_grads(self, labels: torch.Tensor) -> torch.Tensor:
        assert labels.dtype == torch.int64 and labels.is_contiguous() and tuple(labels.shape) == (self.B, self.H, self.W)
        s = self._stream()
        HW = self.H * self.W
        if self.ragged:
            if getattr(self, "_labels_buf", None) is None:
                self._labels_buf = torch.zeros_like(labels)
            self._zero_outside(labels, self._labels_buf, 1, self.H, self.W, 8)
            labels = self._labels_buf
        lg, ax = self.logits, self.aux
        if lg.Cs <= 16 and self.B * HW < (1 << 31) and (ax is None or (ax.C, ax.Cs) == (lg.C, lg.Cs)) \
                and os.environ.get("MSAU_CE_MULTI", "1") != "0":
            K = self.counts_k
            if K > 1:
                L.call("msau_label_counts_split", s, labels.data_ptr(), self.counts.data_ptr(), self.B, HW, K, key="msau_label_counts")
            else:
                L.call("msau_label_counts", s, labels.data_ptr(), self.counts.data_ptr(), self.B, HW)
            L.call("msau_masked_ce_multi", s, self.dtype, lg.data.data_ptr(), _ptr(ax.data) if ax is not None else None,
                   labels.data_ptr(), self.counts.data_ptr(), lg.grad.data_ptr(), _ptr(ax.grad) if ax is not None else None,
                   self.loss_buf.data_ptr(), self.ce_multi_ws.data_ptr(), self.B, HW, lg.C, lg.Cs, 1.0 / self.B, K)
            return self.loss_buf
        L.call("msau_label_counts", s, labels.data_ptr(), self.counts.data_ptr(), self.B, HW)
        self.loss_buf.zero_()
        for act in (self.logits, self.aux):
            if act is None:
                continue
            L.call("msau_masked_ce", s, self.dtype, act.data.data_ptr(), labels.data_ptr(), self.counts.data_ptr(),
                   act.grad.data_ptr(), self.loss_buf.data_ptr(), self.ce_ws.data_ptr(), self.B, HW, act.C, act.Cs,
                   1.0 / self.B)
        return self.loss_buf

    def unet_launches(self, weighted: bool) -> List[Launch]:
        esz = 4 if self.dtype == L.F32 else 2
        HW, lg = self.H * self.W, self.logits
        nl = 2 if self.aux is not None else 1
        out = [Launch(0, None, "msau_label_hist", self.B * HW * 8)] * (nl if weighted else 0)
        out.append(Launch(0, None, "msau_unet_ce", self.B * HW * nl * (8 + 2 * lg.Cs * esz)))
        return out

    def loss_grads_unet(self, labels: torch.Tensor, aux_labels: Optional[torch.Tensor], class_w: Optional[torch.Tensor] = None) -> torch.Tensor:
        lg, ax = self.logits, self.aux
        for t in (labels,) + ((aux_labels,) if ax is not None else ()):
            assert t is not None and t.dtype == torch.int64 and t.is_contiguous() and tuple(t.shape) == (self.B, self.H, self.W)
        assert ax is None or (ax.C, ax.Cs, ax.H, ax.W) == (lg.C, lg.Cs, lg.H, lg.W), "the auxiliary head must have the final head's shape"
        assert (lg.H, lg.W) == (self.H, self.W)
        s = self._stream()
        if getattr(self, "unet_loss_buf", None) is None:
            self.unet_loss_buf = torch.zeros((3,), dtype=torch.float32, device=self.device)
            self.unet_ws = torch.zeros((int(L.load().msau_unet_ce_ws_floats(self.B * self.H * self.W)),), dtype=torch.float32, device=self.device)
            self.unet_hist_k = max(1, min(16, 256 // self.B))
            self.unet_hist = None
        ext = self.extents.data_ptr() if self.ragged else None
        K, hist = self.unet_hist_k, None
        if class_w is not None:
            assert class_w.dtype == torch.float32 and class_w.is_contiguous() and class_w.numel() == lg.C and class_w.device == lg.data.device
            if self.unet_hist is None:
                self.unet_hist = torch.zeros((2, self.B, K, lg.C), dtype=torch.int32, device=self.device)
            hist = self.unet_hist.data_ptr()
            for t, lab in enumerate((labels, aux_labels) if ax is not None else (labels,)):
                L.call("msau_label_hist", s, lab.data_ptr(), ext, hist + 4 * t * self.B * K * lg.C, self.B, self.H, self.W, lg.C, K)
        L.call("msau_unet_ce", s, self.dtype, lg.data.data_ptr(), _ptr(ax.data) if ax is not None else None, labels.data_ptr(),
               aux_labels.data_ptr() if ax is not None else None, ext, _ptr(class_w), hist, K, lg.grad.data_ptr(),
               _ptr(ax.grad) if ax is not None else None, self.unet_loss_buf.data_ptr(), self.unet_ws.data_ptr(),
               self.B, self.H, self.W, lg.C, lg.Cs)
        return self.unet_loss_buf

    def unet_eval_launches(self) -> List[Launch]:
        esz = 4 if self.dtype == L.F32 else 2
        nl = 2 if self.aux is not None else 1
        return [Launch(0, None, "msau_unet_eval", self.B * self.H * self.W * nl * (8 + self.logits.Cs * esz))]

    def unet_eval_k(self) -> int:
        if getattr(self, "_cu_count", None) is None:
            self._cu_count = int(torch.cuda.get_device_properties(self.device).multi_processor_count)
        rows = int(self._ext_host[0, :, 0].min()) if self.ragged else self.H
        return max(1, min(256, rows, -(-2 * self._cu_count // self.B)))

    def eval_unet(self, labels: torch.Tensor, aux_labels: Optional[torch.Tensor], class_w: Optional[torch.Tensor] = None, out=None):
        lg, ax = self.logits, self.aux
        for t in (labels,) + ((aux_labels,) if ax is not None else ()):
            assert t is not None and t.dtype == torch.int64 and t.is_contiguous() and tuple(t.shape) == (self.B, self.H, self.W)
        assert ax is None or (ax.C, ax.Cs, ax.H, ax.W) == (lg.C, lg.Cs, lg.H, lg.W), "the auxiliary head must have the final head's shape"
        assert (lg.H, lg.W) == (self.H, self.W)
        if class_w is not None:
            assert class_w.dtype == torch.float32 and class_w.is_contiguous() and class_w.numel() == lg.C and class_w.device == lg.data.device
        if out is None:
            out = (torch.empty((self.B, 2), dtype=torch.float32, device=self.device),
                   torch.empty((self.B, 2, 2), dtype=torch.int32, device=self.device))
        doc_loss, doc_counts = out
        assert doc_loss.dtype == torch.float32 and doc_loss.is_contiguous() and tuple(doc_loss.shape) == (self.B, 2) \
            and doc_counts.dtype == torch.int32 and doc_counts.is_contiguous() and tuple(doc_counts.shape) == (self.B, 2, 2) \
            and doc_loss.device == doc_counts.device == lg.data.device, "stats: (fp32 [B, 2], int32 [B, 2, 2]) on the model's device"
        K = self.unet_eval_k()
        if getattr(self, "unet_eval_ws", None) is None:
            self.unet_eval_ws = torch.zeros((int(L.load().msau_unet_eval_ws_bytes(self.B, 256)),), dtype=torch.uint8, device=self.device)
        L.call("msau_unet_eval", self._stream(), self.dtype, lg.data.data_ptr(), _ptr(ax.data) if ax is not None else None,
               labels.data_ptr(), aux_labels.data_ptr() if ax is not None else None, self.extents.data_ptr() if self.ragged else None,
               _ptr(class_w), K, doc_loss.data_ptr(), doc_counts.data_ptr(), self.unet_eval_ws.data_ptr(), self.B, self.H, self.W,
               lg.C, lg.Cs)
        return doc_loss, doc_counts
# ... 68 lines not shown
```

Baseline: 5728 tiles/s.

## Compress one-hot first-conv input into per-pixel-group codes instead of dense NHWC copy

The fused NCHW first conv now emits a compact 32-bit code per 8-channel group. The code records empty, a single nonzero channel with its bf16 value, or dense. A dense NHWC store happens only for groups with more than one nonzero. The first-layer weight-gradient kernel reads these codes instead of the 64-channel bf16 input copy, which cuts write and read traffic for one-hot chargrid inputs. A lazy codes_to_nhwc expansion rebuilds the dense input when other code reads it, adding bookkeeping and a risk of stale data if a consumer bypasses the accessor.

```diff
diff --git a/include/msau_hip.h b/include/msau_hip.h
--- a/include/msau_hip.h
+++ b/include/msau_hip.h
@@ -37,6 +37,7 @@
     MSAU_CONV_OWNER    = 2048,
     MSAU_CONV_NCHW     = 4096,
     MSAU_CONV_WGRAD    = 8192,
+    MSAU_CONV_CODES    = 16384,
     MSAU_CONV_ELU      = 32768,
     MSAU_CONV_EXTENT   = 65536,
     MSAU_CONV_HEAD     = 64
@@ -59,7 +60,10 @@
     const void* mask_a;
     const void* mask_b;
     void* y;
-    float* head_probs;
+    union {
+        float* head_probs;
+        uint32_t* codes;
+    };
     uint8_t* head_argmax;
     int32_t head_classes;
     int32_t flags2;
@@ -89,6 +93,8 @@
                             int stride, int ups, msau_conv_pack_geom* out);
 int msau_conv2d(void* stream, int dtype, const msau_conv_desc* d);
 int msau_conv2d_launch_info(int dtype, const msau_conv_desc* d, int32_t* info8);
+int msau_firstconv_takes_codes(int dtype, const msau_conv_desc* d);
+int msau_codes_to_nhwc(void* stream, int dtype, const uint32_t* codes, void* nhwc, int64_t npix);
 
 enum { MSAU_PAIR_RELU_IN = 1, MSAU_PAIR_RELU_MID = 2, MSAU_PAIR_MASK_MID = 4,
        MSAU_PAIR_LRN_BWD = 16,
@@ -146,7 +152,10 @@
     int32_t KH, KW, dil, pad_t, pad_l, stride;
     int32_t flags;
     const void* x1;
-    const void* x2;
+    union {
+        const void* x2;
+        const uint32_t* codes;
+    };
     const void* g;
     float* slabs;
     int32_t nslabs;
diff --git a/msau_amd/_lib.py b/msau_amd/_lib.py
--- a/msau_amd/_lib.py
+++ b/msau_amd/_lib.py
@@ -12,6 +12,7 @@
 CONV_RELU_IN, CONV_RELU_OUT, CONV_ADD, CONV_ACCUM, CONV_MASK_A, CONV_MASK_B, CONV_HEAD, CONV_DOUT = 1, 2, 4, 8, 16, 32, 64, 128
 CONV_LRN, CONV_POOL, CONV_IDS, CONV_OWNER, CONV_NCHW, CONV_WGRAD, CONV_ELU = 256, 512, 1024, 2048, 4096, 8192, 32768
 CONV_EXTENT = 65536
+CONV_CODES = 16384
 
 i32, i64, vp, f32 = C.c_int32, C.c_int64, C.c_void_p, C.c_float
 
@@ -23,6 +24,7 @@
                [("head_classes", i32), ("flags2", i32), ("y2", vp), ("mask_b2", vp)] + \
                [("lrn_alpha_over_n", f32), ("lrn_beta", f32), ("lrn_k", f32), ("reserved0", i32), ("pool_y", vp), ("pool_idx", vp)] + \
                [("wg_x1", vp), ("wg_slabs", vp), ("wg_nslabs", i32), ("reserved1", i32), ("extent", vp)]
+    codes = property(lambda self: self.head_probs, lambda self, v: setattr(self, "head_probs", v))
 
 
 class ConvPairDesc(C.Structure):
@@ -52,6 +54,7 @@
     _fields_ = [(n, i32) for n in ("B", "Hin", "Win", "Hout", "Wout", "C1", "C2", "Cout", "KH", "KW", "dil",
                                    "pad_t", "pad_l", "stride", "flags")] + \
                [(n, vp) for n in ("x1", "x2", "g", "slabs")] + [("nslabs", i32)]
+    codes = property(lambda self: self.x2, lambda self, v: setattr(self, "x2", v))
 
 
 class WgradGeom(C.Structure):
@@ -144,6 +147,8 @@
     "msau_attn_proj_bwd": (C.c_int, [vp, C.c_int, C.POINTER(AttnProjBwdArgs)]),
     "msau_dgrad2_1x1": (C.c_int, [vp, C.c_int, C.POINTER(Dgrad2Args)]),
     "msau_conv2d_launch_info": (C.c_int, [C.c_int, C.POINTER(ConvDesc), C.POINTER(i32)]),
+    "msau_firstconv_takes_codes": (C.c_int, [C.c_int, C.POINTER(ConvDesc)]),
+    "msau_codes_to_nhwc": (C.c_int, [vp, C.c_int, vp, vp, i64]),
     "msau_conv_pair_applicable": (C.c_int, [C.c_int, C.POINTER(ConvPairDesc)]),
     "msau_conv_pair": (C.c_int, [vp, C.c_int, C.POINTER(ConvPairDesc)]),
     "msau_conv_pair_bits_bytes": (C.c_int64, [C.c_int, C.POINTER(ConvPairDesc)]),
diff --git a/msau_amd/csrc/conv.hip b/msau_amd/csrc/conv.hip
--- a/msau_amd/csrc/conv.hip
+++ b/msau_amd/csrc/conv.hip
@@ -337,7 +337,7 @@
 
 enum { CONV_TILE = 0, CONV_LEAN = 1, CONV_CHUNKED = 2, CONV_ROWS = 3,
        CONV_OWNER = 4, CONV_FIRST_NCHW = 5, CONV_REFUSED = 6 };
-constexpr int kRefusalOrder[] = {MSAU_CONV_EXTENT, MSAU_CONV_WGRAD, MSAU_CONV_OWNER, MSAU_CONV_NCHW, MSAU_CONV_HEAD, MSAU_CONV_DOUT,
+constexpr int kRefusalOrder[] = {MSAU_CONV_EXTENT, MSAU_CONV_WGRAD, MSAU_CONV_OWNER, MSAU_CONV_NCHW, MSAU_CONV_CODES, MSAU_CONV_HEAD, MSAU_CONV_DOUT,
                                  MSAU_CONV_LRN, MSAU_CONV_IDS, MSAU_CONV_POOL};
 constexpr int kOnlyOthers = MSAU_CONV_WGRAD | MSAU_CONV_OWNER | MSAU_CONV_NCHW | MSAU_CONV_HEAD | MSAU_CONV_DOUT | MSAU_CONV_LRN |
                             MSAU_CONV_IDS | MSAU_CONV_POOL;
@@ -358,6 +358,7 @@
         if (asked(CONV_OWNER) && msau_ownerconv_takes(dtype, d)) { r->family = CONV_OWNER; r->inst = 1; return 0; }
     } else if (f & MSAU_CONV_NCHW) {
         if (asked(CONV_FIRST_NCHW) && msau_firstconv_takes(dtype, d)) { r->family = CONV_FIRST_NCHW; r->inst = 1; return 0; }
+    } else if (f & MSAU_CONV_CODES) {
     } else if (!rc) {
         const ConvGeom& g = r->g;
         if (g.nslices > 1) r->inst = 0;
@@ -384,6 +385,8 @@
             return msau_set_error(MSAU_ERR_ARG, "conv2d: MSAU_CONV_OWNER is the 3x3 stride-1 C -> 8 conv, no other flag but RELU_OUT and EXTENT");
         case MSAU_CONV_NCHW:
             return msau_set_error(MSAU_ERR_ARG, "conv2d: MSAU_CONV_NCHW is the bf16 3x3 64 -> 8 conv (W %% 4 == 0, W <= 288), head_classes = real input channels");
+        case MSAU_CONV_CODES:
+            return msau_set_error(MSAU_ERR_ARG, "conv2d: MSAU_CONV_CODES is valid only together with MSAU_CONV_NCHW (msau_firstconv_takes_codes)");
         case MSAU_CONV_HEAD:
             return msau_set_error(MSAU_ERR_ARG, "conv2d: MSAU_CONV_HEAD is not implemented for this launch (see "
                                   "msau_conv2d_launch_info info[7]); run msau_softmax_argmax_nhwc on y instead");
@@ -421,7 +424,7 @@
     info[0] = r.g.CT; info[1] = r.PT; info[2] = r.t.total; info[3] = (int32_t)r.nb; info[4] = r.g.cch; info[5] = r.g.nchunks;
     info[6] = r.family <= CONV_ROWS ? r.family : 0;
     const int lean = 1 << CONV_LEAN, rows = 1 << CONV_ROWS;
-    const int feeds = MSAU_CONV_IDS | MSAU_CONV_OWNER | MSAU_CONV_NCHW | MSAU_CONV_WGRAD;
+    const int feeds = MSAU_CONV_IDS | MSAU_CONV_OWNER | MSAU_CONV_NCHW | MSAU_CONV_CODES | MSAU_CONV_WGRAD;
     const int fused = MSAU_CONV_HEAD | MSAU_CONV_DOUT | MSAU_CONV_LRN | MSAU_CONV_POOL;
     info[7] = (conv_offers(dtype, d, MSAU_CONV_HEAD, feeds | fused, lean) == CONV_LEAN) |
               ((conv_offers(dtype, d, MSAU_CONV_DOUT, feeds | fused, lean) == CONV_LEAN ||
@@ -487,7 +490,7 @@
     int rc = conv_route(dtype, d, &r);
     if (rc) return rc;
     const bool refused = r.family == CONV_REFUSED;
-    if (refused && (r.refused & (MSAU_CONV_EXTENT | MSAU_CONV_WGRAD | MSAU_CONV_OWNER | MSAU_CONV_NCHW))) return conv_refusal(d, r.refused);
+    if (refused && (r.refused & (MSAU_CONV_EXTENT | MSAU_CONV_WGRAD | MSAU_CONV_OWNER | MSAU_CONV_NCHW | MSAU_CONV_CODES))) return conv_refusal(d, r.refused);
     if (d->flags & MSAU_CONV_HEAD)
         MSAU_CHECK_ARG(d->head_probs && d->head_argmax && d->head_classes > 0 && d->head_classes <= 16 &&
                        d->head_classes <= d->Cout && d->flags == MSAU_CONV_HEAD, "conv2d: bad HEAD arguments");
diff --git a/msau_amd/csrc/conv_first.hip b/msau_amd/csrc/conv_first.hip
--- a/msau_amd/csrc/conv_first.hip
+++ b/msau_amd/csrc/conv_first.hip
@@ -23,13 +23,16 @@
     int nseg, SH;
     int slot_px;
     int relu_out;
+    unsigned* codes;
 };
+
+constexpr unsigned kDense = 0xFFFFFFFFu;
 
 __device__ __forceinline__ __amdgpu_buffer_rsrc_t rsrc_of(const void* p, unsigned bytes) {
     return __builtin_amdgcn_make_buffer_rsrc(const_cast<void*>(p), 0, bytes, 0x00020000);
 }
 
-template <int NI, int NTW>
+template <int NI, int NTW, bool CODES = false>
 __global__ __launch_bounds__(256) void first_conv_nchw_kernel(const FirstArgs a) {
     extern __shared__ __align__(16) unsigned char smem[];
     const int tid = threadIdx.x, lane = tid & 63;
@@ -66,6 +69,7 @@
     unsigned char* nb = a.xn ? a.xn + (size_t)b * img_n : nullptr;
     const unsigned img_y = (unsigned)H * (unsigned)W * 16u;
     const __amdgpu_buffer_rsrc_t ry = rsrc_of(a.y + (size_t)b * img_y, img_y);
+    const unsigned img_c = (unsigned)H * (unsigned)W * 4u;
 
     const int cg = lane & 7, qs = lane >> 3;
     unsigned ld_off[NI];
@@ -95,16 +99,37 @@
         const bool own = r >= y0 && r < y1;
         const __amdgpu_buffer_rsrc_t rn = rsrc_of(nb, own && nb ? img_n : 0u);
         const unsigned no = own ? (unsigned)r * (unsigned)W * 128u : 0u;
+        __amdgpu_buffer_rsrc_t rc = rn;
+        if constexpr (CODES) rc = rsrc_of(a.codes + (size_t)b * H * W, own ? img_c : 0u);
 #pragma unroll
         for (int it = 0; it < NI; ++it) {
+            u32x4 code;
 #pragma unroll
             for (int p = 0; p < 4; ++p) {
                 bf16x8 o;
 #pragma unroll
                 for (int k = 0; k < 8; ++k) o[k] = (bf16_t)v[it][k][p];
                 *reinterpret_cast<bf16x8*>(slot + lds_px[it] + (lds_px[it] ? p * PS : 0) + cg * 16) = o;
-                __builtin_amdgcn_raw_buffer_store_b128(__builtin_bit_cast(u32x4, o), rn, st_off[it] + (unsigned)p * 128u + no, 0, 0);
-            }
+                if constexpr (CODES) {
+                    const u32x4 ob = __builtin_bit_cast(u32x4, o);
+                    unsigned t = 0u;
+#pragma unroll
+                    for (int k = 0; k < 8; ++k) {
+                        const unsigned bits = (ob[k >> 1] >> ((k & 1) * 16)) & 0xFFFFu;
+                        t += bits ? (1u << 24) | (unsigned)(cg * 8 + k) << 16 | bits : 0u;
+                    }
+                    t += (unsigned)__builtin_amdgcn_update_dpp(0, (int)t, 0xB1, 0xF, 0xF, false);
+                    t += (unsigned)__builtin_amdgcn_update_dpp(0, (int)t, 0x4E, 0xF, 0xF, false);
+                    t += (unsigned)__builtin_amdgcn_update_dpp(0, (int)t, 0x141, 0xF, 0xF, false);
+                    const unsigned n = t >> 24;
+                    code[p] = n == 0u ? 0u : n == 1u ? t & 0x00FFFFFFu : kDense;
+                    __builtin_amdgcn_raw_buffer_store_b128(ob, rn, n > 1u ? st_off[it] + (unsigned)p * 128u + no : kOOB, 0, 0);
+                } else {
+                    __builtin_amdgcn_raw_buffer_store_b128(__builtin_bit_cast(u32x4, o), rn, st_off[it] + (unsigned)p * 128u + no, 0, 0);
+                }
+            }
+            if constexpr (CODES)
+                __builtin_amdgcn_raw_buffer_store_b128(code, rc, cg == 0 && st_off[it] != kOOB ? (st_off[it] >> 5) + (no >> 5) : kOOB, 0, 0);
         }
     };
 
@@ -170,7 +195,7 @@
 int msau_firstconv_takes(int dtype, const msau_conv_desc* d) {
     static const bool off = std::getenv("MSAU_FIRST_NCHW") && std::getenv("MSAU_FIRST_NCHW")[0] == '0';
     if (off || dtype != MSAU_BF16 || !d) return 0;
-    if (d->flags & ~(MSAU_CONV_NCHW | MSAU_CONV_RELU_OUT)) return 0;
+    if (d->flags & ~(MSAU_CONV_NCHW | MSAU_CONV_RELU_OUT | MSAU_CONV_CODES)) return 0;
     if (d->C1 != 64 || d->C2 || d->Cout != 8 || d->KH != 3 || d->KW != 3 || d->dil != 1 || d->stride != 1 || d->ups != 1) return 0;
     if (d->pad_t != 1 || d->pad_l != 1 || d->Hin != d->Hout || d->Win != d->Wout) return 0;
     if (d->Win % 4 || d->Win > 320 || d->Win < 16 || d->Hin < 2) return 0;
@@ -179,9 +204,19 @@
     return 1;
 }
 
+extern "C" int msau_firstconv_takes_codes(int dtype, const msau_conv_desc* d) {
+    if (!d) return 0;
+    msau_conv_desc p = *d;
+    p.flags |= MSAU_CONV_NCHW | MSAU_CONV_CODES;
+    return msau_firstconv_takes(dtype, &p);
+}
+
 int msau_firstconv_launch(hipStream_t s, int dtype, const msau_conv_desc* d, int real_channels) {
     (void)dtype;
+    const bool coded = d->flags & MSAU_CONV_CODES;
+    if (coded && !(d->codes && d->y2)) return msau_set_error(MSAU_ERR_ARG, "first_conv: MSAU_CONV_CODES needs codes and y2");
     FirstArgs a;
+    a.codes = coded ? d->codes : nullptr;
     a.x = static_cast<const float*>(d->x1);
     a.xn = static_cast<unsigned char*>(d->y2);
     a.wpack = static_cast<const bf16_t*>(d->wpack);
@@ -197,20 +232,44 @@
     a.relu_out = (d->flags & MSAU_CONV_RELU_OUT) ? 1 : 0;
     const int lds = 3 * a.slot_px * PS + W_BYTES;
     const int ni = cdiv(d->Win, 128), ntw = cdiv(d->Win, 64);
-#define FIRST_CASE(NIV, NTWV)                                                                                                  \
-    if (ni <= NIV && ntw <= NTWV) {                                                                                            \
+#define FIRST_CASE(NIV, NTWV, CODED)                                                                                           \
+    if (ni <= NIV && ntw <= NTWV && coded == CODED) {                                                                          \
         static bool attr_set = false;                                                                                          \
         if (!attr_set) {                                                                                                       \
-            hipError_t e = hipFuncSetAttribute(reinterpret_cast<const void*>(&first_conv_nchw_kernel<NIV, NTWV>),              \
+            hipError_t e = hipFuncSetAttribute(reinterpret_cast<const void*>(&first_conv_nchw_kernel<NIV, NTWV, CODED>),       \
                                                hipFuncAttributeMaxDynamicSharedMemorySize, MSAU_LDS_LIMIT);                    \
             if (e != hipSuccess) return msau_set_error(MSAU_ERR_HIP, "first_conv: hipFuncSetAttribute: %s", hipGetErrorString(e)); \
             attr_set = true;                                                                                                   \
         }                                                                                                                      \
-        hipLaunchKernelGGL((first_conv_nchw_kernel<NIV, NTWV>), dim3(a.B * a.nseg), dim3(256), lds, s, a);                    \
+        hipLaunchKernelGGL((first_conv_nchw_kernel<NIV, NTWV, CODED>), dim3(a.B * a.nseg), dim3(256), lds, s, a);             \
         MSAU_CHECK_LAUNCH("first_conv_nchw_kernel");                                                                           \
         return 0;                                                                                                              \
     }
-    FIRST_CASE(1, 2) FIRST_CASE(2, 4) FIRST_CASE(3, 5)
+    FIRST_CASE(1, 2, false) FIRST_CASE(2, 4, false) FIRST_CASE(3, 5, false)
+    FIRST_CASE(1, 2, true) FIRST_CASE(2, 4, true) FIRST_CASE(3, 5, true)
 #undef FIRST_CASE
     return msau_set_error(MSAU_ERR_ARG, "first_conv: no instance for width %d", d->Win);
 }
+
+namespace {
+__global__ __launch_bounds__(256) void codes_to_nhwc_kernel(const unsigned* __restrict__ codes, unsigned char* __restrict__ dst, long long n8) {
+    const long long i = (long long)blockIdx.x * 256 + threadIdx.x;
+    if (i >= n8) return;
+    const unsigned code = codes[i >> 3];
+    if (code == kDense) return;
+    const int cg = (int)(i & 7), c = (int)(code >> 16);
+    u32x4 v = u32x4{0u, 0u, 0u, 0u};
+    if (code && (c >> 3) == cg) v[(c & 7) >> 1] = (code & 0xFFFFu) << ((c & 1) * 16);
+    *reinterpret_cast<u32x4*>(dst + i * 16) = v;
+}
+}
+
+extern "C" int msau_codes_to_nhwc(void* stream, int dtype, const uint32_t* codes, void* dst, int64_t npix) {
+    MSAU_CHECK_ARG(codes && dst && npix >= 0 && dtype == MSAU_BF16, "codes_to_nhwc: bf16 storage, 64 stored channels");
+    if (!npix) return 0;
+    const long long n8 = (long long)npix * 8;
+    MSAU_CHECK_ARG(cdiv64(n8, 256) < (1ll << 31), "codes_to_nhwc: grid too large");
+    hipLaunchKernelGGL(codes_to_nhwc_kernel, dim3((unsigned)cdiv64(n8, 256)), dim3(256), 0, static_cast<hipStream_t>(stream), codes, static_cast<unsigned char*>(dst), n8);
+    MSAU_CHECK_LAUNCH("codes_to_nhwc_kernel");
+    return 0;
+}
diff --git a/msau_amd/csrc/conv_wgrad.hip b/msau_amd/csrc/conv_wgrad.hip
--- a/msau_amd/csrc/conv_wgrad.hip
+++ b/msau_amd/csrc/conv_wgrad.hip
@@ -292,13 +292,14 @@
         return msau_ownerconv_wgrad(static_cast<hipStream_t>(stream), dtype, d, g.cch, g.nchunks, g.kextc);
     const int tiles_x = cdiv(d->Wout, 16), tiles_y = cdiv(d->Hout, 16), ntiles = d->B * tiles_x * tiles_y;
     MSAU_CHECK_ARG(d->nslabs >= 1 && d->nslabs <= ntiles, "wgrad: nslabs %d not in [1,%d]", d->nslabs, ntiles);
-    if (msau_rowwgrad_takes(dtype, d, g.cch, g.nchunks, g.kextc))
+    if (!(d->flags & MSAU_CONV_CODES) && msau_rowwgrad_takes(dtype, d, g.cch, g.nchunks, g.kextc))
         return msau_rowwgrad_launch(static_cast<hipStream_t>(stream), d);
     if (d->Cout <= g.slice) {
         rc = msau_wgrad_lean_try(static_cast<hipStream_t>(stream), dtype, d, g.cch, g.nchunks, g.kextc);
         if (rc != 0) return rc < 0 ? rc : 0;
     }
     MSAU_CHECK_ARG(!(d->flags & MSAU_CONV_IDS), "wgrad: MSAU_CONV_IDS is implemented by the bf16 64 -> 8 3x3 instance only");
+    MSAU_CHECK_ARG(!(d->flags & MSAU_CONV_CODES), "wgrad: MSAU_CONV_CODES is implemented by the bf16 64 -> 8 3x3 instance only");
     int CTN = g.CTN == 3 ? 4 : (g.CTN > 4 ? 8 : g.CTN);
     MSAU_CHECK_ARG(!(CTN == 8 && g.NKW > 5), "wgrad: Cout %d with K %d unsupported", d->Cout, g.kextc);
     dim3 grid(d->nslabs, g.nchunks);
diff --git a/msau_amd/csrc/wgrad_lean.hip b/msau_amd/csrc/wgrad_lean.hip
--- a/msau_amd/csrc/wgrad_lean.hip
+++ b/msau_amd/csrc/wgrad_lean.hip
@@ -319,8 +319,11 @@
     static constexpr int LDS = TILE_BYTES > RED_BYTES ? TILE_BYTES : RED_BYTES;
 };
 
-template <bool IDS>
+enum { W64_DENSE = 0, W64_IDS = 1, W64_CODES = 2 };
+constexpr unsigned kDenseCode = 0xFFFFFFFFu;
+template <int SRC>
 __global__ __launch_bounds__(256) void wgrad_in64_kernel(const WLeanArgs a) {
+    constexpr bool IDS = SRC == W64_IDS, CODES = SRC == W64_CODES;
     typedef bf16_t T;
     typedef Vec8<T>::type V8;
     constexpr int PSX = WIn64::PSX, PSG = WIn64::PSG, TG = WIn64::TG;
@@ -362,6 +365,16 @@
 
     V8 xr[IDS ? 1 : 8], gr[2];
     int idr = -1;
+    unsigned cdr = 0u, cdn = 0u;
+    auto code_of = [&](int tile) -> unsigned {
+        if (tile >= a.ntiles) return 0u;
+        const int t1 = a.tiles_x > 1 ? __umulhi((unsigned)tile, a.mag_tx) : tile;
+        const int txi = tile - t1 * a.tiles_x;
+        const int b = a.tiles_y > 1 ? __umulhi((unsigned)t1, a.mag_ty) : t1;
+        const int tyi = t1 - b * a.tiles_y;
+        const int iy = tyi * 16 + (tid >> 4), ix = txi * 16 + (tid & 15);
+        return iy < d.Hin && ix < d.Win ? d.codes[((long long)b * d.Hin + iy) * d.Win + ix] : 0u;
+    };
     auto issue_loads = [&](int tile) {
         const int t1 = a.tiles_x > 1 ? __umulhi((unsigned)tile, a.mag_tx) : tile;
         const int txi = tile - t1 * a.tiles_x;
@@ -373,6 +386,14 @@
             const int iy = iy0 + (tid >> 4), ix = ix0 + (tid & 15);
             idr = -1;
             if (iy < d.Hin && ix < d.Win) idr = static_cast<const int*>(d.x1)[((long long)b * d.Hin + iy) * d.Win + ix];
+        } else if constexpr (CODES) {
+            cdr = cdn;
+            cdn = code_of(tile + gridDim.x);
+            if (cdr == kDenseCode) {
+                const int iy = iy0 + (tid >> 4), ix = ix0 + (tid & 15);
+#pragma unroll
+                for (int cg = 0; cg < 8; ++cg) xr[cg] = *reinterpret_cast<const V8*>(xb + (unsigned)(iy * in_row + ix * in_px + cg * 16));
+            }
         } else
 #pragma unroll
         for (int it = 0; it < 8; ++it) {
@@ -394,6 +415,7 @@
                 gr[it] = *reinterpret_cast<const V8*>(gb + (unsigned)(oy * g_row + ox * g_px));
         }
     };
+    if constexpr (CODES) cdn = code_of(blockIdx.x);
     if ((int)blockIdx.x < a.ntiles) issue_loads(blockIdx.x);
 
     for (int tile = blockIdx.x; tile < a.ntiles; tile += gridDim.x) {
@@ -405,6 +427,21 @@
 #pragma unroll
                 for (int j = 0; j < 8; ++j) v[j] = (T)(cg * 8 + j == idr ? 1.0f : 0.0f);
                 *reinterpret_cast<V8*>(lds_x + tid * PSX + cg * 16) = v;
+            }
+        } else if constexpr (CODES) {
+            if (cdr == kDenseCode) {
+#pragma unroll
+                for (int cg = 0; cg < 8; ++cg) *reinterpret_cast<V8*>(lds_x + tid * PSX + cg * 16) = xr[cg];
+            } else {
+                typedef unsigned u32x4 __attribute__((ext_vector_type(4)));
+                const unsigned c = cdr >> 16, val = (cdr & 0xFFFFu) << ((c & 1u) * 16u), cw = c >> 1;
+#pragma unroll
+                for (int cg = 0; cg < 8; ++cg) {
+                    u32x4 v;
+#pragma unroll
+                    for (int w = 0; w < 4; ++w) v[w] = cw == (unsigned)(cg * 4 + w) ? val : 0u;
+                    *reinterpret_cast<u32x4*>(lds_x + tid * PSX + cg * 16) = v;
+                }
             }
         } else
 #pragma unroll
@@ -501,11 +538,15 @@
 
 int launch_wgrad_in64(hipStream_t s, const WLeanArgs& a) {
     if (a.kextc != 592) return 0;
-    if (a.d.flags & MSAU_CONV_IDS) {
+    if (a.d.flags & MSAU_CONV_CODES) {
+        if (a.nchunks != 1 || a.d.C2 || a.d.flags != MSAU_CONV_CODES || !a.d.codes)
+            return msau_set_error(MSAU_ERR_ARG, "wgrad: MSAU_CONV_CODES needs one 64-channel source, its codes and no other flag");
+        hipLaunchKernelGGL(wgrad_in64_kernel<W64_CODES>, dim3(a.d.nslabs, 1), dim3(256), WIn64::LDS, s, a);
+    } else if (a.d.flags & MSAU_CONV_IDS) {
         if (a.nchunks != 1 || a.d.C2) return msau_set_error(MSAU_ERR_ARG, "wgrad: MSAU_CONV_IDS needs one 64-channel one-hot source");
-        hipLaunchKernelGGL(wgrad_in64_kernel<true>, dim3(a.d.nslabs, 1), dim3(256), WIn64::LDS, s, a);
+        hipLaunchKernelGGL(wgrad_in64_kernel<W64_IDS>, dim3(a.d.nslabs, 1), dim3(256), WIn64::LDS, s, a);
     } else
-    hipLaunchKernelGGL(wgrad_in64_kernel<false>, dim3(a.d.nslabs, a.nchunks), dim3(256), WIn64::LDS, s, a);
+    hipLaunchKernelGGL(wgrad_in64_kernel<W64_DENSE>, dim3(a.d.nslabs, a.nchunks), dim3(256), WIn64::LDS, s, a);
     MSAU_CHECK_LAUNCH("wgrad_in64_kernel");
     return 1;
 }
@@ -601,6 +642,7 @@
 int msau_wgrad_lean_group(hipStream_t s, int dtype, const msau_wgrad_desc* const* ds, int n, int cch, int nchunks, int kextc) {
     const msau_wgrad_desc* d = ds[0];
     if (n < 1 || n > kWGroup || !msau_wgrad_lean_applicable(dtype, d, cch)) return 0;
+    if ((d->flags & MSAU_CONV_CODES) && !(wlean_in64(dtype, d, cch) && kextc == 592)) return 0;
     WLeanMulti m;
     for (int i = 0; i < n; ++i) wlean_fill(m.a[i], ds[i], nchunks, kextc);
     for (int i = n; i < kWGroup; ++i) m.a[i] = m.a[0];
diff --git a/msau_amd/model.py b/msau_amd/model.py
--- a/msau_amd/model.py
+++ b/msau_amd/model.py
@@ -830,6 +830,7 @@
             sx.copy_(x, non_blocking=True)
             sl.copy_(labels, non_blocking=True)
             g1.replay()
+            plan.input_rewritten()
             self._allreduce()
             g2.replay()
         cur.wait_stream(gs)
diff --git a/msau_amd/plan.py b/msau_amd/plan.py
--- a/msau_amd/plan.py
+++ b/msau_amd/plan.py
@@ -67,6 +67,27 @@
     def alloc_grad(self):
         if self.needs_grad and self.n_contrib > 0 and self.grad is None:
             self.grad = torch.zeros_like(self.data)
+
+
+class InputAct(Act):
+
+    stale = False
+
+    @property
+    def data(self):
+        if self.stale:
+            self.stale = False
+            L.call("msau_codes_to_nhwc", torch.cuda.current_stream().cuda_stream, self.plan.dtype, self.plan._codes.data_ptr(),
+                   self._data.data_ptr(), self.npix)
+        return self._data
+
+    @data.setter
+    def data(self, t):
+        self._data = t
+
+    @property
+    def raw(self):
+        return self._data
 
 
 class Op:
@@ -949,7 +970,7 @@
         self._side = None
         self.deterministic = bool(cfg.get("deterministic", os.environ.get("MSAU_DETERMINISTIC", "0") == "1"))
         self.overlap_max_pix = int(cfg.get("overlap_max_pix", 1 << 62))
-        self.x_in = Act(self, "input", H, W, cfg["channels"], needs_grad=bool(cfg.get("input_grad", False)))
+        self.x_in = InputAct(self, "input", H, W, cfg["channels"], needs_grad=bool(cfg.get("input_grad", False)))
         self.logits: Optional[Act] = None
         self.aux: Optional[Act] = None
         if builder is None:
@@ -1291,6 +1312,11 @@
             T = "f32" if self.dtype == L.F32 else "bf16"
             c.fkey = f"first_conv_nchw<{T},CIN{a.Cs},CO{c.out.Cs}>"
             c.fbytes = api_bytes + (a.npix * a.Cs * esz if self.training else 0) + c.out.npix * c.out.Cs * esz
+            if self._codes is not None:
+                c.fkey = f"first_conv_nchw<{T},CIN{a.Cs},CO{c.out.Cs},codes>"
+                c.fbytes = api_bytes + a.npix * 4 + c.out.npix * c.out.Cs * esz
+                c.wkey = f"wgrad_lean_kernel<{T},C{c.wgeom.cch},CO{c.wdesc.Cout},K{c.wdesc.KH},codes>"
+                c.wbytes = a.npix * 4 + c.out.npix * c.out.Cs * esz + c.wdesc.nslabs * c.wgeom.slab_bytes
         nparam = sum(int(math.prod(shp)) for shp in self.pshape.values())
         out.append(Launch(0, None, "msau_pack_params", nparam * 4 + self._pack_bytes))
         if self.training:
@@ -1366,6 +1392,7 @@
     def load_input(self, x_nchw: torch.Tensor):
         assert x_nchw.dtype == torch.float32 and x_nchw.is_contiguous() and tuple(x_nchw.shape) == \
             (self.B, self.cfg["channels"], self.H, self.W), (x_nchw.shape, x_nchw.dtype)
+        self._feed_nchw(None)
         a = self.x_in
         L.call("msau_nchw_to_nhwc", self._stream(), self.dtype, x_nchw.data_ptr(), a.data.data_ptr(), self.B, a.C, a.Cs, self.H, self.W)
         if self.ragged:
@@ -1381,6 +1408,13 @@
                 ok = bool(info[7] & 64)
             self._nchw_conv = c if ok else None
             self._nchw_on = False
+            self._codes = None
+            if ok and self.training and c.wdesc is not None and os.environ.get("MSAU_FIRST_CODES", "1") != "0" \
+                    and L.load().msau_firstconv_takes_codes(self.dtype, C.byref(c.fdesc)) \
+                    and self.dtype == L.BF16 and c.wgeom.lean == 1 and c.wdesc.C1 == 64 and c.wdesc.C2 == 0 and c.wdesc.Cout == 8 \
+                    and c.wdesc.KH == 3 and c.wgeom.nchunks == 1 and c.wgeom.kext == 592 and c.wdesc.flags == 0 \
+                    and os.environ.get("MSAU_WGRAD_IN64", "1") != "0":
+                self._codes = torch.zeros((self.B, self.H, self.W), dtype=torch.int32, device=self.device)
         return self._nchw_conv
 
     def _feed_nchw(self, x_nchw: Optional[torch.Tensor]) -> bool:
@@ -1395,17 +1429,30 @@
         if x_nchw is not None:
             c.fdesc.flags |= L.CONV_NCHW
             c.fdesc.x1 = x_nchw.data_ptr()
-            c.fdesc.y2 = _ptr(self.x_in.data) if self.training else None
+            c.fdesc.y2 = _ptr(self.x_in.raw) if self.training else None
             c.fdesc.head_classes = self.x_in.C
+            if self._codes is not None:
+                c.fdesc.flags |= L.CONV_CODES
+                c.fdesc.codes = c.wdesc.codes = self._codes.data_ptr()
+                c.wdesc.flags |= L.CONV_CODES
+                self.x_in.stale = True
             self._nchw_on = True
             return True
         if self._nchw_on:
-            c.fdesc.flags &= ~L.CONV_NCHW
-            c.fdesc.x1 = _ptr(self.x_in.data)
+            c.fdesc.flags &= ~(L.CONV_NCHW | L.CONV_CODES)
+            c.fdesc.x1 = _ptr(self.x_in.raw)
             c.fdesc.y2 = None
             c.fdesc.head_classes = 0
+            if self._codes is not None:
+                c.fdesc.codes = c.wdesc.codes = None
+                c.wdesc.flags &= ~L.CONV_CODES
+                self.x_in.stale = False
             self._nchw_on = False
         return False
+
+    def input_rewritten(self):
+        if getattr(self, "_nchw_on", False) and self._codes is not None:
+            self.x_in.stale = True
 
     def _feed_ids(self, ids: Optional[torch.Tensor]) -> bool:
         self._feed_nchw(None)
@@ -1433,10 +1480,10 @@
             self._ids_keep = ids
         else:
             c.fdesc.flags &= ~L.CONV_IDS
-            c.fdesc.x1 = _ptr(self.x_in.data)
+            c.fdesc.x1 = _ptr(self.x_in.raw)
             if c.wdesc is not None:
                 c.wdesc.flags &= ~L.CONV_IDS
-                c.wdesc.x1 = _ptr(self.x_in.data)
+                c.wdesc.x1 = _ptr(self.x_in.raw)
             self._ids_keep = None
         return True
 
@@ -1465,10 +1512,10 @@
         if src is None:
             if self._owner_keep is not None:
                 c.fdesc.flags &= ~L.CONV_OWNER
-                c.fdesc.x1 = _ptr(self.x_in.data)
+                c.fdesc.x1 = _ptr(self.x_in.raw)
                 if c.wdesc is not None:
                     c.wdesc.flags &= ~(L.CONV_OWNER | L.CONV_EXTENT)
-                    c.wdesc.x1 = _ptr(self.x_in.data)
+                    c.wdesc.x1 = _ptr(self.x_in.raw)
                     self._set_unpack_slabs(c, c.wdesc.nslabs)
                 self._owner_keep = None
             return True
@@ -1551,17 +1598,17 @@
 
     def input_buffer(self, k: int) -> torch.Tensor:
         if not hasattr(self, "_x_bufs"):
-            self._x_bufs = [self.x_in.data, None]
+            self._x_bufs = [self.x_in.raw, None]
         if self._x_bufs[k] is None:
-            self._x_bufs[k] = torch.zeros_like(self.x_in.data)
+            self._x_bufs[k] = torch.zeros_like(self.x_in.raw)
         return self._x_bufs[k]
 
     def use_input(self, k: int):
         buf = self.input_buffer(k)
-        if buf is self.x_in.data:
+        if buf is self.x_in.raw:
             return
         self._feed_ids(None)
-        old = self.x_in.data.data_ptr()
+        old = self.x_in.raw.data_ptr()
         for op in self.ops:
             if isinstance(op, ConvOp):
                 for d in (op.fdesc, op.wdesc):
```

New measurement: 5744 tiles/s (median of 6 runs). About the same (+0.3%).
